# ilovin/lstm_ctc_ocr

Measured on AMD Instinct MI355X. Metric: captcha images/sec training (32x256, bs=64/GPU), higher is better.
Workload: dtype bf16; 1 GPU; VGG-7 + BiLSTM(256) + CTC train step, H=32 W=256, 10-char labels, C=64, bs=64/GPU (BASELINE.json configs[1]), Adam lr 1e-4 wd 1e-5 clip 10; global_batch=64, parallelism=dp1, hipgraph=True

## Files before the change

### include/ocr_hip.h

```cpp
#ifndef OCR_HIP_H
#define OCR_HIP_H
#include <stddef.h>
#ifdef __cplusplus
extern "C" {
#endif

enum { OCR_STATUS_OK = 0, OCR_STATUS_MEMOPS = 1, OCR_STATUS_INVALID = 2, OCR_STATUS_EXEC = 3 };

enum {
    OCR_EPI_BIAS = 1, OCR_EPI_RELU = 2, OCR_EPI_OUT_F32 = 4,
    OCR_EPI_MASK = 16, OCR_EPI_ROWSWAP = 32, OCR_EPI_ACCUM = 64
};

const char* ocr_status_string(int status);
int ocr_abi_version(void);
const char* ocr_build_id(void);

int ocr_ctc_workspace_size(int max_label_len, int max_time, int minibatch, size_t* bytes);
int ocr_ctc_loss(const float* activations, float* gradients, const int* flat_labels, const int* label_lengths,
                 const int* input_lengths, int alphabet_size, int minibatch, int max_time, int max_label_len,
                 int blank_label, float* costs, void* workspace, void* stream);
int ocr_ctc_debug(void* dbg);
int ocr_ctc_train_supported(int alphabet_size, int max_time, int max_label_len);
int ocr_ctc_loss_train(const float* activations, void* grad_ntc_bf16, float scale, const int* flat_labels,
                       const int* label_lengths, const int* input_lengths, int alphabet_size, int minibatch, int max_time,
                       int max_label_len, int blank_label, float* costs, void* stream);
int ocr_set_ctc_engine(int fast);
int ocr_ctc_long_placement(int alphabet_size, int max_time, int max_label_len);
int ocr_ctc_long_supported(int alphabet_size, int max_time, int max_label_len);
int ocr_ctc_long_workspace_size(int alphabet_size, int max_label_len, int max_time, int minibatch, size_t* bytes);
int ocr_ctc_loss_long(const float* activations, float* gradients ,
                      void* grad_ntc_bf16 , float scale,
                      const int* flat_labels, const int* label_lengths, const int* input_lengths,
                      int alphabet_size, int minibatch, int max_time, int max_label_len, int blank_label,
                      float* costs, void* workspace, size_t workspace_bytes, void* stream);
int ocr_ctc_greedy_decode(const float* activations, const int* input_lengths, int alphabet_size, int minibatch,
                          int max_time, int blank_label, int pad_value, int* decoded, int* decoded_lengths,
                          void* stream);

int ocr_ctc_beam_workspace_size(int alphabet_size, int minibatch, int max_time, int beam_width, size_t* bytes);
int ocr_ctc_beam_decode(const float* activations, const int* input_lengths, int alphabet_size, int minibatch,
                        int max_time, int beam_width, int merge_repeated, int pad_value, int* decoded,
                        int* decoded_lengths, float* neg_log_prob, void* workspace, size_t workspace_bytes, void* stream);
int ocr_ctc_beam_kernel_choice(int alphabet_size, int beam_width);
int ocr_set_beam_engine(int engine);

int ocr_gemm_nt_bf16(const void* P, long ldp, const void* Q, long ldq, void* out, long ldo, int M, int N, int K,
                     const float* bias, const void* mask, long ldmask, int flags, int splits, int row_group,
                     int row_skip, int swap_inner, int swap_outer, void* stream);
int ocr_set_gemm_engine(int use_large_tile);
int ocr_conv3x3_bf16(const void* x, const void* wpack, void* y, int Nb, int W, int H, int Cin, int Cout,
                     const float* bias, const void* mask, int flags, void* stream);
int ocr_conv3x3_stats_rows(int Nb, int W, int H, int Cin, int Cout, int flags);
int ocr_conv3x3_bf16_stats(const void* x, const void* wpack, void* y, int Nb, int W, int H, int Cin, int Cout, const float* bias, int flags,
                           float* partials, void* stream);
int ocr_conv3x3_kernel_choice(int Nb, int W, int H, int Cin, int Cout, int flags, int kw, int kh);
int ocr_conv3x3_accum_supported(int Nb, int W, int H, int Cin, int Cout);
int ocr_conv_halo_clock_debug(void* dbg);
int ocr_conv_ws_debug(void* dbg);
int ocr_conv3x3_pool_supported(int Nb, int W, int H, int Cin, int Cout, int kw, int kh);
int ocr_conv3x3_pool_codes_supported(int Nb, int W, int H, int Cin, int Cout, int kw, int kh);
int ocr_conv3x3_relu_pool_codes_bf16(const void* x, const void* wpack, void* y, void* pooled, void* codes, int Nb, int W, int H, int Cin,
                                     int Cout, const float* bias, int kw, int kh, void* stream);
int ocr_conv3x3_relu_pool_bf16(const void* x, const void* wpack, void* y, void* pooled, int Nb, int W, int H, int Cin, int Cout,
                               const float* bias, int kw, int kh, void* stream);
int ocr_conv3x3_unpool_supported(int Nb, int W, int H, int Cin, int Cout, int kw, int kh);
int ocr_conv3x3_dgrad_unpool_bf16(const void* dy, const void* wdgrad, void* out_full, const void* codes, int Nb, int W, int H, int Cin,
                                  int Cout, int kw, int kh, int relu_mask, void* stream);
int ocr_gemm_tn_bf16(const void* A, long lda, const void* B, long ldb, float* out, long ldo, int Mk, int I, int J,
                     int row_group, int row_skip, long a_row_off, float scale, int splits, float* colsum, void* stream);
long ocr_gemm_tn_split_workspace_floats(int Mk, int I, int J);
int ocr_gemm_tn_split_bf16(const void* A, long lda, const void* B, long ldb, float* out, long ldo, int Mk, int I, int J, float scale,
                           float* colsum, float* part, long part_floats, void* stream);
int ocr_gemm_tn_batched_bf16(const void* A, long lda, long strideA, const void* B, long ldb, long strideB, float* out, long ldo,
                             long strideOut, int Mk, int I, int J, int nbatch, float scale, int splits, float* colsum,
                             long strideColsum, void* stream);
typedef struct ocr_tn_job {
    const void* A; long lda; long strideA;
    const void* B; long ldb; long strideB;
    float* out; long ldo; long strideOut;
    float* colsum; long strideColsum;
    int Mk, I, J, nbatch;
    int row_group, row_skip;
    float scale; int reserved;
} ocr_tn_job;
int ocr_gemm_tn_jobs_supported(const ocr_tn_job* jobs, int njobs);
int ocr_gemm_tn_jobs_bf16(const ocr_tn_job* jobs, int njobs, void* stream);
int ocr_set_wgrad_engine(int engine);
int ocr_conv3x3_wgrad_bf16(const void* x, const void* dy, float* dw, float* dbias, int Nb, int W, int H, int Cin,
                           int Cout, int splits, void* stream);
int ocr_conv3x3_wgrad_kernel_choice(int Nb, int W, int H, int Cin, int Cout, int has_workspace, int splits);

int ocr_conv3x3_wgrad_workspace_size(int Nb, int W, int H, int Cin, int Cout, size_t* bytes);
int ocr_conv3x3_wgrad_ws_bf16(const void* x, const void* dy, float* dw, float* dbias, int Nb, int W, int H, int Cin,
                              int Cout, int splits, void* workspace, size_t workspace_bytes, void* stream);
int ocr_conv3x3_wgrad_defer_bf16(const void* x, const void* dy, float* dw, float* dbias, int Nb, int W, int H, int Cin, int Cout,
                                 void* workspace, size_t workspace_bytes, void* job, int* job_blocks, int* deferred, void* stream);
int ocr_wgrad9_reduce_jobs(const void* jobs, int njobs, int total_blocks, void* stream);

int ocr_conv1_fwd(const float* x, const float* w, const float* bias, void* y, int Nb, int W, int H, int Cout,
                  int relu, void* stream);
int ocr_conv1_wgrad(const float* x, const void* dz, float* dw, float* db, int Nb, int W, int H, int Cout,
                    void* stream);
int ocr_eltwise_bf16(int op, const void* a, const void* b, void* out, long n, void* stream);
int ocr_conv1_pool_fwd(const float* x, const float* w, const float* bias, void* p, int Nb, int W, int H, int Cout, void* stream);
int ocr_conv1_pool_fwd_train(const float* x, const float* w, const float* bias, void* p, int Nb, int W, int H, int Cout,
                             void* codes, float* zero, long zero_n, void* ones, long ones_n, void* stream);
int ocr_conv1_pool_bwd_codes(const float* x, const float* w, const float* bias, const void* dp, float* dw, float* db,
                             int Nb, int W, int H, int Cout, const void* codes, void* stream);
int ocr_conv1_pool_bwd_slab_rows(int Nb, int W, int H);
int ocr_conv1_pool_bwd_slab(const float* x, const float* w, const float* bias, const void* dp, int Nb, int W, int H, int Cout,
                            const void* codes, float* slab, void* stream);
int ocr_conv1_pool_bwd(const float* x, const float* w, const float* bias, const void* dp, float* dw, float* db, int Nb,
                       int W, int H, int Cout, void* stream);
int ocr_maxpool_fwd(const void* x, void* y, int Nb, int W, int H, int C, int kw, int kh, void* stream);
int ocr_maxpool_bwd(const void* x, const void* dy, void* dx, int Nb, int W, int H, int C, int kw, int kh,
                    int relu_mask, void* stream);
int ocr_maxpool_bwd_codes(const void* codes, const void* dy, void* dx, int Nb, int W, int H, int C, int kw, int kh,
                          int relu_mask, void* stream);
size_t ocr_bn_workspace_bytes(long M, int C);
int ocr_bn_train_fwd(const void* x, void* y, const float* gamma, const float* beta, float* save_mean,
                     float* save_rstd, long M, int C, float eps, int relu, void* workspace, const void* residual, void* stream);
int ocr_bn_train_bwd(const void* x, const void* y, const void* dy, void* dx, const float* gamma,
                     const float* save_mean, const float* save_rstd, float* dgamma, float* dbeta, long M, int C,
                     int relu, void* workspace, void* stream);
int ocr_bn_train_fwd2(const void* x, void* y, const float* gamma, const float* beta, float* save_mean, float* save_rstd, long M, int C,
                      float eps, int relu, void* workspace, const void* residual, int partial_rows, void* pooled, void* stream);
int ocr_bn_train_bwd2(const void* x, const void* y, const void* dy, void* dx, const float* gamma, const float* save_mean,
                      const float* save_rstd, float* dgamma, float* dbeta, long M, int C, int relu, void* workspace, int pooled_dy,
                      int partial_rows, void* stream);
int ocr_bn_train_fwd_codes(const void* x, const float* gamma, const float* beta, float* save_mean, float* save_rstd, long M, int C,
                           float eps, int relu, void* workspace, int partial_rows, void* pooled, void* codes, void* stream);
int ocr_bn_train_bwd_codes(const void* x, const void* codes, const void* dy, void* dx, const float* gamma, const float* save_mean,
                           const float* save_rstd, float* dgamma, float* dbeta, long M, int C, int relu, void* workspace, void* stream);
int ocr_bn_train_bwd_codes_col(const void* x, const void* codes, const void* col, int Nb, int W, int HC, void* dy_pooled_out, void* dx,
                               const float* gamma, const float* save_mean, const float* save_rstd, float* dgamma, float* dbeta, long M,
                               int C, int relu, void* workspace, void* stream);
int ocr_conv3x3_bnbwd_rows(int Nb, int W, int H, int Cin, int Cout);
int ocr_conv3x3_dgrad_bnbwd_bf16(const void* dy, const void* wdgrad, void* dx, int Nb, int W, int H, int Cin, int Cout, const void* mask_y,
                                 const void* z, const float* mean, const float* rstd, float* partials, void* stream);
int ocr_colsum_bf16(const void* a, float* out, long M, int C, long lda, void* stream);
int ocr_pack_transpose(const float* in, void* out, int R, int Cc, long ldin, int lstm_units, void* stream);
int ocr_pack_conv_dgrad(const float* w, void* out, int Cin, int Cout, void* stream);
int ocr_pack_jobs(const void* jobs, int njobs, int total_blocks, void* stream);
int ocr_cast_f32_bf16(const float* in, void* out, long n, void* stream);
int ocr_u8_to_unit_f32(const void* in, float* out, long n, void* stream);
int ocr_step_report(const float* costs, int n, const double* scalars, const void* word_addrs, int nwords, double* out, void* stream);
int ocr_bind_batch(const void* pixels, int pixels_are_u8, float* x, long n_pixels, const int* seq_len, int* seq_len_dst, int n_seq,
                   const int* labels, int* labels_dst, int n_labels, const int* labels_len, int* labels_len_dst, int n_labels_len,
                   void* stream);
int ocr_cast2d_f32_bf16(const float* in, long ldin, void* out, long ldout, int rows, int cols, void* stream);
int ocr_tnc_to_ntc_bf16(const float* in, void* out, int T, int N, int C, float scale, void* stream);
int ocr_conv5_col2im(const void* col, void* dx, int Nb, int W, int HC, void* stream);

int ocr_bn_infer_fwd(const void* x, void* y, const float* gamma, const float* beta, const float* mean, const float* var,
                     long M, int C, float eps, int relu, void* stream);
int ocr_bn_infer_bwd(const void* x, const void* y, const void* dy, void* dx, const float* gamma, const float* mean,
                     const float* var, float* dgamma, float* dbeta, long M, int C, float eps, int relu, void* stream);
int ocr_dropout_bf16(const void* in, void* out, long n, unsigned seed, const void* step_counter, float keep_prob, void* stream);
int ocr_avgpool_bf16(const void* src, void* dst, int Nb, int W, int H, int C, int kw, int kh, int backward, void* stream);
int ocr_subsample_bf16(const void* src, void* dst, int Nb, int W, int H, int C, int Wo, int Ho, int sw, int sh, int ow, int oh,
                       int backward, void* stream);
int ocr_softmax_f32(const float* in, float* out, long rows, int C, void* stream);

int ocr_lstm_fwd_step(const float* xproj, const void* whT_packed, const int* seq_len, void* hout, float* gates,
                      float* cell, int Nb, int T, int U, int step, float forget_bias, int ndir, void* stream);
int ocr_lstm_bwd_step(const void* wh, long ldw, long w_dir_stride, const int* seq_len, const void* dhout,
                      const float* gates, const float* cell, void* dz, float* dc_state, int Nb, int T, int U,
                      int step, int ndir, void* stream);
int ocr_lstm_seq_supported(int Nb, int U);
long ocr_lstm_seq_sync_words(int Nb, int U);
int ocr_lstm_seq_debug(void* dbg );
int ocr_lstm_seq_test_skew(int units, int at);
int ocr_lstm_fwd_seq(const float* xproj, const void* whT_packed, const int* seq_len, void* hout, float* gates,
                     float* cell, int Nb, int T, int U, float forget_bias, void* sync, void* stream);
int ocr_lstm_bwd_seq(const void* wh, long ldw, long w_dir_stride, const int* seq_len, const void* dhout,
                     const float* gates, const float* cell, void* dz, int Nb, int T, int U, void* sync, void* stream);
#define OCR_LSTM_PREPARED 1
int ocr_lstm_fwd_seq2(const float* xproj, const void* whT_packed, const int* seq_len, void* hout, float* gates,
                      float* cell, int Nb, int T, int U, float forget_bias, void* sync, int flags, void* stream);
int ocr_lstm_bwd_seq2(const void* wh, long ldw, long w_dir_stride, const int* seq_len, const void* dhout,
                      const float* gates, const float* cell, void* dz, int Nb, int T, int U, void* sync, int flags, void* stream);
int ocr_lstm_fwd_seq_x_supported(int Nb, int U, int D);
int ocr_lstm_fwd_seq_x(const void* x, const void* wxT_packed, const float* bias_packed, int D, const void* whT_packed,
                       const int* seq_len, void* hout, float* gates, float* cell, int Nb, int T, int U, float forget_bias,
                       void* sync, int flags, void* stream);
int ocr_set_lstm_proto(int proto);
int ocr_set_lstm_ksplit(int waves);
int ocr_lstm_hprev(const void* hout, const int* seq_len, void* hprev, int Nb, int T, int U, int ndir, void* stream);
int ocr_lstm_xh(const void* x, const void* hout, const int* seq_len, void* xh, int Nb, int T, int D, int U, int ndir, void* stream);
int ocr_lstm_pack_bias(const float* b_fw, const float* b_bw , float* out, int U, int ndir, void* stream);

int ocr_optim_scalar_count(void);
int ocr_optim_init(void* scalars , double lr, void* stream);
int ocr_optim_set_lr(void* scalars, double lr, int multiply, void* stream);
int ocr_optim_step(float* params, float* grads, float* state1, float* state2, long n, long reg_begin, long reg_end,
                   float weight_decay, float clip_norm, int solver, float beta1, float beta2, float eps,
                   void* scalars, void* stream);
int ocr_optim_step_guarded(float* params, float* grads, float* state1, float* state2, long n, long reg_begin, long reg_end,
                           float weight_decay, float clip_norm, int solver, float beta1, float beta2, float eps,
                           void* scalars, const void* guard_addrs, int nguard, void* stream);
int ocr_optim_step_guarded2(float* params, float* grads, float* state1, float* state2, long n, long reg_begin, long reg_end,
                            float weight_decay, float clip_norm, int solver, float beta1, float beta2, float eps,
                            void* scalars, const void* guard_addrs, int nguard, const float* drop_flag, void* stream);
int ocr_guard_flag(const void* guard_addrs, int nguard, float* flag_out, void* stream);

int ocr_captcha_synth(const int* params, int n_images, int words_per_image, int max_glyphs, const void* atlas, const int* stamp, int n_stamp,
                      void* out, int W, int out_h, int canvas_cap, int width_cap, void* stream);

int ocr_wgrad9_debug(void* dbg);

int ocr_probe_tr16(const int* addr , int* out , void* stream);
int ocr_probe_xcc(int* out , int nblocks, int threads, void* stream);
int ocr_occupy_cus(int nblocks, int threads, int lds_bytes, float us, void* stream);
int ocr_mfma_busy_probe(float* out, int nblocks, int threads , int iters, long long* clk, void* stream);

#ifdef __cplusplus
}
#endif
#endif
```

### lstm_ctc_ocr_amd/_native.py

```python
import ctypes
import os
import re

_HERE = os.path.dirname(os.path.abspath(__file__))
LIB_PATH = os.environ.get("OCR_NATIVE_LIB") or os.path.join(_HERE, "libocrhip.so")
HEADER_PATH = os.path.join(os.path.dirname(_HERE), "include", "ocr_hip.h")

EPI_BIAS, EPI_RELU, EPI_OUT_F32, EPI_MASK, EPI_ROWSWAP, EPI_ACCUM = 1, 2, 4, 16, 32, 64

_P, _I, _L, _F, _D = ctypes.c_void_p, ctypes.c_int, ctypes.c_long, ctypes.c_float, ctypes.c_double

_SIGS = {
    "ocr_abi_version": ([], _I),
    "ocr_build_id": ([], ctypes.c_char_p),
    "ocr_status_string": ([_I], ctypes.c_char_p),
    "ocr_ctc_workspace_size": ([_I, _I, _I, ctypes.POINTER(ctypes.c_size_t)], _I),
    "ocr_ctc_loss": ([_P, _P, _P, _P, _P, _I, _I, _I, _I, _I, _P, _P, _P], _I),
    "ocr_set_ctc_engine": ([_I], _I),
    "ocr_ctc_debug": ([_P], _I),
    "ocr_ctc_train_supported": ([_I, _I, _I], _I),
    "ocr_ctc_loss_train": ([_P, _P, _F, _P, _P, _P, _I, _I, _I, _I, _I, _P, _P], _I),
    "ocr_ctc_long_placement": ([_I, _I, _I], _I),
    "ocr_ctc_long_supported": ([_I, _I, _I], _I),
    "ocr_ctc_long_workspace_size": ([_I, _I, _I, _I, ctypes.POINTER(ctypes.c_size_t)], _I),
    "ocr_ctc_loss_long": ([_P, _P, _P, _F, _P, _P, _P, _I, _I, _I, _I, _I, _P, _P, ctypes.c_size_t, _P], _I),
    "ocr_ctc_greedy_decode": ([_P, _P, _I, _I, _I, _I, _I, _P, _P, _P], _I),
    "ocr_ctc_beam_workspace_size": ([_I, _I, _I, _I, ctypes.POINTER(ctypes.c_size_t)], _I),
    "ocr_ctc_beam_decode": ([_P, _P, _I, _I, _I, _I, _I, _I, _P, _P, _P, _P, ctypes.c_size_t, _P], _I),
    "ocr_ctc_beam_kernel_choice": ([_I, _I], _I),
    "ocr_set_beam_engine": ([_I], _I),
    "ocr_gemm_nt_bf16": ([_P, _L, _P, _L, _P, _L, _I, _I, _I, _P, _P, _L, _I, _I, _I, _I, _I, _I, _P], _I),
    "ocr_set_gemm_engine": ([_I], _I),
    "ocr_gemm_tn_batched_bf16": ([_P, _L, _L, _P, _L, _L, _P, _L, _L, _I, _I, _I, _I, _F, _I, _P, _L, _P], _I),
    "ocr_gemm_tn_jobs_supported": ([_P, _I], _I),
    "ocr_gemm_tn_jobs_bf16": ([_P, _I, _P], _I),
    "ocr_lstm_xh": ([_P, _P, _P, _P, _I, _I, _I, _I, _I, _P], _I),
    "ocr_set_wgrad_engine": ([_I], _I),
    "ocr_conv3x3_bf16": ([_P, _P, _P, _I, _I, _I, _I, _I, _P, _P, _I, _P], _I),
    "ocr_conv_halo_clock_debug": ([_P], _I),
    "ocr_occupy_cus": ([_I, _I, _I, _F, _P], _I),
    "ocr_conv_ws_debug": ([_P], _I),
    "ocr_conv3x3_accum_supported": ([_I, _I, _I, _I, _I], _I),
    "ocr_conv3x3_kernel_choice": ([_I, _I, _I, _I, _I, _I, _I, _I], _I),
    "ocr_conv3x3_pool_supported": ([_I, _I, _I, _I, _I, _I, _I], _I),
    "ocr_conv3x3_relu_pool_bf16": ([_P, _P, _P, _P, _I, _I, _I, _I, _I, _P, _I, _I, _P], _I),
    "ocr_conv3x3_pool_codes_supported": ([_I, _I, _I, _I, _I, _I, _I], _I),
    "ocr_conv3x3_relu_pool_codes_bf16": ([_P, _P, _P, _P, _P, _I, _I, _I, _I, _I, _P, _I, _I, _P], _I),
    "ocr_gemm_tn_bf16": ([_P, _L, _P, _L, _P, _L, _I, _I, _I, _I, _I, _L, _F, _I, _P, _P], _I),
    "ocr_gemm_tn_split_workspace_floats": ([_I, _I, _I], _L),
    "ocr_gemm_tn_split_bf16": ([_P, _L, _P, _L, _P, _L, _I, _I, _I, _F, _P, _P, _L, _P], _I),
    "ocr_conv3x3_wgrad_bf16": ([_P, _P, _P, _P, _I, _I, _I, _I, _I, _I, _P], _I),
    "ocr_conv3x3_wgrad_kernel_choice": ([_I, _I, _I, _I, _I, _I, _I], _I),
    "ocr_conv3x3_wgrad_workspace_size": ([_I, _I, _I, _I, _I, ctypes.POINTER(ctypes.c_size_t)], _I),
    "ocr_conv3x3_wgrad_ws_bf16": ([_P, _P, _P, _P, _I, _I, _I, _I, _I, _I, _P, ctypes.c_size_t, _P], _I),
    "ocr_conv3x3_wgrad_defer_bf16": ([_P, _P, _P, _P, _I, _I, _I, _I, _I, _P, ctypes.c_size_t, _P, ctypes.POINTER(_I),
                                      ctypes.POINTER(_I), _P], _I),
    "ocr_wgrad9_reduce_jobs": ([_P, _I, _I, _P], _I),
    "ocr_conv1_fwd": ([_P, _P, _P, _P, _I, _I, _I, _I, _I, _P], _I),
    "ocr_conv1_wgrad": ([_P, _P, _P, _P, _I, _I, _I, _I, _P], _I),
    "ocr_eltwise_bf16": ([_I, _P, _P, _P, _L, _P], _I),
    "ocr_conv1_pool_fwd": ([_P, _P, _P, _P, _I, _I, _I, _I, _P], _I),
    "ocr_conv1_pool_fwd_train": ([_P, _P, _P, _P, _I, _I, _I, _I, _P, _P, _L, _P, _L, _P], _I),
    "ocr_conv1_pool_bwd_codes": ([_P, _P, _P, _P, _P, _P, _I, _I, _I, _I, _P, _P], _I),
    "ocr_conv1_pool_bwd_slab_rows": ([_I, _I, _I], _I),
    "ocr_conv1_pool_bwd_slab": ([_P, _P, _P, _P, _I, _I, _I, _I, _P, _P, _P], _I),
    "ocr_conv1_pool_bwd": ([_P, _P, _P, _P, _P, _P, _I, _I, _I, _I, _P], _I),
    "ocr_maxpool_fwd": ([_P, _P, _I, _I, _I, _I, _I, _I, _P], _I),
    "ocr_maxpool_bwd": ([_P, _P, _P, _I, _I, _I, _I, _I, _I, _I, _P], _I),
    "ocr_bn_workspace_bytes": ([_L, _I], ctypes.c_size_t),
    "ocr_bn_train_fwd": ([_P, _P, _P, _P, _P, _P, _L, _I, _F, _I, _P, _P, _P], _I),
    "ocr_bn_train_bwd": ([_P, _P, _P, _P, _P, _P, _P, _P, _P, _L, _I, _I, _P, _P], _I),
    "ocr_bn_train_fwd2": ([_P, _P, _P, _P, _P, _P, _L, _I, _F, _I, _P, _P, _I, _P, _P], _I),
    "ocr_bn_train_bwd2": ([_P, _P, _P, _P, _P, _P, _P, _P, _P, _L, _I, _I, _P, _I, _I, _P], _I),
    "ocr_maxpool_bwd_codes": ([_P, _P, _P, _I, _I, _I, _I, _I, _I, _I, _P], _I),
    "ocr_bn_train_fwd_codes": ([_P, _P, _P, _P, _P, _L, _I, _F, _I, _P, _I, _P, _P, _P], _I),
    "ocr_bn_train_bwd_codes": ([_P, _P, _P, _P, _P, _P, _P, _P, _P, _L, _I, _I, _P, _P], _I),
    "ocr_bn_train_bwd_codes_col": ([_P, _P, _P, _I, _I, _I, _P, _P, _P, _P, _P, _P, _P, _L, _I, _I, _P, _P], _I),
    "ocr_conv3x3_unpool_supported": ([_I, _I, _I, _I, _I, _I, _I], _I),
    "ocr_conv3x3_dgrad_unpool_bf16": ([_P, _P, _P, _P, _I, _I, _I, _I, _I, _I, _I, _I, _P], _I),
    "ocr_conv3x3_bnbwd_rows": ([_I, _I, _I, _I, _I], _I),
    "ocr_conv3x3_dgrad_bnbwd_bf16": ([_P, _P, _P, _I, _I, _I, _I, _I, _P, _P, _P, _P, _P, _P], _I),
    "ocr_conv3x3_stats_rows": ([_I, _I, _I, _I, _I, _I], _I),
    "ocr_conv3x3_bf16_stats": ([_P, _P, _P, _I, _I, _I, _I, _I, _P, _I, _P, _P], _I),
    "ocr_bn_infer_fwd": ([_P, _P, _P, _P, _P, _P, _L, _I, _F, _I, _P], _I),
    "ocr_bn_infer_bwd": ([_P, _P, _P, _P, _P, _P, _P, _P, _P, _L, _I, _F, _I, _P], _I),
    "ocr_dropout_bf16": ([_P, _P, _L, ctypes.c_uint, _P, _F, _P], _I),
    "ocr_avgpool_bf16": ([_P, _P, _I, _I, _I, _I, _I, _I, _I, _P], _I),
    "ocr_subsample_bf16": ([_P, _P, _I, _I, _I, _I, _I, _I, _I, _I, _I, _I, _I, _P], _I),
    "ocr_softmax_f32": ([_P, _P, _L, _I, _P], _I),
    "ocr_colsum_bf16": ([_P, _P, _L, _I, _L, _P], _I),
    "ocr_pack_transpose": ([_P, _P, _I, _I, _L, _I, _P], _I),
    "ocr_pack_conv_dgrad": ([_P, _P, _I, _I, _P], _I),
    "ocr_pack_jobs": ([_P, _I, _I, _P], _I),
    "ocr_cast_f32_bf16": ([_P, _P, _L, _P], _I),
    "ocr_u8_to_unit_f32": ([_P, _P, _L, _P], _I),
    "ocr_step_report": ([_P, _I, _P, _P, _I, _P, _P], _I),
    "ocr_bind_batch": ([_P, _I, _P, _L, _P, _P, _I, _P, _P, _I, _P, _P, _I, _P], _I),
    "ocr_captcha_synth": ([_P, _I, _I, _I, _P, _P, _I, _P, _I, _I, _I, _I, _P], _I),
    "ocr_cast2d_f32_bf16": ([_P, _L, _P, _L, _I, _I, _P], _I),
    "ocr_tnc_to_ntc_bf16": ([_P, _P, _I, _I, _I, _F, _P], _I),
    "ocr_conv5_col2im": ([_P, _P, _I, _I, _I, _P], _I),
    "ocr_lstm_fwd_step": ([_P, _P, _P, _P, _P, _P, _I, _I, _I, _I, _F, _I, _P], _I),
    "ocr_lstm_bwd_step": ([_P, _L, _L, _P, _P, _P, _P, _P, _P, _I, _I, _I, _I, _I, _P], _I),
    "ocr_lstm_seq_supported": ([_I, _I], _I),
    "ocr_lstm_seq_debug": ([_P], _I),
    "ocr_lstm_seq_test_skew": ([_I, _I], _I),
    "ocr_lstm_seq_sync_words": ([_I, _I], _L),
    "ocr_lstm_fwd_seq": ([_P, _P, _P, _P, _P, _P, _I, _I, _I, _F, _P, _P], _I),
    "ocr_lstm_bwd_seq": ([_P, _L, _L, _P, _P, _P, _P, _P, _I, _I, _I, _P, _P], _I),
    "ocr_lstm_fwd_seq2": ([_P, _P, _P, _P, _P, _P, _I, _I, _I, _F, _P, _I, _P], _I),
    "ocr_lstm_fwd_seq_x_supported": ([_I, _I, _I], _I),
    "ocr_lstm_fwd_seq_x": ([_P, _P, _P, _I, _P, _P, _P, _P, _P, _I, _I, _I, _F, _P, _I, _P], _I),
    "ocr_lstm_bwd_seq2": ([_P, _L, _L, _P, _P, _P, _P, _P, _I, _I, _I, _P, _I, _P], _I),
    "ocr_lstm_hprev": ([_P, _P, _P, _I, _I, _I, _I, _P], _I),
    "ocr_lstm_pack_bias": ([_P, _P, _P, _I, _I, _P], _I),
    "ocr_optim_scalar_count": ([], _I),
    "ocr_optim_init": ([_P, _D, _P], _I),
    "ocr_optim_set_lr": ([_P, _D, _I, _P], _I),
    "ocr_optim_step": ([_P, _P, _P, _P, _L, _L, _L, _F, _F, _I, _F, _F, _F, _P, _P], _I),
    "ocr_optim_step_guarded": ([_P, _P, _P, _P, _L, _L, _L, _F, _F, _I, _F, _F, _F, _P, _P, _I, _P], _I),
    "ocr_optim_step_guarded2": ([_P, _P, _P, _P, _L, _L, _L, _F, _F, _I, _F, _F, _F, _P, _P, _I, _P, _P], _I),
    "ocr_guard_flag": ([_P, _I, _P, _P], _I),
    "ocr_wgrad9_debug": ([_P], _I),
    "ocr_probe_tr16": ([_P, _P, _P], _I),
    "ocr_set_lstm_proto": ([_I], _I),
    "ocr_set_lstm_ksplit": ([_I], _I),
    "ocr_probe_xcc": ([_P, _I, _I, _P], _I),
    "ocr_mfma_busy_probe": ([_P, _I, _I, _I, _P, _P], _I),
}


class NativeError(RuntimeError):
    pass


def declared_symbols(header=HEADER_PATH):
    text = open(header).read()
    text = re.sub(r"/\*.*?\*/", "", text, flags=re.S)
    return sorted(set(re.findall(r"\b(ocr_[a-z0-9_]+)\s*\(", text)))


def source_build_id(csrc=os.path.join(_HERE, "csrc"), experiments=False):
    import glob
    import hashlib
    rel = [os.path.basename(f) for f in glob.glob(os.path.join(csrc, "*.hip"))]
    h = hashlib.sha256()
    for f in sorted(rel) + ["common.h", "conv_plan.h", "Makefile"]:
        h.update(open(os.path.join(csrc, f), "rb").read())
    return h.hexdigest()[:16] + ("-exp" if experiments else "")


def build_id():
    return lib().ocr_build_id().decode()


_lib = None


def lib():
    global _lib
    if _lib is None:
        if not os.path.exists(LIB_PATH):
            raise NativeError(
                "libocrhip.so not found at %s — build it with `python -c 'import __graft_entry__ as g; g.build()'` "
                "(there is no CPU/eager fallback for the hot path)" % LIB_PATH)
        _lib = ctypes.CDLL(LIB_PATH)
        for name, (argtypes, restype) in _SIGS.items():
            fn = getattr(_lib, name)
            fn.argtypes = argtypes
            fn.restype = restype
        for env, setter in (("OCR_GEMM_ENGINE", "ocr_set_gemm_engine"), ("OCR_WGRAD_ENGINE", "ocr_set_wgrad_engine")):
            if os.environ.get(env):
                getattr(_lib, setter)(int(os.environ[env]))
    return _lib


def status_string(code):
    return lib().ocr_status_string(code).decode()


def call(name, *args):
    rc = getattr(lib(), name)(*args)
    if rc != 0:
        raise NativeError("%s failed: status %d (%s)" % (name, rc, status_string(rc)))


def ptr(t):
    return None if t is None else t.data_ptr()


def stream():
    import torch
    return torch.cuda.current_stream().cuda_stream
```

### lstm_ctc_ocr_amd/csrc/common.h

```cpp
#pragma once
#include <stdlib.h>
#include <hip/hip_runtime.h>
#include <stdint.h>
#include <atomic>

#define OCR_WAVE 64

enum {
    OCR_OK = 0,
    OCR_ERR_MEMOPS = 1,
    OCR_ERR_INVALID = 2,
    OCR_ERR_EXEC = 3,
};

#define OCR_CHECK_LAUNCH()                                        \
    do {                                                          \
        hipError_t e__ = hipGetLastError();                       \
        if (e__ != hipSuccess) return OCR_ERR_EXEC;               \
    } while (0)

typedef uint16_t bf16_t;
typedef __attribute__((ext_vector_type(8))) __bf16 bf16x8;
typedef __attribute__((ext_vector_type(4))) float f32x4;
typedef __attribute__((ext_vector_type(4))) unsigned int u32x4;
typedef __attribute__((ext_vector_type(2))) unsigned int u32x2;

__device__ __forceinline__ bf16_t f2bf(float f) {
    uint32_t u = __float_as_uint(f);
    if ((u & 0x7fffffffu) > 0x7f800000u) return (bf16_t)((u >> 16) | 0x40);
    u += 0x7fffu + ((u >> 16) & 1u);
    return (bf16_t)(u >> 16);
}
__device__ __forceinline__ float bf2f(bf16_t h) { return __uint_as_float(((uint32_t)h) << 16); }
typedef __attribute__((ext_vector_type(2))) __bf16 bf16x2_t;
__device__ __forceinline__ uint32_t pack_bf2(float lo, float hi) {
    bf16x2_t v = {(__bf16)lo, (__bf16)hi};
    return __builtin_bit_cast(uint32_t, v);
}
__device__ __forceinline__ float bf_lo(uint32_t p) { return __uint_as_float(p << 16); }
__device__ __forceinline__ float bf_hi(uint32_t p) { return __uint_as_float(p & 0xffff0000u); }

template <int CNT>
__device__ __forceinline__ uint32_t pool_code_word(const u32x4 (&rows)[CNT]) {
    uint32_t word = 0;
#pragma unroll
    for (int c = 0; c < 8; ++c) {
        float v[CNT];
#pragma unroll
        for (int e = 0; e < CNT; ++e) {
            const uint32_t pr = c < 2 ? rows[e].x : c < 4 ? rows[e].y : c < 6 ? rows[e].z : rows[e].w;
            v[e] = (c & 1) ? bf_hi(pr) : bf_lo(pr);
        }
        int best = 0; float bv = v[0];
#pragma unroll
        for (int e = 1; e < CNT; ++e) if (v[e] > bv) { bv = v[e]; best = e; }
        word |= (uint32_t)(best | ((bv > 0.f) ? 4 : 0)) << (4 * c);
    }
    return word;
}

typedef unsigned short u16x2_t __attribute__((ext_vector_type(2)));
template <int CNT>
__device__ __forceinline__ uint32_t pool_code2_u16(const uint32_t (&p)[CNT], uint32_t& mx) {
    const u16x2_t one = {1, 1};
    u16x2_t v[CNT];
#pragma unroll
    for (int e = 0; e < CNT; ++e) v[e] = __builtin_bit_cast(u16x2_t, p[e]);
    u16x2_t m = v[0];
#pragma unroll
    for (int e = 1; e < CNT; ++e) m = __builtin_elementwise_max(m, v[e]);
    u16x2_t t = __builtin_elementwise_min((u16x2_t)(m - v[CNT - 2]), one);
#pragma unroll
    for (int e = CNT - 3; e >= 0; --e) t = __builtin_elementwise_min((u16x2_t)(m - v[e]), one) * (u16x2_t)(t + one);
    const u16x2_t code = t + (u16x2_t)(__builtin_elementwise_min(m, one) << (u16x2_t){2, 2});
    mx = __builtin_bit_cast(uint32_t, m);
    return __builtin_bit_cast(uint32_t, code);
}
__device__ __forceinline__ uint32_t pool_code2_merge(uint32_t c0, uint32_t c1, uint32_t c2, uint32_t c3) {
    return ((c0 | (c0 >> 12)) & 0xffu) | (((c1 | (c1 >> 12)) & 0xffu) << 8) | (((c2 | (c2 >> 12)) & 0xffu) << 16) | ((c3 | (c3 >> 12)) << 24);
}

__device__ __forceinline__ void unpack8(u32x4 p, float* f) {
    f[0] = bf_lo(p.x); f[1] = bf_hi(p.x); f[2] = bf_lo(p.y); f[3] = bf_hi(p.y);
    f[4] = bf_lo(p.z); f[5] = bf_hi(p.z); f[6] = bf_lo(p.w); f[7] = bf_hi(p.w);
}
__device__ __forceinline__ uint32_t max2(uint32_t a, uint32_t b) {
    uint32_t lo = (bf_lo(b) > bf_lo(a)) ? (b & 0xffffu) : (a & 0xffffu);
    uint32_t hi = (bf_hi(b) > bf_hi(a)) ? (b & 0xffff0000u) : (a & 0xffff0000u);
    return lo | hi;
}
__device__ __forceinline__ u32x4 max8(u32x4 a, u32x4 b) {
    u32x4 r = {max2(a.x, b.x), max2(a.y, b.y), max2(a.z, b.z), max2(a.w, b.w)};
    return r;
}
__device__ __forceinline__ u32x4 col2im_unit8(const bf16_t* __restrict__ col, unsigned idx, int W, int HC) {
    const unsigned hc8 = (unsigned)HC >> 3;
    const unsigned e = (idx % hc8) * 8u, q = idx / hc8;
    const unsigned w = q % (unsigned)W, n = q / (unsigned)W;
    float a[8], b[8];
#pragma unroll
    for (int c = 0; c < 8; ++c) { a[c] = 0.f; b[c] = 0.f; }
    const long r0 = ((long)n * (W - 1) + w) * 2L;
    if ((int)w < W - 1) unpack8(*(const u32x4*)(col + r0 * HC + e), a);
    if (w > 0) unpack8(*(const u32x4*)(col + (r0 - 1) * HC + e), b);
    bf16_t o[8];
#pragma unroll
    for (int c = 0; c < 8; ++c) o[c] = f2bf((0.f + a[c]) + b[c]);
    u32x4 pk = {(uint32_t)o[0] | ((uint32_t)o[1] << 16), (uint32_t)o[2] | ((uint32_t)o[3] << 16),
                (uint32_t)o[4] | ((uint32_t)o[5] << 16), (uint32_t)o[6] | ((uint32_t)o[7] << 16)};
    return pk;
}

__device__ __forceinline__ float wave_sum(float v) {
#pragma unroll
    for (int o = 32; o > 0; o >>= 1) v += __shfl_xor(v, o, 64);
    return v;
}
__device__ __forceinline__ float wave_max(float v) {
#pragma unroll
    for (int o = 32; o > 0; o >>= 1) v = fmaxf(v, __shfl_xor(v, o, 64));
    return v;
}
template <typename AccT, bool STORE = false>
__device__ __forceinline__ void block_channel_reduce(const float (&v)[8], float* red, AccT* dst, int C, int groups,
                                                     int rl, int gq, int rlanes) {
    __syncthreads();
    if (rl < rlanes) {
#pragma unroll
        for (int c = 0; c < 8; ++c) red[rl * C + gq * 8 + c] = v[c];
    }
    __syncthreads();
    for (int ch = threadIdx.x; ch < C; ch += 256) {
        float t = 0.f;
        for (int r = 0; r < rlanes; ++r) t += red[r * C + ch];
        if (STORE) dst[ch] = (AccT)t;
        else atomicAdd(&dst[ch], (AccT)t);
    }
}

__device__ __forceinline__ float sigmoidf_(float x) { return __frcp_rn(1.0f + __expf(-x)); }
__device__ __forceinline__ float tanhf_(float x) {
    float e = __expf(-2.0f * fabsf(x));
    float t = (1.0f - e) * __frcp_rn(1.0f + e);
    return copysignf(t, x);
}

static inline const char* ocr_tune_env(const char* name) {
#ifdef OCR_EXPERIMENTS
    return getenv(name);
#else
    (void)name; return nullptr;
#endif
}
__device__ __forceinline__ long long ocr_wall_clock() { return (long long)__builtin_amdgcn_s_memrealtime(); }
__device__ __forceinline__ void ocr_clk_enter(long long* clk) {
    clk[0] = (long long)__builtin_amdgcn_s_memtime(); clk[1] = ocr_wall_clock();
}
__device__ __forceinline__ void ocr_clk_exit(long long* clk) {
    const long long c = (long long)__builtin_amdgcn_s_memtime(), t = ocr_wall_clock();
    clk[2] = c; clk[3] = t;
    clk[4] += c - clk[0]; clk[5] += t - clk[1]; clk[6] += 1;
}
__host__ __device__ static inline int ceil_div(long a, long b) { return (int)((a + b - 1) / b); }
static inline int grid_for(long total, int cap = 4096) {
    long b = (total + 255) / 256;
    if (b > cap) b = cap;
    if (b < 1) b = 1;
    return (int)b;
}

#define OCR_MAX_DEVICES 64
template <auto KERNEL>
static inline hipError_t ocr_allow_lds(int bytes) {
    static std::atomic<int> allowed[OCR_MAX_DEVICES];
    int dev = 0;
    if (hipGetDevice(&dev) != hipSuccess || dev < 0 || dev >= OCR_MAX_DEVICES) return hipErrorInvalidDevice;
    int have = allowed[dev].load(std::memory_order_acquire);
    if (bytes <= have) return hipSuccess;
    const hipError_t e = hipFuncSetAttribute((const void*)KERNEL, hipFuncAttributeMaxDynamicSharedMemorySize, bytes);
    if (e != hipSuccess) return e;
    while (have < bytes && !allowed[dev].compare_exchange_weak(have, bytes, std::memory_order_acq_rel)) {}
    return hipSuccess;
}
```

### lstm_ctc_ocr_amd/csrc/gemm.hip

```cpp
#include "conv_plan.h"
#include <string.h>

enum {
    EPI_BIAS = 1,
    EPI_RELU = 2,
    EPI_OUT_F32 = 4,
    EPI_ATOMIC = 8,
    EPI_MASK = 16,
    EPI_ROWSWAP = 32,
    EPI_ACCUM = 64,
};

struct GemmArgs {
    const bf16_t* P;
    const bf16_t* Q;
    long ldp, ldq;
    int M, N, K;
    int k_per_split;
    int grp, skip;
    int cW, cH, cC;
    void* out;
    long ldo;
    const float* bias;
    const bf16_t* mask;
// ... 118 lines not shown
#pragma unroll
            for (int b = 0; b < FM; ++b)
                bfr[b] = *(const bf16x8*)(&Ps[(wm * 16 * FM + b * 16 + frow) * LDS_ROW + fk]);
#pragma unroll
            for (int a = 0; a < FN; ++a)
#pragma unroll
                for (int b = 0; b < FM; ++b)
                    acc[a][b] = __builtin_amdgcn_mfma_f32_16x16x32_bf16(af[a], bfr[b], acc[a][b], 0, 0, 0);
        }
    }

    const int flags = g.flags;
    const bool add_bias = (flags & EPI_BIAS) && (!(flags & EPI_ATOMIC) || blockIdx.z == 0);
#pragma unroll
    for (int a = 0; a < FN; ++a) {
        int n = n0 + wn * 16 * FN + a * 16 + (lane >> 4) * 4;
        if (n >= g.N) continue;
        f32x4 bv = {0.f, 0.f, 0.f, 0.f};
        if (add_bias) bv = *(const f32x4*)(g.bias + n);
#pragma unroll
        for (int b = 0; b < FM; ++b) {
            int m = m0 + wm * 16 * FM + b * 16 + (lane & 15);
            if (m >= g.M) continue;
            f32x4 v = acc[a][b] + bv;
            if (flags & EPI_RELU) {
                v.x = fmaxf(v.x, 0.f); v.y = fmaxf(v.y, 0.f); v.z = fmaxf(v.z, 0.f); v.w = fmaxf(v.w, 0.f);
            }
            if (flags & EPI_MASK) {
                u32x2 mk = *(const u32x2*)(g.mask + (long)m * g.ldmask + n);
                if (!(bf_lo(mk.x) > 0.f)) v.x = 0.f;
                if (!(bf_hi(mk.x) > 0.f)) v.y = 0.f;
                if (!(bf_lo(mk.y) > 0.f)) v.z = 0.f;
                if (!(bf_hi(mk.y) > 0.f)) v.w = 0.f;
            }
            long orow = m;
            if (flags & EPI_ROWSWAP) orow = (long)(m % g.swap_inner) * g.swap_outer + m / g.swap_inner;
            if (flags & EPI_OUT_F32) {
                float* o = (float*)g.out + orow * g.ldo + n;
                if (flags & EPI_ATOMIC) {
                    atomicAdd(o + 0, v.x); atomicAdd(o + 1, v.y); atomicAdd(o + 2, v.z); atomicAdd(o + 3, v.w);
                } else if (flags & EPI_ACCUM) {
                    f32x4 old = *(f32x4*)o;
                    *(f32x4*)o = old + v;
                } else {
                    *(f32x4*)o = v;
                }
            } else {
                u32x2 pk;
                pk.x = pack_bf2(v.x, v.y);
                pk.y = pack_bf2(v.z, v.w);
                *(u32x2*)((bf16_t*)g.out + orow * g.ldo + n) = pk;
            }
        }
    }
}

template <int MODE, int FM, int FN>
static int launch_gemm(const GemmArgs& g, hipStream_t stream) {
    constexpr int BM = 32 * FM, BN = 32 * FN;
    int splits = ceil_div(g.K, g.k_per_split);
    dim3 grid(ceil_div(g.M, BM), ceil_div(g.N, BN), splits);
    gemm_nt_kernel<MODE, FM, FN><<<grid, 256, 0, stream>>>(g);
    OCR_CHECK_LAUNCH();
    return OCR_OK;
}

static int dispatch_gemm(GemmArgs& g, int mode, int splits, hipStream_t stream) {
    if (g.M <= 0 || g.N <= 0 || g.K <= 0 || (g.K & 7) || (g.N & 3)) return OCR_ERR_INVALID;
    if (!g.P || !g.Q || !g.out) return OCR_ERR_INVALID;
    if (splits < 1) splits = 1;
    int kps = ceil_div(ceil_div(g.K, splits), 32) * 32;
    g.k_per_split = kps;
    if (splits > 1) {
        if (!(g.flags & EPI_OUT_F32) || (g.flags & (EPI_RELU | EPI_MASK | EPI_ACCUM))) return OCR_ERR_INVALID;
        g.flags |= EPI_ATOMIC;
    }
    long big_blocks = (long)ceil_div(g.M, 128) * ceil_div(g.N, 128) * ceil_div(g.K, kps);
    bool big = big_blocks >= 192 && g.N >= 128;
    if (mode == 1) {
        if (g.cC % 32 || g.K != 9 * g.cC) return OCR_ERR_INVALID;
        return big ? launch_gemm<1, 4, 4>(g, stream) : launch_gemm<1, 2, 2>(g, stream);
    }
    return big ? launch_gemm<0, 4, 4>(g, stream) : launch_gemm<0, 2, 2>(g, stream);
}

int ig_try_dispatch(const void* P, long ldp, const void* Q, long ldq, void* out, long ldo, int M, int N, int K,
                    const float* bias, const void* mask, long ldmask, int flags, int mode, int grp, int skip, int cW,
                    int cH, int cC, int swap_inner, int swap_outer, hipStream_t stream);
static int g_use_igemm = 1, g_use_halo = 1;
extern int g_ig_stages;
extern "C" int ocr_set_gemm_engine(int mode) {
    if (mode < 0 || mode > 3) return OCR_ERR_INVALID;
    g_use_igemm = mode != 0; g_use_halo = mode == 1; g_ig_stages = (mode == 2) ? 2 : 3;
    return OCR_OK;
}

extern "C" int ocr_gemm_nt_bf16(const void* P, long ldp, const void* Q, long ldq, void* out, long ldo,
                                int M, int N, int K, const float* bias, const void* mask, long ldmask,
                                int flags, int splits, int row_group, int row_skip, int swap_inner,
                                int swap_outer, void* stream) {
    GemmArgs g = {};
    g.P = (const bf16_t*)P; g.Q = (const bf16_t*)Q; g.ldp = ldp; g.ldq = ldq;
    g.M = M; g.N = N; g.K = K; g.grp = row_group; g.skip = row_skip;
    g.out = out; g.ldo = ldo; g.bias = bias; g.mask = (const bf16_t*)mask; g.ldmask = ldmask;
    g.flags = flags & ~EPI_ATOMIC; g.swap_inner = swap_inner; g.swap_outer = swap_outer;
    if ((flags & EPI_BIAS) && !bias) return OCR_ERR_INVALID;
    if ((flags & EPI_MASK) && !mask) return OCR_ERR_INVALID;
    if ((flags & EPI_ROWSWAP) && (swap_inner <= 0 || swap_outer <= 0)) return OCR_ERR_INVALID;
    if (g_use_igemm && splits <= 1 && P && Q && out && M > 0 && N > 0 && K > 0) {
        int rc = ig_try_dispatch(P, ldp, Q, ldq, out, ldo, M, N, K, bias, mask, ldmask, g.flags, 0, row_group, row_skip, 0, 0, 0,
                                 swap_inner, swap_outer, (hipStream_t)stream);
        if (rc >= 0) return rc;
    }
    return dispatch_gemm(g, 0, splits, (hipStream_t)stream);
}


struct ConvKnobs {
    int ws, k2, k3, k2_cfg;
    int k2_minsteps, k2_mintiles, k2_allow_a, k2_abl, k2_nst;
    int k3_minsteps, k3_genw, k3_prio;
    int halo_nw, halo_stagger, halo_stagger_bit, halo_prio;
};
static int env_int(const char* e, int dflt) { return e ? atoi(e) : dflt; }
static ConvKnobs read_conv_knobs() {
    ConvKnobs k;
    k.ws = env_int(getenv("OCR_CONV_WS"), 1);
    k.k2 = env_int(getenv("OCR_CONV_K2"), 1);
    k.k3 = env_int(getenv("OCR_CONV_K3"), 1);
    const char* cfg = getenv("OCR_K2_CFG");
    k.k2_cfg = (cfg && (cfg[0] == 'A' || cfg[0] == 'D')) ? cfg[0] : 0;
    k.k2_minsteps = env_int(ocr_tune_env("OCR_K2_MINSTEPS"), 18);
    k.k2_mintiles = env_int(ocr_tune_env("OCR_K2_MINTILES"), 128);
    const char* tiles = ocr_tune_env("OCR_K2_TILES");
    k.k2_allow_a = !(tiles && tiles[0] == 'D');
    k.k2_abl = env_int(ocr_tune_env("OCR_K2_ABL"), 0);
    k.k2_nst = env_int(ocr_tune_env("OCR_K2_NST"), 0);
    k.k3_minsteps = env_int(ocr_tune_env("OCR_K3_MINSTEPS"), 18);
    k.k3_genw = env_int(ocr_tune_env("OCR_K3_GENW"), 1);
    k.k3_prio = env_int(ocr_tune_env("OCR_K3_PRIO"), 2);
    k.halo_nw = env_int(ocr_tune_env("OCR_HALO_NW"), 0);
    const char* st = ocr_tune_env("OCR_HALO_STAGGER");
    const char* comma = st ? strchr(st, ',') : nullptr;
    k.halo_stagger = st && atoi(st) > 0 ? atoi(st) : 0;
    k.halo_stagger_bit = comma ? atoi(comma + 1) : 32;
    k.halo_prio = env_int(ocr_tune_env("OCR_HALO_PRIO"), 1);
    return k;
}
static const ConvKnobs& conv_knobs() {
    static const ConvKnobs k = read_conv_knobs();
    return k;
}

static bool plan_ws(ConvPlan& p, const ConvKnobs& k) {
    if (!k.ws || (p.flags & ~(EPI_BIAS | EPI_RELU | EPI_MASK))) return false;
    if (p.epi_kind && (!(p.flags & EPI_RELU) || (p.flags & EPI_MASK))) return false;
    if ((p.Cout & 63) || (long)p.M * p.Cin * 2 > 0x7fffffffL || (long)p.M * p.Cout * 2 > 0x7fffffffL) return false;
    int nc, bm;
    if (p.H == 16 && p.Cin == 64) { nc = 16; bm = 256; }
    else if (p.H == 16 && p.Cin == 128) { nc = 8; bm = 128; }
    else if (p.H == 8 && p.Cin == 128) { nc = 16; bm = 128; }
    else return false;
    if (p.W % nc || p.M % bm || (p.epi_kind == CONV_EPI_POOL22 && (p.W & 1))) return false;
    static int cus = 0;
    if (!cus) {
        int dev = 0; hipDeviceProp_t prop;
        if (hipGetDevice(&dev) == hipSuccess && hipGetDeviceProperties(&prop, dev) == hipSuccess && prop.multiProcessorCount > 0) cus = prop.multiProcessorCount;
    }
    const int ncu = cus > 0 ? cus : 256;
    const int mtiles = p.M / bm, ntiles = p.Cout / 64;
    if (k.ws == 1 && (p.Cin != 64 || (long)mtiles * ntiles < 2L * ncu)) return false;
    int slots = ncu / ntiles;
    if (slots < 1) slots = 1;
    if (slots > mtiles) slots = mtiles;
    p.per_slot = (mtiles + slots - 1) / slots;
    p.slots = (mtiles + p.per_slot - 1) / p.per_slot;
    p.grid = p.slots * ntiles;
    p.xcd_map = (p.grid % 8 == 0 && (p.grid / 8) % ntiles == 0) ? 1 : 0;
    p.family = CONV_WS; p.ws_nc = nc; p.ws_ksplit = p.Cin == 64 ? 1 : 2;
    return true;
}

static char k2_tile(const ConvPlan& p, const ConvKnobs& k, int minsteps) {
    const long M = p.M;
    if ((p.Cin & 63) || (p.Cout & 63) || M < 4096 || p.H > 16 || p.H < 1) return 0;
    if (M * p.Cin * 2 >= 0x7fffffffL || (long)p.Cout * 9 * p.Cin * 2 >= 0x7fffffffL) return 0;
    for (int pass = 0; pass < 2; ++pass)
        for (const char c : {'A', 'D'}) {
            if (k.k2_cfg && c != k.k2_cfg) continue;
            if (!k.k2_cfg && c == 'A' && !k.k2_allow_a) continue;
            const int bn = c == 'A' ? 128 : 64;
            if (p.Cout % bn) continue;
            if (k.k2_cfg) return c;
            if (9 * (p.Cin / 64) < minsteps) return 0;
            if ((M + 255) / 256 * (p.Cout / bn) >= (pass == 0 ? 224 : k.k2_mintiles)) return c;
        }
    return 0;
}

static bool plan_k3(ConvPlan& p, const ConvKnobs& k, char tile) {
    const int H = p.H, epi = p.epi_kind;
    if (H != 2 && H != 4 && H != 8 && H != 16) return false;
    if (p.M % 256 || (p.Cin & 63) || (p.Cout & 63) || (tile == 'A' && p.Cout % 128)) return false;
    const int NC = 256 / H, PS = (NC + 2 + 7) / 8 * 8;
    const bool genw = p.W % NC != 0;
    if (genw && (H == 16 || NC + 2 + (NC + p.W - 1) / p.W > PS)) return false;
    if (genw && !k.k3_genw) return false;
    if (H == 2 && (!genw || epi == CONV_EPI_POOL12 || epi == CONV_EPI_POOL22)) return false;
    if (epi >= CONV_EPI_STATS && (p.flags & EPI_ACCUM)) return false;
    if (epi == CONV_EPI_BNBWD && (!(p.flags & EPI_MASK) || p.Cin == 64 || (H != 4 && H != 8))) return false;
    p.family = CONV_K3; p.tile = tile; p.genw = genw; p.single = H == 16 && p.Cin == 64; p.prio = k.k3_prio;
    return true;
}

static bool plan_k3_k2(ConvPlan& p, const ConvKnobs& k) {
    if (k.k3) {
        const char t = k2_tile(p, k, k.k3_minsteps >= 0 ? k.k3_minsteps : k.k2_minsteps);
        if (t && plan_k3(p, k, t)) return true;
    }
    if (p.epi_kind >= CONV_EPI_STATS) return false;
    const char t = k2_tile(p, k, k.k2_minsteps);
    if (!t) return false;
    int nst = t == 'A' ? 5 : 4;
    if ((t == 'A' && k.k2_nst == 4) || (t == 'D' && (k.k2_nst == 5 || k.k2_nst == 6))) nst = k.k2_nst;
    const int FM = t == 'A' ? 8 : 4, BN = t == 'A' ? 128 : 64;
    const int NRpad = (256 + 2 * p.H + 4 + 7) / 8 * 8;
    const int lds = 2 * NRpad * 128 + nst * BN * 128;
    if (lds > 163840 || lds < 8 * FM * 2048) return false;
#ifdef OCR_EXPERIMENTS
    if (lds + 10240 > 163840 && (k.k2_abl & 8)) return false;
#endif
    p.family = CONV_K2; p.tile = t; p.nst = nst; p.abl = k.k2_abl;
    return true;
}

static bool plan_halo(ConvPlan& p, const ConvKnobs& k) {
    const int H = p.H, Cout = p.Cout, nw = k.halo_nw;
    p.prio = k.halo_prio; p.stagger = k.halo_stagger; p.stagger_bit = k.halo_stagger_bit;
    if (nw != 8) {
        const int NR = 128 + 2 * H + 2, NRp = (NR + 32) / 32 * 32;
        const long mt4 = (p.M + 127) / 128;
        if (NRp / 32 == 5 || NRp / 32 == 6) {
            p.family = CONV_HALO; p.nw = 4; p.bn = (Cout >= 128 && mt4 * ((Cout + 127) / 128) >= 448) ? 128 : 64;
            return true;
        }
        if (nw == 4) return false;
    }
    const int NRpad = (256 + 2 * H + 2 + 64) / 64 * 64;
    if (NRpad / 64 != 5 && NRpad / 64 != 6) return false;
    const long mt = (p.M + 255) / 256;
    p.family = CONV_HALO; p.nw = 8;
    p.bn = (Cout >= 128 && (mt * ((Cout + 127) / 128) >= 200 || mt * ((Cout + 63) / 64) < 256)) ? 128 : 64;
    return true;
}

static void plan_unpool(ConvPlan& p, const ConvKnobs& k) {
    const int H = p.H;
    if (!k.k2 || !k.k3 || p.flags || (H != 4 && H != 8) || p.M <= 0 || p.M % 256 || p.W % (256 / H) || (p.Cin & 63) || (p.Cout & 63)) return;
    if ((long)p.M * p.Cin * 2 >= 0x7fffffffL || (long)p.Cout * 9 * p.Cin * 2 >= 0x7fffffffL) return;
    const ConvPlan plain = conv3x3_plan(p.M, p.W, H, p.Cin, p.Cout, 0, CONV_EPI_PLAIN);
    p.tile = (plain.family == CONV_K3 && !plain.genw) ? plain.tile : ((p.Cout % 128) ? 'D' : 'A');
    p.family = CONV_K3; p.genw = false; p.single = false; p.prio = k.k3_prio;
}

ConvPlan conv3x3_plan(int M, int W, int H, int Cin, int Cout, int flags, int epi_kind) {
    const ConvKnobs& k = conv_knobs();
    ConvPlan p = {};
    p.family = CONV_GEMM; p.M = M; p.W = W; p.H = H; p.Cin = Cin; p.Cout = Cout; p.flags = flags; p.epi_kind = epi_kind;
    if (epi_kind == CONV_EPI_UNPOOL12 || epi_kind == CONV_EPI_UNPOOL22) {
        if (g_use_halo) plan_unpool(p, k);
        return p;
    }
    if (!g_use_halo || (Cin & 63) || (Cout & 3) || M < 1024 || H > 30) return p;
    if (flags & ~(EPI_BIAS | EPI_RELU | EPI_MASK | EPI_ACCUM)) return p;
    if (epi_kind < CONV_EPI_STATS && plan_ws(p, k)) return p;
    if (epi_kind >= CONV_EPI_STATS) {
        if (epi_kind > CONV_EPI_BNBWD || (flags & EPI_ACCUM) || (M & 255)) return p;
        if (epi_kind == CONV_EPI_STATS ? (flags & EPI_MASK) != 0 : !(flags & EPI_MASK)) return p;
        if (k.k2) plan_k3_k2(p, k);
        return p;
    }
    if (epi_kind) {
        if ((flags & (EPI_MASK | EPI_ACCUM)) || !(flags & EPI_RELU) || (H & 1) || (Cout % 64)) return p;
        if (epi_kind == CONV_EPI_POOL22 && ((H != 4 && H != 8 && H != 16) || (W & 1))) return p;
        if (epi_kind != CONV_EPI_POOL12 && epi_kind != CONV_EPI_POOL22) return p;
        if (M % (epi_kind == CONV_EPI_POOL22 ? 2 * H : 2)) return p;
    }
    if (k.k2 && plan_k3_k2(p, k)) return p;
    plan_halo(p, k);
    return p;
}

static int conv3x3_launch(const ConvPlan& p, const ConvOperands& o, hipStream_t stream) {
    switch (p.family) {
    case CONV_WS: return launch_ws(p, o, stream);
    case CONV_K3: return launch_k3(p, o, stream);
    case CONV_K2: return launch_k2(p, o, stream);
    case CONV_HALO: return launch_halo(p, o, stream);
    }
    return OCR_ERR_INVALID;
}
static int conv3x3_pixels(int Nb, int W, int H, int Cin, int Cout) {
    const long M = (long)Nb * W * H;
    return (Nb <= 0 || W <= 0 || H <= 0 || Cin <= 0 || Cout <= 0 || M > 0x7fffffffL) ? 0 : (int)M;
}

extern "C" int ocr_conv3x3_accum_supported(int Nb, int W, int H, int Cin, int Cout) {
    return conv3x3_plan(conv3x3_pixels(Nb, W, H, Cin, Cout), W, H, Cin, Cout, EPI_ACCUM, CONV_EPI_PLAIN).family != CONV_GEMM;
}
extern "C" int ocr_conv3x3_kernel_choice(int Nb, int W, int H, int Cin, int Cout, int flags, int kw, int kh) {
    if (Nb <= 0 || W <= 0 || H <= 0 || Cin <= 0 || Cout <= 0) return -OCR_ERR_INVALID;
    const int pool_kind = (kw == 1 && kh == 2) ? 1 : ((kw == 2 && kh == 2) ? 2 : 0);
    if ((kw || kh) && !pool_kind) return 0;
    return conv3x3_plan(Nb * W * H, W, H, Cin, Cout, flags & ~(EPI_ATOMIC | EPI_ROWSWAP), pool_kind).choice();
}

extern "C" int ocr_conv3x3_bf16(const void* x, const void* wpack, void* y, int Nb, int W, int H,
                                int Cin, int Cout, const float* bias, const void* mask, int flags,
                                void* stream) {
    GemmArgs g = {};
    g.P = (const bf16_t*)x; g.Q = (const bf16_t*)wpack; g.ldp = Cin; g.ldq = 9L * Cin;
    g.M = Nb * W * H; g.N = Cout; g.K = 9 * Cin; g.cW = W; g.cH = H; g.cC = Cin;
// ... 71 lines not shown
```

### lstm_ctc_ocr_amd/csrc/gemm_tn.hip

```cpp
#include "common.h"

struct TnArgs {
    const bf16_t* A;
    const bf16_t* B;
    long lda, ldb;
    int Mk;
    int I, J;
    int k_per_split;
    int grp, skip;
    long a_row_off;
    int cW, cH, cC;
    float* out;
    long ldo;
    float scale;
    float* colsum;
    float* part;
};

typedef __attribute__((ext_vector_type(8))) unsigned short u16x8;

typedef __attribute__((ext_vector_type(4))) short s16x4;
typedef __attribute__((ext_vector_type(8))) short s16x8;

template <bool USE_TR>
// ... 24 lines not shown
    constexpr int NCA = 32 * CPA / 256, NCB = 32 * CPB / 256;
    static_assert(NCA >= 1 && NCB >= 1, "tile too small for 256 threads");
    __shared__ __attribute__((aligned(16))) bf16_t As[32 * LDA];
    __shared__ __attribute__((aligned(16))) bf16_t Bs[32 * LDB];

    const int tid = threadIdx.x, lane = tid & 63, wave = tid >> 6;
    const int wi = wave >> 1, wj = wave & 1;
    const int itiles = ceil_div(g.I, BI);
    const int tap = (MODE == 1) ? (int)(blockIdx.x / itiles) : 0;
    const int i0 = (int)(blockIdx.x % itiles) * BI;
    const int j0 = blockIdx.y * BJ;
    const int kbeg = blockIdx.z * g.k_per_split;
    const int kend = min(g.Mk, kbeg + g.k_per_split);
    const int dw = tap / 3 - 1, dh = tap % 3 - 1;
    const bool do_cs = g.colsum != nullptr && i0 == 0 && (MODE == 0 || tap == 4);
    float cs[8] = {0.f, 0.f, 0.f, 0.f, 0.f, 0.f, 0.f, 0.f};

    u32x4 ast[NCA], bst[NCB];
    auto load_tiles = [&](int k0) {
#pragma unroll
        for (int t = 0; t < NCA; ++t) {
            int c = tid + t * 256;
            int r = c / CPA, col = (c % CPA) * 8;
            int m = k0 + r;
            u32x4 v = {0, 0, 0, 0};
            bool ok = m < kend && (i0 + col) < g.I;
            if (ok) {
                if (MODE == 0) {
                    long phys = (long)m + (g.grp > 0 ? (long)(m / g.grp) * g.skip : 0);
                    v = *(const u32x4*)(g.A + phys * g.lda + g.a_row_off + i0 + col);
                } else {
                    int h = m % g.cH, q = m / g.cH, w = q % g.cW;
                    int ww = w + dw, hh = h + dh;
                    if ((unsigned)ww < (unsigned)g.cW && (unsigned)hh < (unsigned)g.cH)
                        v = *(const u32x4*)(g.A + ((long)m + (long)dw * g.cH + dh) * g.cC + i0 + col);
                }
            }
            ast[t] = v;
        }
#pragma unroll
        for (int t = 0; t < NCB; ++t) {
            int c = tid + t * 256;
            int r = c / CPB, col = (c % CPB) * 8;
            int m = k0 + r;
            u32x4 v = {0, 0, 0, 0};
            if (m < kend && (j0 + col) < g.J) v = *(const u32x4*)(g.B + (long)m * g.ldb + j0 + col);
            bst[t] = v;
        }
    };
    auto store_tiles = [&]() {
#pragma unroll
        for (int t = 0; t < NCA; ++t) {
            int c = tid + t * 256;
            *(u32x4*)(&As[(c / CPA) * LDA + (c % CPA) * 8]) = ast[t];
        }
#pragma unroll
        for (int t = 0; t < NCB; ++t) {
            int c = tid + t * 256;
            *(u32x4*)(&Bs[(c / CPB) * LDB + (c % CPB) * 8]) = bst[t];
        }
    };

    f32x4 acc[FI][FJ];
#pragma unroll
    for (int a = 0; a < FI; ++a)
#pragma unroll
        for (int b = 0; b < FJ; ++b) acc[a][b] = (f32x4){0.f, 0.f, 0.f, 0.f};

    if (kbeg < kend) {
        load_tiles(kbeg);
        for (int k0 = kbeg; k0 < kend; k0 += 32) {
            __syncthreads();
            store_tiles();
            if (do_cs) {
#pragma unroll
                for (int t = 0; t < NCB; ++t) {
                    cs[0] += bf_lo(bst[t].x); cs[1] += bf_hi(bst[t].x); cs[2] += bf_lo(bst[t].y); cs[3] += bf_hi(bst[t].y);
                    cs[4] += bf_lo(bst[t].z); cs[5] += bf_hi(bst[t].z); cs[6] += bf_lo(bst[t].w); cs[7] += bf_hi(bst[t].w);
                }
            }
            __syncthreads();
            if (k0 + 32 < kend) load_tiles(k0 + 32);
            bf16x8 af[FI], bfr[FJ];
#pragma unroll
            for (int a = 0; a < FI; ++a) af[a] = load_frag<USE_TR>(As, LDA, wi * 16 * FI + a * 16, lane);
#pragma unroll
            for (int b = 0; b < FJ; ++b) bfr[b] = load_frag<USE_TR>(Bs, LDB, wj * 16 * FJ + b * 16, lane);
#pragma unroll
            for (int a = 0; a < FI; ++a)
#pragma unroll
                for (int b = 0; b < FJ; ++b)
                    acc[a][b] = __builtin_amdgcn_mfma_f32_16x16x32_bf16(af[a], bfr[b], acc[a][b], 0, 0, 0);
        }
    }

    if (do_cs) {
        __shared__ float red[256 * 8];
#pragma unroll
        for (int e = 0; e < 8; ++e) red[tid * 8 + e] = cs[e];
        __syncthreads();
        if (tid < BJ && j0 + tid < g.J) {
            float t = 0.f;
            for (int u = tid >> 3; u < 256; u += CPB) t += red[u * 8 + (tid & 7)];
            if (g.part) g.part[(long)blockIdx.z * ((long)g.I * g.J + g.J) + (long)g.I * g.J + j0 + tid] = t * g.scale;
            else atomicAdd(g.colsum + j0 + tid, t * g.scale);
        }
    }
    float* pz = g.part ? g.part + (long)blockIdx.z * ((long)g.I * g.J + g.J) : nullptr;
    float* out = g.out;
    long ldo = g.ldo;
    if (MODE == 1) { out += (long)tap * g.cC * g.J; ldo = g.J; }
#pragma unroll
    for (int a = 0; a < FI; ++a) {
#pragma unroll
        for (int b = 0; b < FJ; ++b) {
            int j = j0 + wj * 16 * FJ + b * 16 + (lane & 15);
            if (j >= g.J) continue;
#pragma unroll
            for (int r = 0; r < 4; ++r) {
                int i = i0 + wi * 16 * FI + a * 16 + (lane >> 4) * 4 + r;
                if (i < g.I) {
                    if (pz) pz[(long)i * g.J + j] = acc[a][b][r] * g.scale;
                    else atomicAdd(out + (long)i * ldo + j, acc[a][b][r] * g.scale);
                }
            }
        }
    }
}

template <int MODE, int FI, int FJ>
static int launch_tn(const TnArgs& g, int taps, hipStream_t stream) {
    constexpr int BI = 32 * FI, BJ = 32 * FJ;
    dim3 grid(ceil_div(g.I, BI) * taps, ceil_div(g.J, BJ), ceil_div(g.Mk, g.k_per_split));
    gemm_tn_kernel<MODE, FI, FJ><<<grid, 256, 0, stream>>>(g);
    OCR_CHECK_LAUNCH();
    return OCR_OK;
}

static int pick_splits(long tiles, int Mk) {
    int s = (int)((1024 + tiles - 1) / tiles);
    int maxs = Mk / 128; if (maxs < 1) maxs = 1;
    if (s > maxs) s = maxs;
    if (s < 1) s = 1;
    return s;
}

int tn2_try_dispatch(const void* A, long lda, const void* B, long ldb, float* out, long ldo, int Mk, int I, int J, int mode,
                     int grp, int skip, long a_row_off, int cW, int cH, int cC, float scale, int splits, float* colsum,
                     hipStream_t stream, int nbatch = 1, long sA = 0, long sB = 0, long sO = 0, long sC = 0);
int wgrad9_try_dispatch(const void* x, const void* dy, float* dw, float* dbias, int Nb, int W, int H, int Cin, int Cout,
                        void* workspace, size_t ws_bytes, hipStream_t stream, void* defer_job = nullptr, int* defer_blocks = nullptr);
int tn2_choice(int Mk, int I, int J, int mode, int splits, int nbatch, int* S);
int wgrad9_choice(int Nb, int W, int H, int Cin, int Cout, int* S);
static int g_use_tn2 = 1, g_use_w9 = 1;
extern "C" int ocr_set_wgrad_engine(int engine) { g_use_tn2 = engine != 0; g_use_w9 = engine >= 2; return OCR_OK; }

extern "C" int ocr_gemm_tn_bf16(const void* A, long lda, const void* B, long ldb, float* out, long ldo,
                                int Mk, int I, int J, int row_group, int row_skip, long a_row_off,
                                float scale, int splits, float* colsum, void* stream) {
    if (!A || !B || !out || Mk <= 0 || I <= 0 || J <= 0 || (I & 7) || (J & 7)) return OCR_ERR_INVALID;
    TnArgs g = {};
    g.A = (const bf16_t*)A; g.B = (const bf16_t*)B; g.lda = lda; g.ldb = ldb; g.Mk = Mk; g.I = I; g.J = J;
    if (g_use_tn2) {
        int rc = tn2_try_dispatch(A, lda, B, ldb, out, ldo, Mk, I, J, 0, row_group, row_skip, a_row_off, 0, 0, 0, scale, splits,
                                  colsum, (hipStream_t)stream);
        if (rc >= 0) return rc;
    }
    g.grp = row_group; g.skip = row_skip; g.a_row_off = a_row_off; g.out = out; g.ldo = ldo; g.scale = scale; g.colsum = colsum;
    bool big = (I >= 128 && J >= 128);
    long tiles = big ? (long)ceil_div(I, 128) * ceil_div(J, 128) : (long)ceil_div(I, 64) * ceil_div(J, 64);
    if (splits <= 0) splits = pick_splits(tiles, Mk);
    g.k_per_split = ceil_div(ceil_div(Mk, splits), 32) * 32;
    return big ? launch_tn<0, 4, 4>(g, 1, (hipStream_t)stream) : launch_tn<0, 2, 2>(g, 1, (hipStream_t)stream);
}

__global__ __launch_bounds__(256) void tn_split_reduce_kernel(const float* __restrict__ part, int S, int I, int J, float* __restrict__ out,
                                                              long ldo, float* __restrict__ colsum) {
    const long IJ = (long)I * J, stride = IJ + J;
    const long e = (long)blockIdx.x * 256 + threadIdx.x;
    if (e >= stride || (e >= IJ && colsum == nullptr)) return;
    float t = 0.f;
    int s = 0;
    for (; s + 8 <= S; s += 8) {
        float v[8];
#pragma unroll
        for (int u = 0; u < 8; ++u) v[u] = part[(long)(s + u) * stride + e];
#pragma unroll
        for (int u = 0; u < 8; ++u) t += v[u];
    }
    for (; s < S; ++s) t += part[(long)s * stride + e];
    if (e < IJ) out[(e / J) * ldo + e % J] += t;
    else colsum[e - IJ] += t;
}

static void tn_split_plan(int Mk, int I, int J, bool* big, int* k_per_split, int* S) {
    *big = (I >= 128 && J >= 128);
    long tiles = *big ? (long)ceil_div(I, 128) * ceil_div(J, 128) : (long)ceil_div(I, 64) * ceil_div(J, 64);
    *k_per_split = ceil_div(ceil_div(Mk, pick_splits(tiles, Mk)), 32) * 32;
    *S = ceil_div(Mk, *k_per_split);
}

extern "C" long ocr_gemm_tn_split_workspace_floats(int Mk, int I, int J) {
    if (Mk <= 0 || I <= 0 || J <= 0) return -1;
    bool big; int kps, S;
    tn_split_plan(Mk, I, J, &big, &kps, &S);
    return (long)S * ((long)I * J + J);
}

extern "C" int ocr_gemm_tn_split_bf16(const void* A, long lda, const void* B, long ldb, float* out, long ldo, int Mk, int I, int J,
                                      float scale, float* colsum, float* part, long part_floats, void* stream) {
    if (!A || !B || !out || !part || Mk <= 0 || I <= 0 || J <= 0 || (I & 7) || (J & 7) || ldo < J) return OCR_ERR_INVALID;
    if (part_floats < ocr_gemm_tn_split_workspace_floats(Mk, I, J)) return OCR_ERR_INVALID;
    TnArgs g = {};
    g.A = (const bf16_t*)A; g.B = (const bf16_t*)B; g.lda = lda; g.ldb = ldb; g.Mk = Mk; g.I = I; g.J = J;
    g.out = out; g.ldo = ldo; g.scale = scale; g.colsum = colsum; g.part = part;
    bool big; int S;
    tn_split_plan(Mk, I, J, &big, &g.k_per_split, &S);
    int rc = big ? launch_tn<0, 4, 4>(g, 1, (hipStream_t)stream) : launch_tn<0, 2, 2>(g, 1, (hipStream_t)stream);
    if (rc != OCR_OK) return rc;
    const long n = (long)I * J + J;
    tn_split_reduce_kernel<<<(unsigned)ceil_div(n, 256), 256, 0, (hipStream_t)stream>>>(part, S, I, J, out, ldo, colsum);
    OCR_CHECK_LAUNCH();
    return OCR_OK;
}

extern "C" int ocr_gemm_tn_batched_bf16(const void* A, long lda, long strideA, const void* B, long ldb, long strideB, float* out,
                                        long ldo, long strideOut, int Mk, int I, int J, int nbatch, float scale, int splits,
                                        float* colsum, long strideColsum, void* stream) {
    if (!A || !B || !out || Mk <= 0 || I <= 0 || J <= 0 || (I & 7) || (J & 7) || nbatch <= 0) return OCR_ERR_INVALID;
    if (g_use_tn2 && nbatch > 1) {
        int rc = tn2_try_dispatch(A, lda, B, ldb, out, ldo, Mk, I, J, 0, 0, 0, 0, 0, 0, 0, scale, splits, colsum, (hipStream_t)stream,
                                  nbatch, strideA, strideB, strideOut, strideColsum);
        if (rc >= 0) return rc;
    }
    for (int b = 0; b < nbatch; ++b) {
        int rc = ocr_gemm_tn_bf16((const bf16_t*)A + b * strideA, lda, (const bf16_t*)B + b * strideB, ldb, out + b * strideOut, ldo, Mk,
                                  I, J, 0, 0, 0, scale, splits, colsum ? colsum + b * strideColsum : nullptr, stream);
        if (rc != OCR_OK) return rc;
    }
    return OCR_OK;
}

extern "C" int ocr_conv3x3_wgrad_bf16(const void* x, const void* dy, float* dw, float* dbias, int Nb, int W, int H,
                                      int Cin, int Cout, int splits, void* stream);
extern "C" int ocr_conv3x3_wgrad_ws_bf16(const void* x, const void* dy, float* dw, float* dbias, int Nb, int W, int H, int Cin,
                                         int Cout, int splits, void* workspace, size_t workspace_bytes, void* stream) {
    if (!x || !dy || !dw || Nb <= 0 || W <= 0 || H <= 0 || (Cin & 7) || (Cout & 7)) return OCR_ERR_INVALID;
    if (g_use_w9 && workspace && splits <= 0) {
        int rc = wgrad9_try_dispatch(x, dy, dw, dbias, Nb, W, H, Cin, Cout, workspace, workspace_bytes, (hipStream_t)stream);
        if (rc >= 0) return rc;
    }
    return ocr_conv3x3_wgrad_bf16(x, dy, dw, dbias, Nb, W, H, Cin, Cout, splits, stream);
}

extern "C" int ocr_conv3x3_wgrad_defer_bf16(const void* x, const void* dy, float* dw, float* dbias, int Nb, int W, int H, int Cin,
                                            int Cout, void* workspace, size_t workspace_bytes, void* job, int* job_blocks,
                                            int* deferred, void* stream) {
    if (!x || !dy || !dw || !job || !job_blocks || !deferred || Nb <= 0 || W <= 0 || H <= 0 || (Cin & 7) || (Cout & 7)) return OCR_ERR_INVALID;
    *deferred = 0;
    if (g_use_w9 && workspace) {
        int rc = wgrad9_try_dispatch(x, dy, dw, dbias, Nb, W, H, Cin, Cout, workspace, workspace_bytes, (hipStream_t)stream, job, job_blocks);
        if (rc >= 0) { if (rc == OCR_OK) *deferred = 1; return rc; }
    }
    return ocr_conv3x3_wgrad_bf16(x, dy, dw, dbias, Nb, W, H, Cin, Cout, 0, stream);
}

static void tn_wgrad_plan(int Mk, int Cin, int Cout, int splits, bool* big, int* k_per_split) {
    *big = (Cin >= 128 && Cout >= 128);
    long tiles = 9L * (*big ? (long)ceil_div(Cin, 128) * ceil_div(Cout, 128) : (long)ceil_div(Cin, 64) * ceil_div(Cout, 64));
    if (splits <= 0) splits = pick_splits(tiles, Mk);
    *k_per_split = ceil_div(ceil_div(Mk, splits), 32) * 32;
}

extern "C" int ocr_conv3x3_wgrad_bf16(const void* x, const void* dy, float* dw, float* dbias, int Nb, int W, int H,
                                      int Cin, int Cout, int splits, void* stream) {
    if (!x || !dy || !dw || Nb <= 0 || W <= 0 || H <= 0 || (Cin & 7) || (Cout & 7)) return OCR_ERR_INVALID;
    if (g_use_tn2) {
        int rc = tn2_try_dispatch(x, Cin, dy, Cout, dw, Cout, Nb * W * H, Cin, Cout, 1, 0, 0, 0, W, H, Cin, 1.0f, splits, dbias,
                                  (hipStream_t)stream);
        if (rc >= 0) return rc;
    }
    TnArgs g = {};
    g.A = (const bf16_t*)x; g.B = (const bf16_t*)dy; g.lda = Cin; g.ldb = Cout;
    g.Mk = Nb * W * H; g.I = Cin; g.J = Cout; g.cW = W; g.cH = H; g.cC = Cin;
    g.out = dw; g.ldo = Cout; g.scale = 1.0f; g.colsum = dbias;
    bool big;
    tn_wgrad_plan(g.Mk, Cin, Cout, splits, &big, &g.k_per_split);
    return big ? launch_tn<1, 4, 4>(g, 9, (hipStream_t)stream) : launch_tn<1, 2, 2>(g, 9, (hipStream_t)stream);
}

extern "C" int ocr_conv3x3_wgrad_kernel_choice(int Nb, int W, int H, int Cin, int Cout, int has_workspace, int splits) {
    if (Nb <= 0 || W <= 0 || H <= 0 || Cin <= 0 || Cout <= 0 || (Cin & 7) || (Cout & 7)) return -OCR_ERR_INVALID;
    int S = 0, k;
    if (g_use_w9 && has_workspace && splits <= 0 && (k = wgrad9_choice(Nb, W, H, Cin, Cout, &S)) >= 0) return k | (S << 8);
    const int Mk = Nb * W * H;
    if (g_use_tn2 && (k = tn2_choice(Mk, Cin, Cout, 1, splits, 1, &S)) >= 0) return (k == 2 ? 6 : 5) | (S << 8);
    bool big; int kps;
    tn_wgrad_plan(Mk, Cin, Cout, splits, &big, &kps);
    return (big ? 7 : 8) | (ceil_div(Mk, kps) << 8);
}
```

### lstm_ctc_ocr_amd/csrc/wgrad9.hip

```cpp
#include "common.h"
#include <stdlib.h>
#include <utility>
#include <type_traits>

struct W9Args {
    const bf16_t* X; const bf16_t* dY;
    int M, Cin, Cout, cW, cH;
    int k_per_split;
    int S, T_ci, T_co, map;
    float* part;
    float* cs_part;
};

__device__ u32x4 w9_zero_page[4];
typedef const __attribute__((address_space(1))) void* gptr_t;
typedef __attribute__((address_space(3))) void* lptr_t;
typedef __attribute__((ext_vector_type(4))) short s16x4;

constexpr int W9_NDMA = 5;
constexpr int W9_STAGE = 8 * W9_NDMA * 1024;
constexpr int W9_NST = 3;
constexpr int W9_LA = 2;
constexpr int W9_NSLOT = W9_LA + 1;
constexpr int W9_DMA_AT = 3;
constexpr unsigned W9_ZOFF = W9_NST * W9_STAGE;
constexpr int W9_LDS = 4 * 9 * 4 * 4 * 64 * 4;

__device__ __forceinline__ void w9_tr(s16x4& dst, unsigned addr, int imm) { asm volatile("ds_read_b64_tr_b16 %0, %1 offset:%2" : "=v"(dst) : "v"(addr), "n"(imm)); }
#define W9_WAIT(n) asm volatile("s_waitcnt lgkmcnt(%0)" ::"n"(n) : "memory")

constexpr int w9_gsize(int p) { return (p == 0 || p == 10) ? 8 : 2; }
constexpr int w9_gpos(int n) { return n < 9 ? 1 + n : 2 + n; }
constexpr int w9_younger(int n, int upto) { int o = 0; for (int q = w9_gpos(n) + 1; q <= upto; ++q) o += w9_gsize(q); return o; }
constexpr int w9_upto(int n, int LA) {
    int p = w9_gpos(n) + LA;
    if (p > 19) p = 19;
    const int own = n == 0 ? 10 : 2;
    while (own + w9_younger(n, p) > 15) --p;
    return p;
}
struct W9Tab { int upto[18]; int wait[18]; };
constexpr W9Tab w9_make_tab(int LA) {
    W9Tab t = {};
    for (int n = 0; n < 18; ++n) { t.upto[n] = w9_upto(n, LA); t.wait[n] = w9_younger(n, t.upto[n]); }
    return t;
}
constexpr W9Tab W9_TAB = w9_make_tab(W9_LA);

template <int FROM, int... I, class F>
__device__ __forceinline__ void w9_for_seq(std::integer_sequence<int, I...>, F&& f) { (f(std::integral_constant<int, FROM + I>{}), ...); }
template <int FROM, int TO, class F>
__device__ __forceinline__ void w9_for(F&& f) { w9_for_seq<FROM>(std::make_integer_sequence<int, (TO >= FROM ? TO - FROM + 1 : 0)>{}, f); }

__device__ __forceinline__ void w9_wait(int reads) {
    switch (reads) {
        case 0: W9_WAIT(0); break;   case 2: W9_WAIT(2); break;   case 4: W9_WAIT(4); break;   case 6: W9_WAIT(6); break;
        case 8: W9_WAIT(8); break;   case 10: W9_WAIT(10); break; case 12: W9_WAIT(12); break; default: W9_WAIT(14); break;
    }
}

__device__ __forceinline__ void w9_mfma_tap(f32x4 (&acc)[4], const s16x4& alo, const s16x4& ahi, const s16x4 (&blo)[4], const s16x4 (&bhi)[4]) {
    const u32x2 lo = __builtin_bit_cast(u32x2, alo), hi = __builtin_bit_cast(u32x2, ahi);
    const u32x4 av = {lo.x, lo.y, hi.x, hi.y};
    const bf16x8 fa = __builtin_bit_cast(bf16x8, av);
#pragma unroll
    for (int c = 0; c < 4; ++c) {
        const u32x2 bl = __builtin_bit_cast(u32x2, blo[c]), bh = __builtin_bit_cast(u32x2, bhi[c]);
        const u32x4 bv = {bl.x, bl.y, bh.x, bh.y};
        acc[c] = __builtin_amdgcn_mfma_f32_16x16x32_bf16(fa, __builtin_bit_cast(bf16x8, bv), acc[c], 0, 0, 0);
    }
}

__device__ __forceinline__ void w9_block_decode(const W9Args& g, int& split, int& tile) {
    const int b = blockIdx.x, T = g.T_ci * g.T_co;
    if (g.map == 1) { const int x = b & 7, q = b >> 3; split = (q / T) * 8 + x; tile = q % T; }
    else if (g.map == 2) { const int x = b & 7, q = b >> 3, G = 8 / g.S; split = x / G; tile = (x % G) * (T / G) + q; }
    else { split = b / T; tile = b % T; }
}

__device__ __forceinline__ unsigned w9_cs_offset(int tid) {
    const int csq = tid & 7, csr = tid >> 3;
    return csr * 128 + (((((csq >> 1) ^ ((csr >> 1) & 3)) << 1) | (csq & 1)) << 4);
}
__device__ __forceinline__ void w9_cs_step(float (&cs)[8], unsigned addr) {
    u32x4 v0, v1;
    asm volatile("ds_read_b128 %0, %1" : "=v"(v0) : "v"(addr));
    asm volatile("ds_read_b128 %0, %1 offset:8192" : "=v"(v1) : "v"(addr));
    W9_WAIT(0);
    __builtin_amdgcn_sched_barrier(0);
    cs[0] += bf_lo(v0.x) + bf_lo(v1.x); cs[1] += bf_hi(v0.x) + bf_hi(v1.x); cs[2] += bf_lo(v0.y) + bf_lo(v1.y); cs[3] += bf_hi(v0.y) + bf_hi(v1.y);
    cs[4] += bf_lo(v0.z) + bf_lo(v1.z); cs[5] += bf_hi(v0.z) + bf_hi(v1.z); cs[6] += bf_lo(v0.w) + bf_lo(v1.w); cs[7] += bf_hi(v0.w) + bf_hi(v1.w);
}
__device__ __forceinline__ void w9_cs_store(const W9Args& g, unsigned char* smem, const float (&cs)[8], int split, int co0, int tid) {
    float* red = (float*)smem;
#pragma unroll
    for (int e = 0; e < 8; ++e) red[tid * 8 + e] = cs[e];
    __syncthreads();
    if (tid < 64) {
        float s = 0.f;
        for (int u = 0; u < 64; ++u) s += red[(u * 8 + (tid >> 3)) * 8 + (tid & 7)];
        g.cs_part[(long)split * g.Cout + co0 + tid] = s;
    }
    __syncthreads();
}

__device__ __forceinline__ void w9_store_tile(const W9Args& g, unsigned char* smem, const f32x4 (&acc)[9][4], int split, int ci0, int co0,
                                              int cb, int kh, int lane) {
    const int g4 = lane >> 4, L = lane & 15;
    float* xch = (float*)smem + cb * (9 * 4 * 4 * 64) + lane;
    if (kh == 1) {
#pragma unroll
        for (int t = 0; t < 9; ++t)
#pragma unroll
            for (int c = 0; c < 4; ++c)
#pragma unroll
                for (int r = 0; r < 4; ++r) xch[((t * 4 + c) * 4 + r) * 64] = acc[t][c][r];
    }
    __syncthreads();
    if (kh == 0) {
        float* slab = g.part + (long)split * 9 * g.Cin * g.Cout;
#pragma unroll
        for (int t = 0; t < 9; ++t)
#pragma unroll
            for (int c = 0; c < 4; ++c)
#pragma unroll
                for (int r = 0; r < 4; ++r) {
                    const int ci = ci0 + cb * 16 + g4 * 4 + r, co = co0 + c * 16 + L;
                    slab[((long)t * g.Cin + ci) * g.Cout + co] = acc[t][c][r] + xch[((t * 4 + c) * 4 + r) * 64];
                }
    }
}

__global__ __launch_bounds__(512) void wgrad9_kernel(W9Args g) {
    extern __shared__ __attribute__((aligned(16))) unsigned char smem[];
    const int tid = threadIdx.x, lane = tid & 63;
    const unsigned lds0 = (unsigned)(size_t)(lptr_t)smem;
    const int wave = __builtin_amdgcn_readfirstlane(tid >> 6);
    const int cb = wave & 3, kh = wave >> 2;
    const int H = g.cH, W = g.cW;
    int split, tile;
    w9_block_decode(g, split, tile);
    const int ti = tile / g.T_co, tj = tile % g.T_co;
    const int ci0 = ti * 64, co0 = tj * 64;
    const int kbeg = split * g.k_per_split;
    const int kend = min(g.M, kbeg + g.k_per_split);
    const int nsteps = kend > kbeg ? (kend - kbeg + 127) >> 7 : 0;
    const int NR = 128 + 2 * H + 2;
    const int nhalo = (NR + 7) >> 3;
    const int NRp = nhalo << 3;
    const bool do_cs = g.cs_part != nullptr && ti == 0;
    const bf16_t* zero = (const bf16_t*)w9_zero_page;

    const int rr = lane >> 3, pp = lane & 7;
    const int qsrc = ((((pp >> 1) ^ ((rr >> 1) & 3)) << 1) | (pp & 1)) * 8;
    const bf16_t* src[W9_NDMA];
    int pix[W9_NDMA];
#pragma unroll
    for (int i = 0; i < W9_NDMA; ++i) {
        const int u = wave + 8 * i;
        src[i] = zero; pix[i] = 0x40000000;
        if (u < nhalo) {
            const int r = 8 * u + rr;
            pix[i] = (r < NR) ? kbeg - (H + 1) + r : 0x40000000;
            src[i] = g.X + (long)(kbeg - (H + 1) + r) * g.Cin + ci0 + qsrc;
        } else if (u < nhalo + 16) {
            const int r = 8 * (u - nhalo) + rr;
            pix[i] = kbeg + r;
            src[i] = g.dY + (long)(kbeg + r) * g.Cout + co0 + qsrc;
        }
    }
    auto stage_load = [&](int step, int buf) {
        unsigned char* st = smem + buf * W9_STAGE;
#pragma unroll
        for (int i = 0; i < W9_NDMA; ++i) {
            const int u = wave + 8 * i;
            const int px = pix[i] + step * 128;
            const bf16_t* s = zero;
            if (u < nhalo) { if (px >= 0 && px < g.M) s = src[i] + (long)step * 128 * g.Cin; }
            else if (u < nhalo + 16) { if (px < kend) s = src[i] + (long)step * 128 * g.Cout; }
            __builtin_amdgcn_global_load_lds((gptr_t)s, (lptr_t)(st + u * 1024), 16, 0, 0);
        }
    };

    const int g4 = lane >> 4, L = lane & 15;
    const int rowl = kh * 64 + 4 * g4 + (L >> 2);
    unsigned offA[9], offB[4];
#pragma unroll
    for (int t = 0; t < 9; ++t) {
        const int a0 = rowl + (H + 1) + (t / 3 - 1) * H + (t % 3 - 1);
        offA[t] = a0 * 128 + ((cb ^ ((a0 >> 1) & 3)) << 5) + (L & 3) * 8;
    }
#pragma unroll
    for (int c = 0; c < 4; ++c) offB[c] = NRp * 128 + rowl * 128 + ((c ^ ((rowl >> 1) & 3)) << 5) + (L & 3) * 8;
    const int hsup = (4 * g4 + (L >> 2)) % H;
    const bool red_m = hsup == 0;
    const bool red_p = hsup == H - 1;
    const unsigned zabs = lds0 + W9_ZOFF + (L & 3) * 8;
#pragma unroll
    for (int t = 0; t < 9; ++t) {
        const int dh = t % 3 - 1;
        if ((dh < 0 && red_m) || (dh > 0 && red_p)) offA[t] = lds0 + W9_ZOFF + (offA[t] & 255);
    }
    *(u32x4*)(smem + W9_ZOFF + tid * 16) = (u32x4){0, 0, 0, 0};
    const int hs = H == 2 ? 1 : (H == 4 ? 2 : (H == 8 ? 3 : 4));
    const int ncol = 32 >> hs;
    int wc = (kbeg >> hs) % W;
    const int lc0 = (4 * g4 + (L >> 2)) >> hs, lc1 = (4 * g4 + (L >> 2) + 16) >> hs;

    f32x4 acc[9][4];
#pragma unroll
    for (int t = 0; t < 9; ++t)
#pragma unroll
        for (int c = 0; c < 4; ++c) acc[t][c] = (f32x4){0.f, 0.f, 0.f, 0.f};
    float cs[8] = {0.f, 0.f, 0.f, 0.f, 0.f, 0.f, 0.f, 0.f};
    const unsigned offC = NRp * 128 + w9_cs_offset(tid);

#pragma unroll
    for (int p = 0; p < W9_NST - 1; ++p)
        if (p < nsteps) stage_load(p, p);
    int cur = 0;
    for (int step = 0; step < nsteps; ++step) {
        if (step + 1 < nsteps) asm volatile("s_waitcnt vmcnt(%0)" ::"n"(W9_NDMA) : "memory");
        else asm volatile("s_waitcnt vmcnt(0)" ::: "memory");
        __builtin_amdgcn_s_barrier();
        asm volatile("" ::: "memory");
        const unsigned sb = lds0 + cur * W9_STAGE;
        const unsigned sbm = red_m ? 0u : sb, sbp = red_p ? 0u : sb;

        s16x4 alo[W9_NSLOT], ahi[W9_NSLOT], blo[2][4], bhi[2][4];
        bool zl_m[2], zh_m[2], zl_p[2], zh_p[2];
#pragma unroll
        for (int kb = 0; kb < 2; ++kb) {
            int cbase = wc + ((kh * 64 + kb * 32) >> hs);
            while (cbase >= W) cbase -= W;
            const bool bd = cbase == 0 || cbase + ncol >= W;
            int c0 = cbase + lc0, c1 = cbase + lc1;
            if (c0 >= W) c0 -= W;
            if (c1 >= W) c1 -= W;
            zl_m[kb] = bd && c0 == 0; zh_m[kb] = bd && c1 == 0; zl_p[kb] = bd && c0 == W - 1; zh_p[kb] = bd && c1 == W - 1;
        }
        auto issue = [&](int P) __attribute__((always_inline)) {
            if (P == 0 || P == 10) {
                const int kb = P == 0 ? 0 : 1;
#pragma unroll
                for (int c = 0; c < 4; ++c) { w9_tr(blo[kb][c], sb + offB[c], kb * 32 * 128); w9_tr(bhi[kb][c], sb + offB[c], kb * 32 * 128 + 16 * 128); }
            } else {
                const int m = P < 10 ? P - 1 : P - 2, kb = m / 9, tt = m % 9;
                const unsigned sa = (tt % 3 == 0 ? sbm : (tt % 3 == 2 ? sbp : sb)) + offA[tt];
                unsigned sl = sa, sh = sa;
                if (tt / 3 == 0) { sl = zl_m[kb] ? zabs : sa; sh = zh_m[kb] ? zabs : sa; }
                if (tt / 3 == 2) { sl = zl_p[kb] ? zabs : sa; sh = zh_p[kb] ? zabs : sa; }
                w9_tr(alo[m % W9_NSLOT], sl, kb * 32 * 128); w9_tr(ahi[m % W9_NSLOT], sh, kb * 32 * 128 + 16 * 128);
            }
        };
#pragma unroll
        for (int P = 0; P < 20; ++P)
            if (P <= W9_TAB.upto[0]) issue(P);
#pragma unroll
        for (int n = 0; n < 18; ++n) {
            if (n == W9_DMA_AT) {
                if (step + 2 < nsteps) { int nb = cur + 2; if (nb >= W9_NST) nb -= W9_NST; stage_load(step + 2, nb); }
            }
            if (n > 0) {
#pragma unroll
                for (int P = 0; P < 20; ++P)
                    if (P > W9_TAB.upto[n - 1] && P <= W9_TAB.upto[n]) issue(P);
            }
            w9_wait(W9_TAB.wait[n]);
            __builtin_amdgcn_sched_barrier(0);
            w9_mfma_tap(acc[n % 9], alo[n % W9_NSLOT], ahi[n % W9_NSLOT], blo[n / 9], bhi[n / 9]);
            __builtin_amdgcn_sched_barrier(0);
        }
        if (do_cs) w9_cs_step(cs, sb + offC);
        wc += 128 >> hs;
        while (wc >= W) wc -= W;
        cur = (cur + 1 == W9_NST) ? 0 : cur + 1;
    }
    __syncthreads();

    if (do_cs) w9_cs_store(g, smem, cs, split, co0, tid);
    w9_store_tile(g, smem, acc, split, ci0, co0, cb, kh, lane);
}

__device__ long long* w9_dbg;
#ifdef OCR_EXPERIMENTS
#define W9P_PHASE(slot) do { if (w9_dbg && threadIdx.x == 0) w9_dbg[blockIdx.x * 8 + (slot)] = wall_clock64(); } while (0)
#else
#define W9P_PHASE(slot) do { } while (0)
#endif
constexpr int w9p_plane(int H, int kh, int kk, int dh, int half) {
    const int pl = H == 4 ? kh * 2 + kk + dh : kh * 4 + kk * 2 + half + dh;
    return pl >= 0 && pl < H ? pl : -1;
}
template <int H, bool GENW>
__global__ __launch_bounds__(512) void wgrad9p_kernel(W9Args g) {
    constexpr int NC = 128 / H;
    constexpr int PS = (NC + 2 + 7) / 8 * 8;
    constexpr int XROWS = H * PS, XPIECES = XROWS / 8;
    static_assert(XPIECES + 16 <= 8 * W9_NDMA, "a stage holds the planes and the dY tile");
    constexpr unsigned OOB = 0x80000000u;
    extern __shared__ __attribute__((aligned(16))) unsigned char smem[];
    const int tid = threadIdx.x, lane = tid & 63;
    W9P_PHASE(0);
    const unsigned lds0 = (unsigned)(size_t)(lptr_t)smem;
    const int wave = __builtin_amdgcn_readfirstlane(tid >> 6);
    const int cb = wave & 3, kh = wave >> 2;
    const int W = g.cW;
    int split, tile;
    w9_block_decode(g, split, tile);
    const int ti = tile / g.T_co, tj = tile % g.T_co;
    const int ci0 = ti * 64, co0 = tj * 64;
    const int kbeg = split * g.k_per_split;
    const int kend = min(g.M, kbeg + g.k_per_split);
    const int nsteps = kend > kbeg ? (kend - kbeg) >> 7 : 0;
    const bool do_cs = g.cs_part != nullptr && ti == 0;

    const int rr = lane >> 3, pp = lane & 7;
    const int qsrc = ((((pp >> 1) ^ ((rr >> 1) & 3)) << 1) | (pp & 1)) * 8;
    const __amdgpu_buffer_rsrc_t xsrd = __builtin_amdgcn_make_buffer_rsrc((void*)(g.X + ((long)kbeg - H) * g.Cin), 0,
                                                                          (int)(((long)g.M - kbeg + H) * g.Cin * 2), 0x00020000);
    const __amdgpu_buffer_rsrc_t ysrd = __builtin_amdgcn_make_buffer_rsrc((void*)(g.dY + (long)kbeg * g.Cout), 0,
                                                                          (int)(((long)g.M - kbeg) * g.Cout * 2), 0x00020000);
    constexpr int ZLO = NC + 4, ZHI = H == 4 ? NC + 4 - 16 : NC + 4;
    static_assert(NC + 2 <= ZLO && ZLO < PS, "a zero row exists behind the columns of every plane");
    unsigned voff[W9_NDMA], eL[W9_NDMA], eR[W9_NDMA];
#pragma unroll
    for (int i = 0; i < W9_NDMA; ++i) {
        const int u = wave + 8 * i;
        voff[i] = OOB; eL[i] = 0; eR[i] = 0;
        if (u < XPIECES) {
            const int r = 8 * u + rr, h = r / PS, cp = r % PS;
            if (cp < NC + 2) voff[i] = (unsigned)(((cp * H + h) * g.Cin + ci0 + qsrc) * 2);
            eL[i] = cp == 0 ? OOB : 0; eR[i] = cp == NC + 1 ? OOB : 0;
        } else if (u < XPIECES + 16) {
            const int r = 8 * (u - XPIECES) + rr, h = r / NC, col = r % NC;
            voff[i] = (unsigned)(((col * H + h) * g.Cout + co0 + qsrc) * 2);
        }
    }
    const int xstep = 128 * g.Cin * 2, ystep = 128 * g.Cout * 2;
    const int wc0 = (kbeg / H) % W;
    auto stage_load = [&](int step, int buf, int wcs ) {
        const unsigned selL = wcs == 0 ? OOB : 0u, selR = wcs + NC == W ? OOB : 0u;
#pragma unroll
        for (int i = 0; i < W9_NDMA; ++i) {
            const int u = wave + 8 * i;
            lptr_t dst = (lptr_t)(smem + buf * W9_STAGE + u * 1024);
            if (u < XPIECES) {
                const unsigned vo = voff[i] | (eL[i] & selL) | (eR[i] & selR);
                __builtin_amdgcn_raw_ptr_buffer_load_lds(xsrd, dst, 16, (int)vo, step * xstep, 0, 0);
            } else {
                __builtin_amdgcn_raw_ptr_buffer_load_lds(ysrd, dst, 16, (int)voff[i], step * ystep, 0, 0);
            }
        }
    };

    const int g4 = lane >> 4, L = lane & 15;
    unsigned baseA[3], zabs[3], offB[4];
#pragma unroll
    for (int d = 0; d < 3; ++d) {
        const int cp = 1 + 4 * g4 + (L >> 2) + (d - 1);
        baseA[d] = cp * 128 + ((cb ^ ((cp >> 1) & 3)) << 5) + (L & 3) * 8;
        zabs[d] = lds0 + W9_ZOFF + baseA[d];
    }
    const int clo = 4 * g4 + (L >> 2);
    const unsigned zlo0 = ZLO * 128 + (baseA[0] & 127), zlo2 = ZLO * 128 + (baseA[2] & 127);
    const unsigned zhi0 = ZHI * 128 + (baseA[0] & 127), zhi2 = ZHI * 128 + (baseA[2] & 127);
    const int rowl = kh * 64 + 4 * g4 + (L >> 2);
#pragma unroll
    for (int c = 0; c < 4; ++c) offB[c] = XROWS * 128 + rowl * 128 + ((c ^ ((rowl >> 1) & 3)) << 5) + (L & 3) * 8;
    *(u32x4*)(smem + W9_ZOFF + tid * 16) = (u32x4){0, 0, 0, 0};

    f32x4 acc[9][4];
#pragma unroll
    for (int t = 0; t < 9; ++t)
#pragma unroll
        for (int c = 0; c < 4; ++c) acc[t][c] = (f32x4){0.f, 0.f, 0.f, 0.f};
    float cs[8] = {0.f, 0.f, 0.f, 0.f, 0.f, 0.f, 0.f, 0.f};
    const unsigned offC = XROWS * 128 + w9_cs_offset(tid);

    int wcl = wc0;
    int wcc = wc0;
#pragma unroll
    for (int p = 0; p < W9_NST - 1; ++p)
        if (p < nsteps) { stage_load(p, p, wcl); wcl += NC; if (wcl >= W) wcl -= W; }

    auto run = [&](auto khc) {
        constexpr int KH = decltype(khc)::value;
        int cur = 0;
        for (int step = 0; step < nsteps; ++step) {
            if (step + 1 < nsteps) asm volatile("s_waitcnt vmcnt(%0)" ::"n"(W9_NDMA) : "memory");
            else asm volatile("s_waitcnt vmcnt(0)" ::: "memory");
            __builtin_amdgcn_s_barrier();
            asm volatile("" ::: "memory");
            const unsigned sb = lds0 + cur * W9_STAGE;
            unsigned sbA[3], sbAh[3], sbB[4];
#pragma unroll
            for (int d = 0; d < 3; ++d) { sbA[d] = sb + baseA[d]; sbAh[d] = sbA[d]; }
            if (GENW && W - wcc < NC) {
                const int bq = W - wcc, chi = clo + (H == 4 ? 16 : 0);
                if (clo == bq) sbA[0] = sb + zlo0;
                if (clo == bq - 1) sbA[2] = sb + zlo2;
                if (chi == bq) sbAh[0] = sb + zhi0;
                if (chi == bq - 1) sbAh[2] = sb + zhi2;
            }
#pragma unroll
            for (int c = 0; c < 4; ++c) sbB[c] = sb + offB[c];
            s16x4 alo[W9_NSLOT], ahi[W9_NSLOT], blo[2][4], bhi[2][4];
            auto issue = [&](auto pc) {
                constexpr int P = decltype(pc)::value;
                if constexpr (P == 0 || P == 10) {
                    constexpr int kb = P == 0 ? 0 : 1;
#pragma unroll
                    for (int c = 0; c < 4; ++c) { w9_tr(blo[kb][c], sbB[c], kb * 32 * 128); w9_tr(bhi[kb][c], sbB[c], kb * 32 * 128 + 16 * 128); }
                } else {
                    constexpr int m = P < 10 ? P - 1 : P - 2, kb = m / 9, tt = m % 9, dw = tt / 3, dh = tt % 3 - 1;
                    constexpr int pl = w9p_plane(H, KH, kb, dh, 0), ph = w9p_plane(H, KH, kb, dh, 1);
                    constexpr int il = pl >= 0 ? pl * PS * 128 : 0, ih = (ph >= 0 ? ph * PS * 128 : 0) + (H == 4 ? 16 * 128 : 0);
                    w9_tr(alo[m % W9_NSLOT], pl >= 0 ? sbA[dw] : zabs[dw], il);
                    w9_tr(ahi[m % W9_NSLOT], ph >= 0 ? sbAh[dw] : zabs[dw], ih);
                }
            };
            w9_for<0, 17>([&](auto nc) {
                constexpr int n = decltype(nc)::value, kk = n / 9, t = n % 9, dh = t % 3 - 1;
                if constexpr (n == W9_DMA_AT) {
                    if (step + 2 < nsteps) { int nb = cur + 2; if (nb >= W9_NST) nb -= W9_NST; stage_load(step + 2, nb, wcl); wcl += NC; if (wcl >= W) wcl -= W; }
                }
                if constexpr (n == 0) w9_for<0, W9_TAB.upto[0]>(issue);
                else w9_for<W9_TAB.upto[n > 0 ? n - 1 : 0] + 1, W9_TAB.upto[n]>(issue);
                w9_wait(W9_TAB.wait[n]);
                __builtin_amdgcn_sched_barrier(0);
                if constexpr (w9p_plane(H, KH, kk, dh, 0) >= 0 || w9p_plane(H, KH, kk, dh, 1) >= 0)
                    w9_mfma_tap(acc[t], alo[n % W9_NSLOT], ahi[n % W9_NSLOT], blo[kk], bhi[kk]);
                __builtin_amdgcn_sched_barrier(0);
            });
            if (do_cs) w9_cs_step(cs, sb + offC);
            cur = (cur + 1 == W9_NST) ? 0 : cur + 1;
            if (GENW) { wcc += NC; if (wcc >= W) wcc -= W; }
        }
    };
    if (kh == 0) run(std::integral_constant<int, 0>{}); else run(std::integral_constant<int, 1>{});
    __syncthreads();
    W9P_PHASE(1);

    if (do_cs) w9_cs_store(g, smem, cs, split, co0, tid);
    W9P_PHASE(2);
    w9_store_tile(g, smem, acc, split, ci0, co0, cb, kh, lane);
#ifdef OCR_EXPERIMENTS
    W9P_PHASE(3);
    asm volatile("s_waitcnt vmcnt(0)" ::: "memory");
    W9P_PHASE(4);
#endif
}

__device__ __forceinline__ void w9_reduce_body(float* __restrict__ dw, const float* __restrict__ part, long n4, long slab4, int S, int rows,
                                               float* __restrict__ dbias, const float* __restrict__ cs_part, int Cout, int blk) {
    __shared__ f32x4 red[256];
    const int cols = 256 / rows;
    const int col = threadIdx.x % cols, row = threadIdx.x / cols;
    const long i = (long)blk * cols + col;
    f32x4 a = {0.f, 0.f, 0.f, 0.f}, t = a;
    if (i < n4) {
        f32x4 b = {0.f, 0.f, 0.f, 0.f}, c = b, d = b;
        const f32x4* p = (const f32x4*)part + i;
        if (row == 0) t = ((const f32x4*)dw)[i];
        int s = row;
        for (; s + 3 * rows < S; s += 4 * rows) {
            a += __builtin_nontemporal_load(p + (long)s * slab4);              b += __builtin_nontemporal_load(p + (long)(s + rows) * slab4);
            c += __builtin_nontemporal_load(p + (long)(s + 2 * rows) * slab4); d += __builtin_nontemporal_load(p + (long)(s + 3 * rows) * slab4);
        }
        for (; s < S; s += rows) a += __builtin_nontemporal_load(p + (long)s * slab4);
        a = (a + b) + (c + d);
    }
    red[row * cols + col] = a;
    __syncthreads();
    if (row == 0 && i < n4) {
        for (int r = 0; r < rows; ++r) t += red[r * cols + col];
        ((f32x4*)dw)[i] = t;
    }
    if (dbias != nullptr && blk == 0)
        for (int c = threadIdx.x; c < Cout; c += blockDim.x) {
            float t = dbias[c];
            for (int s = 0; s < S; ++s) t += cs_part[(long)s * Cout + c];
            dbias[c] = t;
        }
}
__global__ __launch_bounds__(256) void wgrad9_reduce_kernel(float* __restrict__ dw, const float* __restrict__ part, long n4, long slab4,
                                                            int S, int rows, float* __restrict__ dbias, const float* __restrict__ cs_part, int Cout) {
    w9_reduce_body(dw, part, n4, slab4, S, rows, dbias, cs_part, Cout, blockIdx.x);
}
struct W9ReduceJob {
    float* dw; const float* part; float* dbias; const float* cs_part;
    long n4, slab4;
    int S, rows, Cout, block_start;
};
__global__ __launch_bounds__(256) void wgrad9_reduce_jobs_kernel(const W9ReduceJob* __restrict__ jobs, int njobs) {
    __shared__ int jsel[4];
    int j = 0;
    for (int k = threadIdx.x; k < njobs; k += 256)
        if (jobs[k].block_start <= (int)blockIdx.x) j = k;
#pragma unroll
    for (int off = 32; off > 0; off >>= 1) j = max(j, __shfl_xor(j, off));
    if ((threadIdx.x & 63) == 0) jsel[threadIdx.x >> 6] = j;
    __syncthreads();
    j = max(max(jsel[0], jsel[1]), max(jsel[2], jsel[3]));
    const W9ReduceJob jb = jobs[j];
    w9_reduce_body(jb.dw, jb.part, jb.n4, jb.slab4, jb.S, jb.rows, jb.dbias, jb.cs_part, jb.Cout, (int)blockIdx.x - jb.block_start);
}

struct W9Plan { int S, k_per_split, map, T_ci, T_co; size_t bytes; };

static bool w9_plan(int M, int W, int H, int Cin, int Cout, W9Plan* p) {
    if ((Cin & 63) || (Cout & 63) || (H != 2 && H != 4 && H != 8 && H != 16) || M < 512 || (M % H) || W * H < 32) return false;
    const int T_ci = Cin / 64, T_co = Cout / 64, T = T_ci * T_co;
    static int smax = -1;
    if (smax < 0) { const char* e = ocr_tune_env("OCR_W9_SMAX"); smax = e ? atoi(e) : 64; if (smax < 1) smax = 1; }
    int S = 1;
    while ((long)S * 2 * T <= 256 && S * 2 <= smax && M / (S * 2) >= 512) S *= 2;
    p->S = S; p->T_ci = T_ci; p->T_co = T_co;
    p->k_per_split = ceil_div(ceil_div(M, S), 128) * 128;
    p->map = S >= 8 ? 1 : ((T % (8 / S)) == 0 ? 2 : 0);
    p->bytes = (size_t)S * ((size_t)9 * Cin * Cout + Cout) * sizeof(float);
    return true;
}

extern "C" int ocr_wgrad9_debug(void* dbg ) {
    long long* q = (long long*)dbg;
    return hipMemcpyToSymbol(HIP_SYMBOL(w9_dbg), &q, sizeof(q)) == hipSuccess ? OCR_OK : OCR_ERR_MEMOPS;
}

extern "C" int ocr_conv3x3_wgrad_workspace_size(int Nb, int W, int H, int Cin, int Cout, size_t* bytes) {
    if (!bytes || Nb <= 0 || W <= 0 || H <= 0 || Cin <= 0 || Cout <= 0) return OCR_ERR_INVALID;
    W9Plan p;
    *bytes = w9_plan(Nb * W * H, W, H, Cin, Cout, &p) ? p.bytes : 0;
    return OCR_OK;
}

enum { W9K_WGRAD9 = 0, W9K_P4 = 1, W9K_P8 = 2, W9K_P4_ZERO_ROW = 3, W9K_P8_ZERO_ROW = 4 };
static int w9_choose(int M, int W, int H, int Cin, int Cout, W9Plan* p) {
    if (!w9_plan(M, W, H, Cin, Cout, p)) return -1;
    static int planes = -1;
    if (planes < 0) { const char* e = getenv("OCR_W9_PLANES"); planes = e ? atoi(e) : 1; }
    static int genw = -1;
    if (genw < 0) { const char* e = getenv("OCR_W9P_GENW"); genw = e ? atoi(e) : 1; }
    const bool whole = (H == 4 || H == 8) && W % (128 / H) == 0;
    const bool use_p = planes && (H == 4 || H == 8) && (whole || (genw && W >= 128 / H)) && M % 128 == 0 &&
                       (long)M * (Cin > Cout ? Cin : Cout) * 2 < 0x7fffffffL;
    if (!use_p) return W9K_WGRAD9;
    if (!whole || (genw == 2 && W >= 128 / H)) return H == 4 ? W9K_P4_ZERO_ROW : W9K_P8_ZERO_ROW;
    return H == 4 ? W9K_P4 : W9K_P8;
}
int wgrad9_choice(int Nb, int W, int H, int Cin, int Cout, int* S) {
    W9Plan p;
    const int k = w9_choose(Nb * W * H, W, H, Cin, Cout, &p);
    if (k >= 0) *S = p.S;
    return k;
}

template <auto KERNEL>
static int w9_launch(const W9Args& g, int grid, hipStream_t stream) {
    if (ocr_allow_lds<KERNEL>(W9_LDS) != hipSuccess) return OCR_ERR_EXEC;
    KERNEL<<<grid, 512, W9_LDS, stream>>>(g);
    return OCR_OK;
}

int wgrad9_try_dispatch(const void* x, const void* dy, float* dw, float* dbias, int Nb, int W, int H, int Cin, int Cout,
                        void* workspace, size_t ws_bytes, hipStream_t stream, void* defer_job, int* defer_blocks) {
    W9Plan p;
    const int M = Nb * W * H;
    if (!workspace) return -1;
    const int kern = w9_choose(M, W, H, Cin, Cout, &p);
    if (kern < 0 || ws_bytes < p.bytes) return -1;
    W9Args g = {};
    g.X = (const bf16_t*)x; g.dY = (const bf16_t*)dy; g.M = M; g.Cin = Cin; g.Cout = Cout; g.cW = W; g.cH = H;
    g.k_per_split = p.k_per_split; g.S = p.S; g.T_ci = p.T_ci; g.T_co = p.T_co; g.map = p.map;
    g.part = (float*)workspace;
    g.cs_part = dbias ? g.part + (size_t)p.S * 9 * Cin * Cout : nullptr;
    const int grid = p.S * p.T_ci * p.T_co;
    int rc;
    switch (kern) {
        case W9K_P4: rc = w9_launch<wgrad9p_kernel<4, false>>(g, grid, stream); break;
        case W9K_P8: rc = w9_launch<wgrad9p_kernel<8, false>>(g, grid, stream); break;
        case W9K_P4_ZERO_ROW: rc = w9_launch<wgrad9p_kernel<4, true>>(g, grid, stream); break;
        case W9K_P8_ZERO_ROW: rc = w9_launch<wgrad9p_kernel<8, true>>(g, grid, stream); break;
        default: rc = w9_launch<wgrad9_kernel>(g, grid, stream); break;
    }
    if (rc != OCR_OK) return rc;
    OCR_CHECK_LAUNCH();
    const long n4 = (long)9 * Cin * Cout / 4;
    int rows = p.S / 8;
    rows = rows < 1 ? 1 : (rows > 8 ? 8 : rows);
    while (rows & (rows - 1)) rows &= rows - 1;
    const int cols = 256 / rows;
    const int blocks = (int)((n4 + cols - 1) / cols);
    if (defer_job != nullptr) {
        W9ReduceJob jb = {dw, g.part, dbias, g.cs_part, n4, n4, p.S, rows, Cout, 0};
        *(W9ReduceJob*)defer_job = jb;
        *defer_blocks = blocks;
        return OCR_OK;
    }
    wgrad9_reduce_kernel<<<blocks, 256, 0, stream>>>(dw, g.part, n4, n4, p.S, rows, dbias, g.cs_part, Cout);
    OCR_CHECK_LAUNCH();
    return OCR_OK;
}

extern "C" int ocr_wgrad9_reduce_jobs(const void* jobs, int njobs, int total_blocks, void* stream) {
    static_assert(sizeof(W9ReduceJob) == 64, "W9ReduceJob is mirrored by engine.py");
    if (!jobs || njobs <= 0 || total_blocks <= 0) return OCR_ERR_INVALID;
    wgrad9_reduce_jobs_kernel<<<total_blocks, 256, 0, (hipStream_t)stream>>>((const W9ReduceJob*)jobs, njobs);
    OCR_CHECK_LAUNCH();
    return OCR_OK;
}
```

### lstm_ctc_ocr_amd/engine.py

```python
import time

import numpy as np
import torch

from . import dist as ocr_dist
from . import ops
from ._native import NativeError, call as nat_call
from .engine_ops import (BF16, F32, I32, _env, _number, _switch, _AddOp, _AvgPoolOp, _BatchNormOp, _BiLstmOp, _ConcatOp, _ConvOp,
                         _Conv3x3Op, _DropoutOp, _FcOp, _InputOp, _PoolOp, _ReluOp, _SoftmaxOp, _SubsampleOp, _ViewOp, _conv_op)
from .layout import FlatLayout, execution_order, init_host_parameters

ALIGN = 64





class ShapePlan(object):

    def _init_fields(self, N, W):
        self.N, self.W = N, W
        self.buf, self.shape = {}, {}
        self.scratch = {}
        self.dy_done = set()
        self.w9_pending, self.w9_tables = [], {}
        self.w9_pending_bytes = 0
        self.tn_pending = []
        self.tn_side_open = False
        self.fused_pools = set()
        self.bn_stat_rows = {}
        self.bn_bwd_rows = {}
        self.unpool_pools = set()
        self.col_bn = {}
        self.lstm_sync_keys = ()
        self.lstm_arena, self.lstm_sync = None, ()
        self.rings_ready, self.rings_armed = set(), False
        self.graph_fb = self.graph_fwd = self.graph_fb1 = self.graph_fb2 = self.graph_dp = self.graph_step = None
        self._guard_addrs = None
        self._report = None

    def __init__(self, eng, N, W):
        self._init_fields(N, W)
        dev = eng.device
        self.x = torch.zeros((N, W, eng.num_features), dtype=F32, device=dev)
        self.labels = torch.zeros(N * eng.max_label_len, dtype=I32, device=dev)
        self.labels_len = torch.zeros(N, dtype=I32, device=dev)
        self.seq_len = torch.ones(N, dtype=I32, device=dev)
        self.oshape = {'data': (N, W, eng.num_features)}
        for op in eng.ops:
            s = self.oshape[op.prev.key]
            op.alloc(self, s)
            self.oshape[op.key] = op.out_shape(s)
        keys = self.lstm_sync_keys
        if keys:
            self.lstm_arena = torch.zeros(sum(self.buf[k].numel() for k in keys), dtype=I32, device=dev)
            off = 0
            for k in keys:
                n = self.buf[k].numel()
                self.buf[k] = self.lstm_arena[off:off + n]
                off += n
        self.lstm_sync = tuple(self.buf[k] for k in keys)
        own = [k for k in self.buf if k.endswith('/w9ws')]
        if own and sum(self.buf[k].numel() for k in own) > eng.w9_defer_max_bytes and not eng.w9_flush_bytes:
            need = max(self.buf[k].numel() for k in own)
            for k in own:
                del self.buf[k]
            self.buf['wgrad_ws'] = torch.empty(need, dtype=torch.uint8, device=dev)
        self.T, _, self.C = self.oshape[eng.ops[-1].key]
        self.costs = torch.zeros(N, dtype=F32, device=dev)
        self.ctc_grad = torch.empty((self.T, N, self.C), dtype=F32, device=dev)
        ws_bytes = ops.ctc_workspace_bytes(eng.max_label_len, self.T, N) if eng.max_label_len <= 127 else 1
        if eng.ctc_path_of(self.C, self.T) == 'long':
            ws_bytes = max(ws_bytes, ops.ctc_long_workspace_bytes(self.C, eng.max_label_len, self.T, N))
        self.ctc_ws = torch.empty(ws_bytes, dtype=torch.uint8, device=dev)
        self.decoded = torch.zeros((N, self.T), dtype=I32, device=dev)
        self.decoded_len = torch.zeros(N, dtype=I32, device=dev)


class Engine(object):

    def __init__(self, net, device='cuda:0', seed=None, max_label_len=31, use_graphs=True, group=None,
                 persistent_lstm=True, fuse_conv1_pool=True, ctc_long=True):
        from .config import cfg
        if max_label_len > self.CTC_MAX_LABEL_LEN:
            raise ValueError('max_label_len = %d: the CTC loss covers labels of at most %d characters' % (max_label_len, self.CTC_MAX_LABEL_LEN))
        if not torch.cuda.is_available():
            raise NativeError('Engine needs a ROCm GPU: the hot path has no CPU implementation')
        self.cfg = cfg
        self.net = net
        self.device = torch.device(device)
        torch.cuda.set_device(self.device)
        self.num_features = cfg.NUM_FEATURES
        self.max_label_len = max_label_len
        self.ctc_long = ctc_long
        self.use_graphs = use_graphs
        self.persistent_lstm = persistent_lstm
        self.fuse_conv1_pool = fuse_conv1_pool
        self.fuse_bn_stats = _switch('OCR_FUSE_BN_STATS')
        self.w9_flush_bytes = int(_number('OCR_W9_FLUSH_MB', 80, float) * (1 << 20))
        self.tn_defer = _switch('OCR_TN_JOBS')
        self.tn_side = _switch('OCR_TN_SIDE', False)
        self.side_stream = torch.cuda.Stream(device=self.device) if (self.tn_side and torch.device(self.device).type == 'cuda') else None
        self.group = group
        self.world = 1
        self._check_xcd_placement()
        self.force_allreduce = bool(_env('OCR_FORCE_ALLREDUCE'))
        if group is not None or (torch.distributed.is_available() and torch.distributed.is_initialized()):
            self.world = torch.distributed.get_world_size(group)
        if _env('OCR_FAKE_WORLD'):
            self.world = _number('OCR_FAKE_WORLD', None)
            self.force_allreduce = True
        self.overlap_allreduce = _switch('OCR_OVERLAP_ALLREDUCE')
        self.dp_graph = _env('OCR_DP_GRAPH', '0') == '1'
        self.defer_w9 = _switch('OCR_W9_DEFER')
        self.w9_defer_max_bytes = _number('OCR_W9_DEFER_MAX_MB', self.W9_DEFER_MAX_BYTES >> 20) << 20
        self.w9_ws_pool = {}
        self.comm_stream = torch.cuda.Stream(device=self.device)
        self.dp_host_s = [0.0, 0.0, 0.0, 0.0, 0.0, 0]
        self._pack_table = None
        self._fault_hook = None
        self._watch_pending = None
        self.dropped_reports = 0
        self._lower(net)
        self._layout(net)
        self._init_params(cfg.RNG_SEED if seed is None else seed)
        self.split_op = 0
        if self.split_layer is not None:
            for i, op in enumerate(self.ops):
                if op.name == self.split_layer:
                    self.split_op = i
                    break
            for i, op in enumerate(self.ops):
                for name, owner in self._owner.items():
                    if owner == op.name:
                        assert (self.offsets[name] >= self.late_begin) == (i >= self.split_op), (op.name, name)
        self.plans = {}
        if self.dp_graph and (self.world > 1 or self.force_allreduce):
            self.dp_graph = self._check_graph_collectives()
        self.training = False
        self.train_keep_prob = 0.5
        self.scalars = torch.zeros(ops.optim_scalar_count(), dtype=torch.float64, device=self.device)
        self.opt_ready = False
        self.graph_opt = None
        self.iteration = 0
        self.refresh_weights()
        staged = getattr(net, '_staged_arrays', None)
        if staged:
            self.load_arrays(staged)

    _xcd_checked = False

    def _check_xcd_placement(self):
        if Engine._xcd_checked:
            return
        Engine._xcd_checked = True
        n = 256
        out = torch.zeros(2 * n, dtype=torch.int32, device=self.device)
        nat_call('ocr_probe_xcc', out.data_ptr(), n, 64, torch.cuda.current_stream(self.device).cuda_stream)
        xcc = out[:n].cpu().numpy()
        colocated = all(len(set(xcc[r::8].tolist())) == 1 for r in range(8))
        if not colocated:
            nat_call('ocr_set_lstm_proto', 0)

    def _layout(self, net):
        lay = FlatLayout(net.param_specs.values(), ALIGN, order=[op.name for op in self.ops])
        self._owner = lay.owner
        self.specs, self.offsets, self.n_total = lay.specs, lay.offsets, lay.n_total
        self.split_layer, self.reg_range, self.late_begin = lay.split_layer, lay.reg_range, lay.late_begin
        dev = self.device
        self.params = torch.zeros(self.n_total, dtype=F32, device=dev)
        self._grads_store = torch.zeros(self.n_total + self.GUARD_PAD, dtype=F32, device=dev)
        self.grads = self._grads_store[:self.n_total]
        self.drop_flag = self._grads_store[self.n_total:self.n_total + 1]
        self.params_bf16 = torch.zeros(self.n_total, dtype=BF16, device=dev)

    GUARD_PAD = 64

    def offset(self, name):
        return self.offsets[name]

    def _view(self, flat, name):
        s = self.specs[name]
        n = int(np.prod(s.shape))
        o = self.offsets[name]
        return flat[o:o + n].view(s.shape)

    def param(self, name):
        return self._view(self.params, name)

    def grad(self, name):
        return self._view(self.grads, name)

    def shadow(self, name):
        return self._view(self.params_bf16, name)

    def _init_params(self, seed):
        self.params.copy_(init_host_parameters(self.specs, self.offsets, self.n_total, seed))

    def load_arrays(self, arrays):
        for name, arr in arrays.items():
            t = torch.as_tensor(np.asarray(arr, np.float32))
            if tuple(t.shape) != tuple(self.specs[name].shape):
                raise ValueError('%s: shape %s does not match %s' % (name, tuple(t.shape), self.specs[name].shape))
            self.param(name).copy_(t)
        self.refresh_weights()

    def state_arrays(self):
        return {name: self.param(name).detach().cpu().numpy().copy() for name in self.specs}

    PACK_DTYPE = np.dtype([('type', '<i4'), ('R', '<i4'), ('Cc', '<i4'), ('lstm_units', '<i4'), ('ldin', '<i8'),
                           ('ldout', '<i8'), ('src', '<u8'), ('dst', '<u8'), ('n', '<i8'), ('block_start', '<i4'),
                           ('nblocks', '<i4')])

    def _build_pack_table(self):
        jobs = []
        for op in self.ops:
            for name in op.shadow_params():
                n = int(np.prod(self.specs[name].shape))
                assert n % 4 == 0, name
                jobs.append(dict(type=3, src=self._view(self.params, name).reshape(-1), dst=self._view(self.params_bf16, name).reshape(-1), n=n))
        for op in self.ops:
            jobs.extend(op.pack_jobs())
        tab = np.zeros(len(jobs), self.PACK_DTYPE)
        start = 0
        for i, j in enumerate(jobs):
            t = j['type']
            if t == 0:
                nb = ((j['Cc'] + 63) // 64) * ((j['R'] + 63) // 64)
            elif t == 1:
                nb = min((j['n'] + 255) // 256, 512)
            elif t == 2:
                nb = min((j['R'] * j['Cc'] // 4 + 255) // 256, 512)
            elif t == 4:
                nb = min((j['n'] + 255) // 256, 512)
            else:
                nb = min((j['n'] // 4 + 255) // 256, 2048)
            tab[i] = (t, j.get('R', 0), j.get('Cc', 0), j.get('lstm_units', 0), j.get('ldin', 0), j.get('ldout', 0),
                      j['src'].data_ptr(), j['dst'].data_ptr(), j.get('n', 0), start, nb)
            start += nb
        assert tab.itemsize == 64
        self._pack_table = torch.from_numpy(tab.view(np.uint8).copy()).to(self.device)
        self._pack_njobs, self._pack_blocks = len(jobs), start

    def refresh_weights(self):
        if self._pack_table is None:
            self._build_pack_table()
        ops.pack_jobs(self._pack_table, self._pack_njobs, self._pack_blocks)
        for op in self.ops:
            op.refresh()

    def _lower(self, net):
        table = {'conv': _conv_op, 'fc': _FcOp, 'max_pool': _PoolOp, 'reshape_squeeze': _ViewOp, 'dropout': _DropoutOp, 'bi_lstm': _BiLstmOp, 'lstm': _BiLstmOp,
                 'add': _AddOp, 'relu': _ReluOp, 'batch_norm': _BatchNormOp, 'avg_pool': _AvgPoolOp, 'concat': _ConcatOp,
                 'softmax': _SoftmaxOp}
        data_op = _InputOp(self)
        built = {}
        self.ops = []
        for nd in execution_order(net.get_output('logits')):
            if nd.op not in table:
                raise NotImplementedError('layer %r (%s) has no gfx950 lowering yet' % (nd.op, nd.name))
            ins = [data_op if i.op == 'input' else built[id(i)] for i in (nd.inputs if nd.op in ('add', 'concat') else nd.inputs[:1])]
            op = table[nd.op](self, nd, ins[0])
            op.inputs = ins
            op.key = '%02d:%s' % (len(self.ops), nd.name)
            for i in ins:
                i.grad_owner().consumers += 1
            self.ops.append(op)
            if nd.op == 'conv' and (nd.attrs['s_h'], nd.attrs['s_w']) != (1, 1):
                if nd.attrs['bn']:
                    raise NotImplementedError('%s: a strided convolution with batch norm is not lowered' % nd.name)
                sub = _SubsampleOp(self, nd, op)
                sub.name = nd.name + '/stride'
                sub.inputs, sub.key = [op], '%02d:%s/stride' % (len(self.ops), nd.name)
                op.consumers += 1
                self.ops.append(sub)
                op = sub
            built[id(nd)] = op
        if _switch('OCR_FUSE_ADD_RELU'):
            for r in self.ops:
                a = r.prev
                if isinstance(r, _ReluOp) and isinstance(a, _AddOp) and a.consumers == 1:
                    a.relu, r.fused_into = True, a
                    a.consumers = r.consumers
                    for p in a.inputs:
                        if (isinstance(p, _ConvOp) and p.bn and not p.relu and p.consumers == 1 and p.kind != 'c1'
                                and a.inputs.count(p) == 1):
                            p.mask_from = a
                    cands = [p for p in a.inputs if getattr(p, 'mask_from', None) is a]
                    if cands and len(a.inputs) == 2:
                        p = max(cands, key=lambda q: self.ops.index(q))
                        other = a.inputs[1] if a.inputs[0] is p else a.inputs[0]
                        if isinstance(other, _InputOp) or self.ops.index(other) < self.ops.index(p):
                            p.tail_into, a.fwd_by = (a, other), p
        if _switch('OCR_FUSE_CONV_POOL'):
            for b in self.ops:
                a = b.prev
                if (isinstance(b, _PoolOp) and isinstance(a, _Conv3x3Op) and a.relu and not a.bn and a.biased
                        and a.consumers == 1 and (b.kw_t, b.kh_f) in ((1, 2), (2, 2))):
                    a.pool_after = b
        if _switch('OCR_FUSE_BN_POOL'):
            for b in self.ops:
                a = b.prev
                if (isinstance(b, _PoolOp) and isinstance(a, _ConvOp) and a.bn and a.kind != 'c1' and a.consumers == 1
                        and a.tail_into is None and a.mask_from is None and (b.kw_t, b.kh_f) == (1, 2)):
                    a.bn_pool, b.bn_fused_into = b, a
        if self.fuse_conv1_pool:
            for a, b in zip(self.ops[:-1], self.ops[1:]):
                if (isinstance(a, _ConvOp) and a.kind == 'c1' and a.relu and isinstance(b, _PoolOp) and b.prev is a
                        and a.consumers == 1 and (b.kw_t, b.kh_f) == (2, 2)):
                    a.fused_pool, b.fused_into = b, a

    def _scratch(self, sp, like):
        key = (tuple(like.shape), like.dtype)
        if key not in sp.scratch:
            sp.scratch[key] = torch.empty_like(like)
        return sp.scratch[key]

    def grad_dst(self, sp, producer):
        d = producer.dy(sp)
        if d is None:
            return None, (lambda: None)
        owner = producer.grad_owner()
        if owner.consumers <= 1 or owner.key not in sp.dy_done:
            sp.dy_done.add(owner.key)
            return d, (lambda: None)
        tmp = self._scratch(sp, d)
        return tmp, (lambda: ops.eltwise(0, d, tmp, d))

    def grad_dst_acc(self, sp, producer, can_accumulate):
        d = producer.dy(sp)
        if d is None:
            return None, (lambda: None), False
        owner = producer.grad_owner()
        first = owner.consumers <= 1 or owner.key not in sp.dy_done
        if first or not can_accumulate:
            dst, finish = self.grad_dst(sp, producer)
            return dst, finish, False
        return d, (lambda: None), True

    def deliver(self, sp, producer, grad, mask=None):
        d = producer.dy(sp)
        if d is None:
            return
        g = grad.view(d.shape)
        if mask is None and producer.mask_in_consumer:
            mask = producer.y(sp)
        owner = producer.grad_owner()
        first = owner.consumers <= 1 or owner.key not in sp.dy_done
        sp.dy_done.add(owner.key)
        if first:
            if mask is None:
                d.copy_(g)
            else:
                ops.eltwise(2, g, mask.view(d.shape), d)
        elif mask is None:
            ops.eltwise(0, d, g, d)
        else:
            ops.eltwise(4, g, mask.view(d.shape), d)

    def plan(self, N, W):
        key = (N, W)
        if key not in self.plans:
            self.plans[key] = ShapePlan(self, N, W)
        return self.plans[key]

    def _bind(self, sp, data, seq_len, labels=None, labels_len=None):
        def as_i32(v):
            return v if torch.is_tensor(v) else torch.as_tensor(np.asarray(v, np.int32))
        sl = as_i32(seq_len)
        lab = ll = None
        if labels is not None:
            lab, ll = as_i32(labels), as_i32(labels_len)
            if lab.numel() > sp.labels.numel():
                raise ValueError('flat label vector longer than batch * max_label_len (%d)' % sp.labels.numel())
        ints = [t for t in (sl, lab, ll) if t is not None]
        if (torch.is_tensor(data) and data.is_cuda and data.dtype in (torch.uint8, F32) and data.is_contiguous()
                and data.numel() == sp.x.numel() and all(t.is_cuda and t.dtype == I32 and t.is_contiguous() for t in ints)
                and sl.numel() == sp.seq_len.numel() and (ll is None or ll.numel() == sp.labels_len.numel())):
            ops.bind_batch(data, sp.x, sl, sp.seq_len, lab, sp.labels, ll, sp.labels_len)
            return
        if torch.is_tensor(data) and data.dtype == torch.uint8:
            ops.u8_to_unit_f32(data if data.is_cuda else data.to(self.device, non_blocking=True), sp.x)
            dsts, srcs = [sp.seq_len], [sl]
        else:
            x = torch.as_tensor(np.asarray(data, np.float32)) if not torch.is_tensor(data) else data
            dsts, srcs = [sp.x, sp.seq_len], [x, sl]
        if lab is not None:
            dsts += [sp.labels[:lab.numel()], sp.labels_len]
            srcs += [lab, ll]
        for d, t in zip(dsts, srcs):
            d.copy_(t, non_blocking=True)

    def step_counter(self):
        return self.scalars[6:7]

    def _forward(self, sp, training=False):
        self.training = training
        self._zero_pending = bool(training) and self.grads.numel() % 4 == 0 and _switch('OCR_FUSE_ZERO')
        if training and not self._zero_pending:
            self.grads.zero_()
        sp.rings_ready, sp.rings_armed = set(), False
        self._ones_pending = sp.lstm_arena if (training and sp.lstm_arena is not None and _switch('OCR_FUSE_RINGFILL')) else None
        for op in self.ops:
            op.fwd(sp)
        self._ones_pending = None
        if self._zero_pending:
            self.grads.zero_()
            self._zero_pending = False

    def _loss_and_backward(self, sp, flush=True):
        sp.dy_done = set()
        sp.w9_pending = []
        sp.tn_pending = []
        logits = self.ops[-1].y(sp)
        scale = ocr_dist.loss_scale(sp.N, self.world)
        path = self.ctc_path_of(sp.C, sp.T)
        if path == 'fast':
            ops.ctc_loss_train(logits, self.ops[-1].dy(sp), scale, sp.labels, sp.labels_len, sp.seq_len, self.max_label_len,
                               sp.costs, blank=0)
        elif path == 'long':
            ops.ctc_loss_long(logits, sp.labels, sp.labels_len, sp.seq_len, self.max_label_len, blank=0, want_grad=False,
                              grad_ntc_bf16=self.ops[-1].dy(sp), scale=scale, workspace=sp.ctc_ws, costs=sp.costs)
        else:
            ops.ctc_loss(logits, sp.labels, sp.labels_len, sp.seq_len, self.max_label_len, blank=0, want_grad=True,
                         workspace=sp.ctc_ws, costs=sp.costs, grads=sp.ctc_grad)
            ops.tnc_to_ntc_bf16(sp.ctc_grad, self.ops[-1].dy(sp), scale)
        for op in reversed(self.ops[self.split_op:]):
            op.bwd(sp)
        self._flush_tn(sp)
        self._join_tn(sp)
        if flush:
            self._flush_w9(sp)

    CTC_MAX_LABEL_LEN = 255

    def ctc_path_of(self, C, T):
        if ops.ctc_train_supported(C, T, self.max_label_len):
            return 'fast'
        if self.ctc_long and ops.ctc_long_supported(C, T, self.max_label_len):
            return 'long'
        return 'general'

    def ctc_path(self, N, W):
        sp = self.plan(N, W)
        return self.ctc_path_of(sp.C, sp.T)

    def _backward_early(self, sp):
        for op in reversed(self.ops[:self.split_op]):
            op.bwd(sp)
        self._flush_tn(sp)
        self._join_tn(sp)
        self._flush_w9(sp)

    def tn_push(self, sp, job, keep, fallback):
        if not self.tn_defer or not ops.gemm_tn_jobs_supported([job]):
            fallback()
            return
        sp.tn_pending.append((job, keep, fallback))
        if len(sp.tn_pending) == 2:
            self._flush_tn(sp)

    def _flush_tn(self, sp):
        pend, sp.tn_pending = sp.tn_pending, []
        if len(pend) == 2:
            if self.tn_side:
                main = torch.cuda.current_stream(self.device)
                self.side_stream.wait_stream(main)
                with torch.cuda.stream(self.side_stream):
                    ops.gemm_tn_jobs([pend[0][0], pend[1][0]])
                sp.tn_side_open = True
            else:
                ops.gemm_tn_jobs([pend[0][0], pend[1][0]])
        else:
            for _, _, fallback in pend:
                fallback()

    def _join_tn(self, sp):
        if sp.tn_side_open:
            torch.cuda.current_stream(self.device).wait_stream(self.side_stream)
            sp.tn_side_open = False

    W9_DEFER_MAX_BYTES = 192 << 20
    W9_JOB_DTYPE = np.dtype([('dw', '<u8'), ('part', '<u8'), ('dbias', '<u8'), ('cs_part', '<u8'), ('n4', '<i8'), ('slab4', '<i8'),
                             ('S', '<i4'), ('rows', '<i4'), ('Cout', '<i4'), ('block_start', '<i4')])

    def _flush_w9(self, sp):
        pend, sp.w9_pending = sp.w9_pending, []
        sp.w9_pending_bytes = 0
        if not pend:
            return
        raw = b''.join(job for job, _ in pend)
        ent = sp.w9_tables.get(raw)
        if ent is None:
            tab = np.frombuffer(raw, dtype=self.W9_JOB_DTYPE).copy()
            assert tab.itemsize == 64 and len(tab) == len(pend)
            start = 0
            for i, (_, nblk) in enumerate(pend):
                tab['block_start'][i] = start
                start += nblk
            dev = torch.from_numpy(tab.view(np.uint8).copy()).to(self.device)
            ent = sp.w9_tables[raw] = (dev, len(pend), start)
        ops.wgrad9_reduce_jobs(*ent)

    def _capture(self, fn):
        import gc
        gc.collect()
        torch.cuda.synchronize()
        g = torch.cuda.CUDAGraph()
        was = gc.isenabled()
        gc.disable()
        try:
            with torch.cuda.graph(g, capture_error_mode='thread_local'):
                fn()
        finally:
            if was:
                gc.enable()
        return g

    def _run_split(self, sp):
        def body1():
            self._forward(sp, training=True)
            self._loss_and_backward(sp)
            self._publish_guard(sp)

        def body2():
            self._backward_early(sp)

        if not self.use_graphs:
            body1()
            return body2
        if sp.graph_fb1 is None:
            body1(); body2()
            sp.graph_fb1, sp.graph_fb2 = self._capture(body1), self._capture(body2)
        sp.graph_fb1.replay()
        return sp.graph_fb2.replay

    def _check_graph_collectives(self):
        import torch.distributed as dist
        fake = bool(_env('OCR_FAKE_WORLD'))
        if not fake:
            if not (dist.is_available() and dist.is_initialized()) or dist.get_backend(self.group) != 'nccl':
                return False
        ok = True
        try:
            t = torch.ones(256, dtype=F32, device=self.device)
            main = torch.cuda.current_stream(self.device)
            self.comm_stream.wait_stream(main)
            with torch.cuda.stream(self.comm_stream):
                ocr_dist.allreduce_sum_(t, self.group, force=self.force_allreduce)
            main.wait_stream(self.comm_stream)
            torch.cuda.synchronize()

            def body():
                cur = torch.cuda.current_stream(self.device)
                self.comm_stream.wait_stream(cur)
                with torch.cuda.stream(self.comm_stream):
                    ocr_dist.allreduce_sum_(t, self.group, force=self.force_allreduce)
                cur.wait_stream(self.comm_stream)
            g = self._capture(body)
            t.fill_(1.0)
            g.replay(); g.replay()
            torch.cuda.synchronize()
            w = float(self.world if (fake or self.world > 1) else 1)
            ok = bool(float(t[0]) == w * w and float(t[-1]) == w * w)
        except Exception as e:
            import sys
            sys.stderr.write('[engine] OCR_DP_GRAPH=1: a captured collective failed on this group (%s: %s) — three-graph schedule instead\n' % (type(e).__name__, e))
            ok = False
        if not fake and dist.get_world_size(self.group) > 1:
            v = torch.tensor([1.0 if ok else 0.0], device=self.device)
            dist.all_reduce(v, op=dist.ReduceOp.MIN, group=self.group)
            ok = bool(float(v[0]) == 1.0)
        return ok

    def _run_dp_graph(self, sp):
        if not self.opt_ready:
            self.setup_optimizer()

        def exchange(lo, hi):
            cur = torch.cuda.current_stream(self.device)
            self.comm_stream.wait_stream(cur)
            with torch.cuda.stream(self.comm_stream):
                self.allreduce_grads(lo, hi)

        def body():
            self._forward(sp, training=True)
            self._loss_and_backward(sp)
            self._publish_guard(sp)
            exchange(self.late_begin, self.n_total)
            self._backward_early(sp)
            exchange(0, self.late_begin)
            torch.cuda.current_stream(self.device).wait_stream(self.comm_stream)
            self._optim_body(None)

        if sp.graph_dp is None:
            self._guard_addrs(sp)
            self._forward(sp, training=True)
            self._loss_and_backward(sp)
            self._backward_early(sp)
            sp.graph_dp = self._capture(body)
        sp.graph_dp.replay()

    def _run_step(self, sp):
        if not self.opt_ready:
            self.setup_optimizer()

        def fb():
            self._forward(sp, training=True)
            self._loss_and_backward(sp, flush=False)
            self._backward_early(sp)

        if sp.graph_step is None:
            self._guard(sp)
            fb()

            def body():
                fb()
                self._optim_body(sp)
            sp.graph_step = self._capture(body)
        sp.graph_step.replay()

    def _run(self, sp, which):
        attr = 'graph_fb' if which == 'fb' else 'graph_fwd'

        def body():
            self._forward(sp, training=(which == 'fb'))
            if which == 'fb':
                self._loss_and_backward(sp, flush=False)
                self._backward_early(sp)
                self._publish_guard(sp)

        if not self.use_graphs:
            body()
            return
        g = getattr(sp, attr)
        if g is None:
            body()
            g = self._capture(body)
            setattr(sp, attr, g)
# ... 205 lines not shown
```

### lstm_ctc_ocr_amd/engine_ops.py

```python
import os

import numpy as np
import torch

from . import ops

BF16, F32, I32 = torch.bfloat16, torch.float32, torch.int32
BN_EPS = 1e-3


def _env(name, default=None):
    return os.environ.get(name, default)


def _switch(name, default=True):
    return _env(name, '1' if default else '0') != '0'


def _number(name, default, kind=int):
    return kind(_env(name, default))


def _take_ring(sp, key):
    if key not in sp.rings_ready:
# ... 141 lines not shown
            add, other = self.tail_into
            y, res, relu = add.y(sp), other.y(sp).view(M, self.co), True
        pooled = self.bn_pool.y(sp).view(M // 2, self.co) if self.bn_pool is not None else None
        ops.bn_train_fwd(sp.buf[self.key + '/z'].view(M, self.co), e.param('%s/%s/gamma' % (self.name, self.name)),
                         e.param('%s/%s/beta' % (self.name, self.name)), BN_EPS, relu,
                         sp.buf[self.key + '/bnws'], out=None if y is None else y.view(M, self.co),
                         save_mean=sp.buf[self.key + '/mean'], save_rstd=sp.buf[self.key + '/rstd'], residual=res,
                         partial_rows=sp.bn_stat_rows[self.key], pooled=pooled, codes=codes)

    def _bn_bwd(self, sp):
        e, o = self.eng, sp.shape[self.key][1]
        M = o[0] * o[1] * o[2]
        dy, dz = self.dy(sp), sp.buf[self.key + '/dz']
        codes = sp.buf.get(self.key + '/pool_codes')
        ymask, relu = (self.y(sp) if codes is None else None), self.relu
        if self.mask_from is not None:
            dy, ymask, relu = self.mask_from.dy(sp), self.mask_from.y(sp), True
        dy2 = dy.view(M, self.co)
        if self.bn_pool is not None:
            dy2 = self.bn_pool.dy(sp).view(M // 2, self.co)
        colsrc = sp.col_bn.get(self.key)
        if colsrc is not None:
            col, Nb, W, HC = colsrc
            ops.bn_train_bwd_codes_col(sp.buf[self.key + '/z'].view(M, self.co), codes, col, Nb, W, HC, dy2,
                                       e.param('%s/%s/gamma' % (self.name, self.name)), sp.buf[self.key + '/mean'],
                                       sp.buf[self.key + '/rstd'], e.grad('%s/%s/gamma' % (self.name, self.name)),
                                       e.grad('%s/%s/beta' % (self.name, self.name)), relu, sp.buf[self.key + '/bnws'], out=dz.view(M, self.co))
            return dz
        ops.bn_train_bwd(sp.buf[self.key + '/z'].view(M, self.co), None if ymask is None else ymask.view(M, self.co), dy2,
                         e.param('%s/%s/gamma' % (self.name, self.name)), sp.buf[self.key + '/mean'],
                         sp.buf[self.key + '/rstd'], e.grad('%s/%s/gamma' % (self.name, self.name)),
                         e.grad('%s/%s/beta' % (self.name, self.name)), relu, sp.buf[self.key + '/bnws'],
                         out=dz.view(M, self.co), pooled_dy=self.bn_pool is not None,
                         partial_rows=sp.bn_bwd_rows.get(self.key, 0), codes=codes)
        return dz


class _Conv1Op(_ConvOp):
    kind = 'c1'

    def __init__(self, eng, node, prev):
        super(_Conv1Op, self).__init__(eng, node, prev)
        if (self.kh, self.kw, self.padding) != (3, 3, 'SAME') or self.co != 64 or self.bn or not self.biased:
            raise NotImplementedError('%s: the single-channel input conv is lowered for 3x3 SAME, 64 filters' % self.name)

    def pack_jobs(self):
        return []

    def alloc(self, sp, s):
        if self.fused_pool is None:
            return super(_Conv1Op, self).alloc(sp, s)
        dev = self.eng.device
        sp.shape[self.key] = (s, self.out_shape(s))
        if self.eng.defer_w9 and _switch('OCR_CONV1_SLAB'):
            sp.buf[self.key + '/slab'] = torch.empty((ops.conv1_pool_bwd_slab_rows(s[0], s[1], s[2]), 640), dtype=F32, device=dev)
        if _switch('OCR_CONV1_CODES'):
            sp.buf[self.key + '/codes'] = torch.empty((s[0] * (s[1] // 2) * (s[2] // 2), 8), dtype=torch.int32, device=dev)

    def _conv_fwd(self, sp, x, out, bias, codes):
        ops.conv1_fwd(x, self.eng.param(self.name + '/weights'), bias, relu=self.relu, out=out)

    def _conv_bwd(self, sp, x, dz, dw, db):
        ops.conv1_wgrad(x, dz, dw, db)

    def fwd(self, sp):
        if self.fused_pool is None:
            return super(_Conv1Op, self).fwd(sp)
        e = self.eng
        zero, e._zero_pending = (e.grads if e._zero_pending else None), False
        codes = sp.buf.get(self.key + '/codes') if e.training else None
        ones, e._ones_pending = e._ones_pending, None
        ops.conv1_pool_fwd(self.prev.y(sp), e.param(self.name + '/weights'), e.param(self.name + '/biases'), out=self.fused_pool.y(sp),
                           zero=zero, codes=codes, ones=ones)
        sp.rings_ready = set(sp.lstm_sync_keys) if ones is not None else set()
        sp.rings_armed = ones is not None

    def bwd(self, sp):
        if self.fused_pool is None:
            return super(_Conv1Op, self).bwd(sp)
        e = self.eng
        x, w, b, dp = self.prev.y(sp), e.param(self.name + '/weights'), e.param(self.name + '/biases'), self.fused_pool.dy(sp)
        codes = sp.buf.get(self.key + '/codes')
        slab = sp.buf.get(self.key + '/slab')
        if slab is None:
            ops.conv1_pool_bwd(x, w, b, dp, e.grad(self.name + '/weights'), e.grad(self.name + '/biases'), codes=codes)
            return
        ops.conv1_pool_bwd_slab(x, w, b, dp, slab, codes=codes)
        for dst, off, n4 in ((e.grad(self.name + '/weights'), 0, 144), (e.grad(self.name + '/biases'), 576, 16)):
            job = np.zeros(1, dtype=e.W9_JOB_DTYPE)
            job['dw'], job['part'], job['n4'], job['slab4'] = dst.data_ptr(), slab.data_ptr() + 4 * off, n4, 160
            job['S'], job['rows'], job['Cout'] = slab.shape[0], 8, 64
            sp.w9_pending.append((job.tobytes(), (n4 + 31) // 32))


class _Conv3x3Op(_ConvOp):
    kind = '3x3'

    def __init__(self, eng, node, prev):
        super(_Conv3x3Op, self).__init__(eng, node, prev)
        if self.ci % 32 or self.co % 8:
            raise NotImplementedError('%s: 3x3 conv needs C_in %% 32 == 0 and C_out %% 8 == 0' % self.name)
        self.wpack = torch.empty((self.co, 9 * self.ci), dtype=BF16, device=eng.device)
        if prev.dy_needed():
            self.wdgrad = torch.empty((self.ci, 9 * self.co), dtype=BF16, device=eng.device)

    def pack_jobs(self):
        jobs = super(_Conv3x3Op, self).pack_jobs()
        if hasattr(self, 'wdgrad'):
            w = self.eng.param(self.name + '/weights')
            jobs.append(dict(type=1, R=self.ci, Cc=self.co, src=w, dst=self.wdgrad, n=w.numel()))
        return jobs

    def _code_windows(self, sp, s, o):
        p = self.pool_after
        if (p is not None and p.key in sp.fused_pools
                and ops.conv3x3_pool_codes_supported(s[0], s[1], s[2], self.ci, self.co, p.kw_t, p.kh_f)):
            return o[0] * (o[1] // p.kw_t) * (o[2] // p.kh_f)
        return super(_Conv3x3Op, self)._code_windows(sp, s, o)

    def _stats_rows(self, sp, s):
        if not self.eng.fuse_bn_stats:
            return 0
        rows = ops.conv3x3_stats_rows(s[0], s[1], s[2], self.ci, self.co, bias=self.biased)
        return rows if rows * 2 * self.co * 4 <= sp.buf[self.key + '/bnws'].numel() - 2 * self.co * 8 else 0

    def alloc(self, sp, s):
        e, dev, p = self.eng, self.eng.device, self.pool_after
        if p is not None and ops.conv3x3_pool_supported(s[0], s[1], s[2], self.ci, self.co, p.kw_t, p.kh_f):
            sp.fused_pools.add(p.key)
        super(_Conv3x3Op, self).alloc(sp, s)
        p = self.prev
        if hasattr(self, 'wdgrad') and e.fuse_bn_stats and _switch('OCR_FUSE_BN_BWD') and _bnbwd_rows_allowed(p):
            rows = ops.conv3x3_bnbwd_rows(s[0], s[1], s[2], self.co, self.ci)
            sp.bn_bwd_rows[p.key] = rows if rows * 2 * self.ci * 4 <= sp.buf[p.key + '/bnws'].numel() - 2 * self.ci * 8 else 0
        if (hasattr(self, 'wdgrad') and _switch('OCR_FUSE_UNPOOL') and isinstance(p, _PoolOp) and p.consumers == 1
                and getattr(p.prev, 'pool_after', None) is p and p.key in sp.fused_pools and p.prev.key + '/pool_codes' in sp.buf
                and ops.conv3x3_unpool_supported(s[0], s[1], s[2], self.co, self.ci, p.kw_t, p.kh_f)
                and ops.conv3x3_kernel_choice(s[0], s[1], s[2], self.co, self.ci, bias=False, relu=False) in ('conv_k3/A', 'conv_k3/D')):
            sp.unpool_pools.add(p.key)
            del sp.buf[p.key + '/dy']
        need = ops.conv3x3_wgrad_workspace_bytes(s[0], s[1], s[2], self.ci, self.co)
        have = sp.buf.get('wgrad_ws')
        if need and e.defer_w9:
            pool = e.w9_ws_pool
            have_ws = pool.get(self.key)
            if have_ws is None or have_ws.numel() < need:
                wmax = max(_number('OCR_MAX_WIDTH', 320), sp.W)
                scale = max(1, wmax // sp.W + (1 if wmax % sp.W else 0))
                big = need
                if scale > 1:
                    big = max(need, ops.conv3x3_wgrad_workspace_bytes(s[0], s[1] * scale, s[2], self.ci, self.co))
                have_ws = pool[self.key] = torch.empty(big, dtype=torch.uint8, device=dev)
            sp.buf[self.key + '/w9ws'] = have_ws[:need]
        elif need and (have is None or have.numel() < need):
            sp.buf['wgrad_ws'] = torch.empty(need, dtype=torch.uint8, device=dev)

    def _conv_fwd(self, sp, x, out, bias, codes):
        w, p = self.wpack.view(self.co, 3, 3, self.ci), self.pool_after
        if p is not None and p.key in sp.fused_pools:
            if codes is not None:
                ops.conv3x3_relu_pool_codes(x, w, None, p.y(sp), codes, bias, p.kw_t, p.kh_f)
            else:
                ops.conv3x3_relu_pool(x, w, out, p.y(sp), bias, p.kw_t, p.kh_f)
        elif self.bn and sp.bn_stat_rows[self.key]:
            ops.conv3x3_stats(x, w, out, sp.buf[self.key + '/bnws'], bias=bias)
        else:
            ops.conv3x3(x, w, out=out, bias=bias, relu=self.mask_in_consumer)

    def _conv_bwd(self, sp, x, dz, dw, db):
        e, o, p = self.eng, sp.shape[self.key][1], self.prev
        own_ws = sp.buf.get(self.key + '/w9ws')
        if own_ws is not None:
            job, nblk = ops.conv3x3_wgrad_deferred(x, dz, dw, db, own_ws)
            if job is not None:
                sp.w9_pending.append((job, nblk))
                sp.w9_pending_bytes += own_ws.numel()
                if e.w9_flush_bytes and sp.w9_pending_bytes >= e.w9_flush_bytes:
                    e._flush_w9(sp)
        else:
            ops.conv3x3_wgrad(x, dz, dw, dbias=db, workspace=sp.buf.get('wgrad_ws'))
        if p.key in sp.unpool_pools:
            pdy, finish = e.grad_dst(sp, p.prev)
            if pdy is not None:
                ops.conv3x3_dgrad_unpool(dz, self.wdgrad.view(self.ci, 3, 3, self.co), sp.buf[p.prev.key + '/pool_codes'], p.kw_t, p.kh_f,
                                         p.prev.mask_in_consumer, out=pdy)
                finish()
            return
        pdy, finish, acc = e.grad_dst_acc(sp, p, ops.conv3x3_accum_supported(o[0], o[1], o[2], self.co, self.ci))
        if pdy is not None:
            wd = self.wdgrad.view(self.ci, 3, 3, self.co)
            if sp.bn_bwd_rows.get(p.key, 0) and not acc:
                ops.conv3x3_dgrad_bnbwd(dz, wd, pdy, p.y(sp), sp.buf[p.key + '/z'], sp.buf[p.key + '/mean'], sp.buf[p.key + '/rstd'],
                                        sp.buf[p.key + '/bnws'])
            else:
                ops.conv3x3(dz, wd, out=pdy, mask=x if p.mask_in_consumer else None, accumulate=acc)
            finish()


class _Conv1x1Op(_ConvOp):
    kind = '1x1'

    def __init__(self, eng, node, prev):
        super(_Conv1x1Op, self).__init__(eng, node, prev)
        if self.ci % 8 or self.co % 8:
            raise NotImplementedError('%s: 1x1 conv needs C_in %% 8 == 0 and C_out %% 8 == 0' % self.name)
        self.wpack = torch.empty((self.co, self.ci), dtype=BF16, device=eng.device)

    def shadow_params(self):
        return [self.name + '/weights']

    def _conv_fwd(self, sp, x, out, bias, codes):
        s = sp.shape[self.key][0]
        M = s[0] * s[1] * s[2]
        ops.gemm_nt(x.view(M, self.ci), self.wpack, out=out.view(M, self.co), bias=bias, relu=self.mask_in_consumer)

    def _conv_bwd(self, sp, x, dz, dw, db):
        e, o = self.eng, sp.shape[self.key][1]
        M = o[0] * o[1] * o[2]
        pdy, finish = e.grad_dst(sp, self.prev)
        ops.gemm_tn(x.view(M, self.ci), dz.view(M, self.co), dw.view(self.ci, self.co), colsum=db)
        if pdy is not None:
            wsh = e.shadow(self.name + '/weights').view(self.ci, self.co)
            ops.gemm_nt(dz.view(M, self.co), wsh, out=pdy.view(M, self.ci),
                        mask=x.view(M, self.ci) if self.prev.mask_in_consumer else None)
            finish()


class _ConvFullOp(_ConvOp):
    kind = 'full'

    def __init__(self, eng, node, prev):
        super(_ConvFullOp, self).__init__(eng, node, prev)
        self.wpack = torch.empty((self.co, self.kh * self.kw * self.ci), dtype=BF16, device=eng.device)

    def shadow_params(self):
        return [self.name + '/weights']

    def out_shape(self, s):
        N, W, H = s[0], s[1], s[2]
        if self.kw != H:
            raise NotImplementedError('%s: VALID conv is lowered only when k_w equals the feature-axis size '
                                      '(got k_w=%d, H=%d)' % (self.name, self.kw, H))
        return (N, W - self.kh + 1, 1, self.co)

    def alloc(self, sp, s):
        super(_ConvFullOp, self).alloc(sp, s)
        N, W, H, C = s
        sp.buf[self.key + '/col'] = torch.empty((N * (W - self.kh + 1), self.kh * H * C), dtype=BF16, device=self.eng.device)
        p = self.prev
        bn = getattr(p, 'bn_fused_into', None)
        if (_switch('OCR_FUSE_COL2IM_BN', False) and isinstance(p, _PoolOp) and bn is not None and p.consumers == 1 and self.kh == 2
                and not p.mask_in_consumer and bn.key + '/pool_codes' in sp.buf and (H * C) % 8 == 0):
            sp.col_bn[bn.key] = (sp.buf[self.key + '/col'], N, W, H * C)

    def _conv_fwd(self, sp, x, out, bias, codes):
        (N, W, H, C), o = sp.shape[self.key]
        Wo = o[1]
        ops.gemm_nt(x, self.wpack, out=out.view(N * Wo, self.co), M=N * Wo, N=self.co, K=self.kh * H * C,
                    ldp=H * C, ldq=self.kh * H * C, bias=bias, relu=self.mask_in_consumer, row_group=Wo, row_skip=self.kh - 1)

    def _conv_bwd(self, sp, x, dz, dw, db):
        e, ((N, W, H, C), o) = self.eng, sp.shape[self.key]
        Wo, M, K = o[1], o[0] * o[1] * o[2], self.kh * H * C
        pdy, finish = e.grad_dst(sp, self.prev)
        dz2, dw2 = dz.view(M, self.co), dw.view(K, self.co)
        e.tn_push(sp, ops.tn_job(x, H * C, dz2, self.co, dw2, self.co, M, K, self.co, row_group=Wo, row_skip=self.kh - 1, colsum=db),
                  (x, dz2, dw2, db),
                  lambda: ops.gemm_tn(x, dz2, dw2, Mk=M, I=K, J=self.co, lda=H * C, ldb=self.co,
                                      ldo=self.co, row_group=Wo, row_skip=self.kh - 1, colsum=db))
        if pdy is not None:
            if self.prev.mask_in_consumer or self.kh != 2:
                raise NotImplementedError('%s: data gradient of a full-height VALID conv is lowered for k_h = 2 '
                                          'behind a non-ReLU producer' % self.name)
            col = sp.buf[self.key + '/col']
            wsh = e.shadow(self.name + '/weights').view(K, self.co)
            ops.gemm_nt(dz2, wsh, out=col, M=M, N=K, K=self.co)
            bn = getattr(self.prev, 'bn_fused_into', None)
            if bn is None or bn.key not in sp.col_bn:
                ops.conv5_col2im(col, pdy, N, W, H * C)
            finish()


def _conv_op(eng, node, prev):
    a = node.attrs
    if a['c_i'] == 1:
        cls = _Conv1Op
    elif (a['k_h'], a['k_w'], a['padding']) == (3, 3, 'SAME'):
        cls = _Conv3x3Op
    elif (a['k_h'], a['k_w']) == (1, 1):
        cls = _Conv1x1Op
    elif a['padding'] == 'VALID':
        cls = _ConvFullOp
    else:
        raise NotImplementedError('%s: %dx%d %s convolution is not lowered' % (node.name, a['k_h'], a['k_w'], a['padding']))
    return cls(eng, node, prev)


class _FcOp(_Conv1x1Op):

    def out_shape(self, s):
        return tuple(s[:-1]) + (self.co,)

    def alloc(self, sp, s):
        o = self.out_shape(s)
        rows = int(np.prod(s[:-1]))
        sp.shape[self.key] = ((rows, 1, 1, s[-1]), (rows, 1, 1, self.co))
        sp.buf[self.key + '/y'] = torch.empty(o, dtype=BF16, device=self.eng.device)
        sp.buf[self.key + '/dy'] = torch.empty(o, dtype=BF16, device=self.eng.device)


class _PoolOp(_Op):
    def __init__(self, eng, node, prev):
        super(_PoolOp, self).__init__(eng, node, prev)
        a = node.attrs
        self.kw_t, self.kh_f = a['k_h'], a['k_w']
        if (a['s_h'], a['s_w']) != (a['k_h'], a['k_w']) or self.kw_t not in (1, 2) or self.kh_f not in (1, 2):
            raise NotImplementedError('%s: max-pool is lowered for window == stride in {1,2}' % self.name)

    def dy_needed(self):
        return True

    def out_shape(self, s):
        N, W, H, C = s
        if W % self.kw_t or H % self.kh_f:
            raise NotImplementedError('%s: pooled axes must divide evenly (W=%d, H=%d)' % (self.name, W, H))
        return (N, W // self.kw_t, H // self.kh_f, C)

    def alloc(self, sp, s):
        o = self.out_shape(s)
        sp.shape[self.key] = (s, o)
        sp.buf[self.key + '/y'] = torch.empty(o, dtype=BF16, device=self.eng.device)
# ... 487 lines not shown
```

### lstm_ctc_ocr_amd/ops.py

```python
import ctypes

import torch

from . import _native as nat
from ._native import EPI_ACCUM, EPI_BIAS, EPI_MASK, EPI_OUT_F32, EPI_RELU, EPI_ROWSWAP, call, ptr

BF16 = torch.bfloat16
F32 = torch.float32


def _st():
    return nat.stream()


def _dev(t):
    if not t.is_cuda:
        raise nat.NativeError("hot-path operators take device tensors only (got a CPU tensor)")
    return t


def ctc_workspace_bytes(max_label_len, max_time, minibatch):
    sz = ctypes.c_size_t(0)
    call("ocr_ctc_workspace_size", max_label_len, max_time, minibatch, ctypes.byref(sz))
    return sz.value
# ... 129 lines not shown

def conv3x3(x, wpack, out=None, *, bias=None, relu=False, mask=None, accumulate=False):
    Nb, W, H, Cin = x.shape
    Cout = wpack.shape[0]
    if out is None:
        assert not accumulate
        out = torch.empty((Nb, W, H, Cout), dtype=BF16, device=x.device)
    flags = ((EPI_BIAS if bias is not None else 0) | (EPI_RELU if relu else 0) | (EPI_MASK if mask is not None else 0) |
             (EPI_ACCUM if accumulate else 0))
    call("ocr_conv3x3_bf16", ptr(_dev(x)), ptr(wpack), ptr(out), Nb, W, H, Cin, Cout, ptr(bias), ptr(mask), flags, _st())
    return out


def conv3x3_pool_supported(Nb, W, H, Cin, Cout, kw, kh):
    return bool(nat.lib().ocr_conv3x3_pool_supported(Nb, W, H, Cin, Cout, kw, kh))


def conv3x3_relu_pool(x, wpack, out, pooled, bias, kw, kh):
    Nb, W, H, Cin = x.shape
    call("ocr_conv3x3_relu_pool_bf16", ptr(_dev(x)), ptr(wpack), ptr(out), ptr(pooled), Nb, W, H, Cin, wpack.shape[0], ptr(bias),
         kw, kh, _st())
    return out, pooled


def conv3x3_pool_codes_supported(Nb, W, H, Cin, Cout, kw, kh):
    return bool(nat.lib().ocr_conv3x3_pool_codes_supported(Nb, W, H, Cin, Cout, kw, kh))


def conv3x3_relu_pool_codes(x, wpack, out, pooled, codes, bias, kw, kh):
    Nb, W, H, Cin = x.shape
    Cout = wpack.shape[0]
    assert codes.dtype == torch.int32 and codes.numel() == Nb * (W // kw) * (H // kh) * (Cout // 8), (codes.dtype, tuple(codes.shape))
    call("ocr_conv3x3_relu_pool_codes_bf16", ptr(_dev(x)), ptr(wpack), ptr(out), ptr(pooled), ptr(codes), Nb, W, H, Cin, Cout, ptr(bias),
         kw, kh, _st())
    return out, pooled, codes


def conv3x3_unpool_supported(Nb, W, H, Cin, Cout, kw, kh):
    return bool(nat.lib().ocr_conv3x3_unpool_supported(int(Nb), int(W), int(H), int(Cin), int(Cout), int(kw), int(kh)))


def conv3x3_dgrad_unpool(dy, wdgrad, codes, kw, kh, relu_mask, out=None):
    Nb, W, H, Cin = dy.shape
    Cout = wdgrad.shape[0]
    assert codes.dtype == torch.int32 and codes.numel() == Nb * W * H * (Cout // 8), (codes.dtype, tuple(codes.shape))
    if out is None:
        out = torch.empty((Nb, W * kw, H * kh, Cout), dtype=BF16, device=dy.device)
    assert out.numel() == Nb * W * kw * H * kh * Cout
    call("ocr_conv3x3_dgrad_unpool_bf16", ptr(_dev(dy)), ptr(wdgrad), ptr(out), ptr(codes), Nb, W, H, Cin, Cout, kw, kh, int(relu_mask),
         _st())
    return out


def gemm_tn(A, B, out, *, Mk=None, I=None, J=None, lda=None, ldb=None, ldo=None, row_group=0, row_skip=0,
            a_row_off=0, scale=1.0, splits=0, colsum=None):
    Mk = B.shape[0] if Mk is None else Mk
    I = A.shape[1] if I is None else I
    J = B.shape[1] if J is None else J
    lda = A.stride(0) if lda is None else lda
    ldb = B.stride(0) if ldb is None else ldb
    ldo = out.stride(0) if ldo is None else ldo
    call("ocr_gemm_tn_bf16", ptr(_dev(A)), lda, ptr(B), ldb, ptr(out), ldo, Mk, I, J, row_group, row_skip, a_row_off,
         float(scale), splits, ptr(colsum), _st())
    return out


def gemm_tn_split_workspace(Mk, I, J):
    n = nat.lib().ocr_gemm_tn_split_workspace_floats(int(Mk), int(I), int(J))
    if n < 0:
        raise nat.NativeError("ocr_gemm_tn_split_workspace_floats: invalid shape (%d, %d, %d)" % (Mk, I, J))
    return int(n)


def gemm_tn_split(A, B, out, ws, *, colsum=None, scale=1.0):
    Mk, I, J = B.shape[0], A.shape[1], B.shape[1]
    call("ocr_gemm_tn_split_bf16", ptr(_dev(A)), A.stride(0), ptr(B), B.stride(0), ptr(out), out.stride(0), Mk, I, J, float(scale),
         ptr(colsum), ptr(ws), ws.numel(), _st())
    return out


def gemm_tn_batched(A, lda, strideA, B, ldb, strideB, out, ldo, strideOut, Mk, I, J, nbatch, colsum=None, strideColsum=0,
                    scale=1.0, splits=0):
    call("ocr_gemm_tn_batched_bf16", ptr(_dev(A)), lda, strideA, ptr(B), ldb, strideB, ptr(out), ldo, strideOut, Mk, I, J, nbatch,
         float(scale), splits, ptr(colsum), strideColsum, _st())
    return out


class TnJob(ctypes.Structure):
    _fields_ = [("A", ctypes.c_void_p), ("lda", ctypes.c_long), ("strideA", ctypes.c_long),
                ("B", ctypes.c_void_p), ("ldb", ctypes.c_long), ("strideB", ctypes.c_long),
                ("out", ctypes.c_void_p), ("ldo", ctypes.c_long), ("strideOut", ctypes.c_long),
                ("colsum", ctypes.c_void_p), ("strideColsum", ctypes.c_long),
                ("Mk", ctypes.c_int), ("I", ctypes.c_int), ("J", ctypes.c_int), ("nbatch", ctypes.c_int),
                ("row_group", ctypes.c_int), ("row_skip", ctypes.c_int), ("scale", ctypes.c_float), ("reserved", ctypes.c_int)]


def tn_job(A, lda, B, ldb, out, ldo, Mk, I, J, *, nbatch=1, strideA=0, strideB=0, strideOut=0, colsum=None, strideColsum=0, row_group=0,
           row_skip=0, scale=1.0):
    return TnJob(ptr(_dev(A)), lda, strideA, ptr(_dev(B)), ldb, strideB, ptr(out), ldo, strideOut, ptr(colsum), strideColsum,
                 Mk, I, J, nbatch, row_group, row_skip, float(scale), 0)


def gemm_tn_jobs_supported(jobs):
    arr = (TnJob * len(jobs))(*jobs)
    return bool(nat.lib().ocr_gemm_tn_jobs_supported(ctypes.cast(arr, ctypes.c_void_p), len(jobs)))


def gemm_tn_jobs(jobs):
    arr = (TnJob * len(jobs))(*jobs)
    call("ocr_gemm_tn_jobs_bf16", ctypes.cast(arr, ctypes.c_void_p), len(jobs), _st())


def lstm_xh(x2d, hout, seq_len, xh, Nb, T, D, U, ndir=2):
    call("ocr_lstm_xh", ptr(_dev(x2d)), ptr(hout), ptr(seq_len), ptr(xh), Nb, T, D, U, ndir, _st())
    return xh


def conv3x3_wgrad_workspace_bytes(Nb, W, H, Cin, Cout):
    sz = ctypes.c_size_t(0)
    call("ocr_conv3x3_wgrad_workspace_size", Nb, W, H, Cin, Cout, ctypes.byref(sz))
    return sz.value


WGRAD_KERNEL_NAMES = ("wgrad9", "wgrad9p<4>", "wgrad9p<8>", "wgrad9p<4>/zero-row", "wgrad9p<8>/zero-row", "gemm_tn2/nine-tap",
                      "gemm_tn2/paired-tap", "gemm_tn<1,4,4>", "gemm_tn<1,2,2>")


def conv3x3_wgrad_kernel_choice(Nb, W, H, Cin, Cout, *, workspace=True, splits=0):
    rc = nat.lib().ocr_conv3x3_wgrad_kernel_choice(int(Nb), int(W), int(H), int(Cin), int(Cout), int(bool(workspace)), int(splits))
    if rc < 0:
        raise nat.NativeError("ocr_conv3x3_wgrad_kernel_choice failed: status %d (%s)" % (-rc, nat.status_string(-rc)))
    return WGRAD_KERNEL_NAMES[rc & 255], rc >> 8


def conv3x3_wgrad(x, dy, dw, splits=0, dbias=None, workspace=None):
    Nb, W, H, Cin = x.shape
    Cout = dy.shape[-1]
    if workspace is not None:
        call("ocr_conv3x3_wgrad_ws_bf16", ptr(_dev(x)), ptr(dy), ptr(dw), ptr(dbias), Nb, W, H, Cin, Cout, splits,
             ptr(workspace), workspace.numel(), _st())
    else:
        call("ocr_conv3x3_wgrad_bf16", ptr(_dev(x)), ptr(dy), ptr(dw), ptr(dbias), Nb, W, H, Cin, Cout, splits, _st())
    return dw


def conv3x3_wgrad_deferred(x, dy, dw, dbias, workspace):
    Nb, W, H, Cin = x.shape
    Cout = dy.shape[-1]
    job = (ctypes.c_ubyte * 64)()
    nblk, deferred = ctypes.c_int(0), ctypes.c_int(0)
    call("ocr_conv3x3_wgrad_defer_bf16", ptr(_dev(x)), ptr(dy), ptr(dw), ptr(dbias), Nb, W, H, Cin, Cout, ptr(workspace),
         workspace.numel(), ctypes.cast(job, ctypes.c_void_p), ctypes.byref(nblk), ctypes.byref(deferred), _st())
    return (bytes(job), nblk.value) if deferred.value else (None, 0)


def wgrad9_reduce_jobs(table, njobs, total_blocks):
    call("ocr_wgrad9_reduce_jobs", ptr(_dev(table)), njobs, total_blocks, _st())


def conv1_fwd(x, w, bias, relu=True, out=None):
    Nb, W, H = x.shape
    Cout = w.shape[-1]
    if out is None:
        out = torch.empty((Nb, W, H, Cout), dtype=BF16, device=x.device)
    call("ocr_conv1_fwd", ptr(_dev(x)), ptr(w), ptr(bias), ptr(out), Nb, W, H, Cout, int(relu), _st())
    return out


def conv1_wgrad(x, dz, dw, db):
    Nb, W, H = x.shape
    call("ocr_conv1_wgrad", ptr(_dev(x)), ptr(dz), ptr(dw), ptr(db), Nb, W, H, dz.shape[-1], _st())


def eltwise(op, a, b, out):
    call("ocr_eltwise_bf16", op, ptr(_dev(a)), ptr(b), ptr(out), a.numel(), _st())
    return out


def conv1_pool_fwd(x, w, bias, out=None, zero=None, codes=None, ones=None):
    Nb, W, H = x.shape
    Cout = w.shape[-1]
    if out is None:
        out = torch.empty((Nb, W // 2, H // 2, Cout), dtype=BF16, device=x.device)
    if zero is not None or codes is not None or ones is not None:
        call("ocr_conv1_pool_fwd_train", ptr(_dev(x)), ptr(w), ptr(bias), ptr(out), Nb, W, H, Cout, ptr(codes),
             ptr(_dev(zero)) if zero is not None else None, 0 if zero is None else zero.numel(),
             ptr(_dev(ones)) if ones is not None else None, 0 if ones is None else ones.numel(), _st())
    else:
        call("ocr_conv1_pool_fwd", ptr(_dev(x)), ptr(w), ptr(bias), ptr(out), Nb, W, H, Cout, _st())
    return out


def conv1_pool_bwd(x, w, bias, dp, dw, db, codes=None):
    Nb, W, H = x.shape
    if codes is not None:
        call("ocr_conv1_pool_bwd_codes", ptr(_dev(x)), ptr(w), ptr(bias), ptr(dp), ptr(dw), ptr(db), Nb, W, H, w.shape[-1], ptr(codes), _st())
    else:
        call("ocr_conv1_pool_bwd", ptr(_dev(x)), ptr(w), ptr(bias), ptr(dp), ptr(dw), ptr(db), Nb, W, H, w.shape[-1], _st())


def conv1_pool_bwd_slab_rows(Nb, W, H):
    return int(nat.lib().ocr_conv1_pool_bwd_slab_rows(int(Nb), int(W), int(H)))


def conv1_pool_bwd_slab(x, w, bias, dp, slab, codes=None):
    Nb, W, H = x.shape
    assert slab.dtype == torch.float32 and tuple(slab.shape) == (conv1_pool_bwd_slab_rows(Nb, W, H), 640)
    call("ocr_conv1_pool_bwd_slab", ptr(_dev(x)), ptr(w), ptr(bias), ptr(dp), Nb, W, H, w.shape[-1], ptr(codes), ptr(slab), _st())


def maxpool_fwd(x, kw, kh, out=None):
    Nb, W, H, C = x.shape
    if out is None:
        out = torch.empty((Nb, W // kw, H // kh, C), dtype=BF16, device=x.device)
    call("ocr_maxpool_fwd", ptr(_dev(x)), ptr(out), Nb, W, H, C, kw, kh, _st())
    return out


def maxpool_bwd(x, dy, kw, kh, relu_mask, out=None):
    Nb, W, H, C = x.shape
    if out is None:
        out = torch.empty_like(x)
    call("ocr_maxpool_bwd", ptr(_dev(x)), ptr(dy), ptr(out), Nb, W, H, C, kw, kh, int(relu_mask), _st())
    return out


def maxpool_bwd_codes(codes, dy, kw, kh, relu_mask, out=None):
    Nb, Wo, Ho, C = dy.shape
    W, H = Wo * kw, Ho * kh
    assert codes.dtype == torch.int32 and codes.numel() == Nb * Wo * Ho * (C // 8), (codes.dtype, tuple(codes.shape))
    if out is None:
        out = torch.empty((Nb, W, H, C), dtype=BF16, device=dy.device)
    call("ocr_maxpool_bwd_codes", ptr(_dev(codes)), ptr(dy), ptr(out), Nb, W, H, C, kw, kh, int(relu_mask), _st())
    return out


def bn_workspace(M, C, device):
    return torch.empty(int(nat.lib().ocr_bn_workspace_bytes(int(M), int(C))), dtype=torch.uint8, device=device)


def bn_train_fwd(x2d, gamma, beta, eps, relu, workspace, out=None, save_mean=None, save_rstd=None, residual=None, partial_rows=0,
                 pooled=None, codes=None):
    M, C = x2d.shape
    if codes is not None:
        assert pooled is not None and residual is None and out is None
        assert codes.dtype == torch.int32 and tuple(codes.shape) == (M // 2, C // 8), (codes.dtype, tuple(codes.shape))
        if save_mean is None: save_mean = torch.empty(C, dtype=F32, device=x2d.device)
        if save_rstd is None: save_rstd = torch.empty(C, dtype=F32, device=x2d.device)
        call("ocr_bn_train_fwd_codes", ptr(_dev(x2d)), ptr(gamma), ptr(beta), ptr(save_mean), ptr(save_rstd), M, C,
             float(eps), int(relu), ptr(workspace), int(partial_rows), ptr(pooled), ptr(codes), _st())
        return None, save_mean, save_rstd
    if out is None: out = torch.empty_like(x2d)
    if save_mean is None: save_mean = torch.empty(C, dtype=F32, device=x2d.device)
    if save_rstd is None: save_rstd = torch.empty(C, dtype=F32, device=x2d.device)
    if partial_rows or pooled is not None:
        call("ocr_bn_train_fwd2", ptr(_dev(x2d)), ptr(out), ptr(gamma), ptr(beta), ptr(save_mean), ptr(save_rstd), M, C,
             float(eps), int(relu), ptr(workspace), ptr(residual), int(partial_rows), ptr(pooled), _st())
    else:
        call("ocr_bn_train_fwd", ptr(_dev(x2d)), ptr(out), ptr(gamma), ptr(beta), ptr(save_mean), ptr(save_rstd), M, C,
             float(eps), int(relu), ptr(workspace), ptr(residual), _st())
    return out, save_mean, save_rstd


def bn_train_bwd(x2d, y2d, dy2d, gamma, save_mean, save_rstd, dgamma, dbeta, relu, workspace, out=None, pooled_dy=False, partial_rows=0,
                 codes=None):
    M, C = x2d.shape
    if out is None: out = torch.empty_like(x2d)
    if codes is not None:
        assert pooled_dy and not partial_rows and tuple(dy2d.shape) == (M // 2, C)
        assert codes.dtype == torch.int32 and tuple(codes.shape) == (M // 2, C // 8), (codes.dtype, tuple(codes.shape))
        call("ocr_bn_train_bwd_codes", ptr(_dev(x2d)), ptr(codes), ptr(dy2d), ptr(out), ptr(gamma), ptr(save_mean), ptr(save_rstd),
             ptr(dgamma), ptr(dbeta), M, C, int(relu), ptr(workspace), _st())
        return out
    if pooled_dy or partial_rows:
        assert tuple(dy2d.shape) == ((M // 2, C) if pooled_dy else (M, C))
        call("ocr_bn_train_bwd2", ptr(_dev(x2d)), ptr(y2d), ptr(dy2d), ptr(out), ptr(gamma), ptr(save_mean), ptr(save_rstd),
             ptr(dgamma), ptr(dbeta), M, C, int(relu), ptr(workspace), int(bool(pooled_dy)), int(partial_rows), _st())
    else:
        call("ocr_bn_train_bwd", ptr(_dev(x2d)), ptr(y2d), ptr(dy2d), ptr(out), ptr(gamma), ptr(save_mean), ptr(save_rstd),
             ptr(dgamma), ptr(dbeta), M, C, int(relu), ptr(workspace), _st())
    return out


def bn_train_bwd_codes_col(x2d, codes, col, Nb, W, HC, dy_pooled_out, gamma, save_mean, save_rstd, dgamma, dbeta, relu, workspace, out=None):
    M, C = x2d.shape
    if out is None: out = torch.empty_like(x2d)
    assert codes.dtype == torch.int32 and tuple(codes.shape) == (M // 2, C // 8), (codes.dtype, tuple(codes.shape))
    assert (M // 2) * C == Nb * W * HC and dy_pooled_out.numel() == (M // 2) * C and col.numel() == Nb * (W - 1) * 2 * HC
    call("ocr_bn_train_bwd_codes_col", ptr(_dev(x2d)), ptr(codes), ptr(col), Nb, W, HC, ptr(dy_pooled_out), ptr(out), ptr(gamma),
         ptr(save_mean), ptr(save_rstd), ptr(dgamma), ptr(dbeta), M, C, int(relu), ptr(workspace), _st())
    return out


def conv3x3_stats_rows(Nb, W, H, Cin, Cout, *, bias=True, relu=False):
    flags = (EPI_BIAS if bias else 0) | (EPI_RELU if relu else 0)
    return int(nat.lib().ocr_conv3x3_stats_rows(int(Nb), int(W), int(H), int(Cin), int(Cout), flags))


def conv3x3_bnbwd_rows(Nb, W, H, Cin, Cout):
    return int(nat.lib().ocr_conv3x3_bnbwd_rows(int(Nb), int(W), int(H), int(Cin), int(Cout)))


def conv3x3_dgrad_bnbwd(dy, wdgrad, out, mask_y, z, mean, rstd, partials):
    Nb, W, H, Cin = dy.shape
    Cout = wdgrad.shape[0]
    call("ocr_conv3x3_dgrad_bnbwd_bf16", ptr(_dev(dy)), ptr(wdgrad), ptr(out), Nb, W, H, Cin, Cout, ptr(mask_y), ptr(z), ptr(mean), ptr(rstd),
# ... 213 lines not shown
```

Measured before the change: 58850 images/sec.

## Pair two conv3x3 weight-gradient kernels into one launch

Adds a paired wgrad9 launch that runs one layer's generic wgrad9 blocks and the next layer's wgrad9p blocks in a single grid, split by block index. The engine holds the first layer's wgrad until the paired partner's backward arrives and then dispatches both together, deferring their reductions as before. The aim is to fill the GPU with two small, under-occupied grids and cut one launch. In exchange, the held layer's wgrad runs later and the pair kernel carries both code paths, which may raise register or code-size pressure. The path only runs when the OCR_W9_PAIR switch is on and the shapes qualify.

```diff
diff --git a/include/ocr_hip.h b/include/ocr_hip.h
--- a/include/ocr_hip.h
+++ b/include/ocr_hip.h
@@ -97,6 +97,11 @@
 int ocr_conv3x3_wgrad_defer_bf16(const void* x, const void* dy, float* dw, float* dbias, int Nb, int W, int H, int Cin, int Cout,
                                  void* workspace, size_t workspace_bytes, void* job, int* job_blocks, int* deferred, void* stream);
 int ocr_wgrad9_reduce_jobs(const void* jobs, int njobs, int total_blocks, void* stream);
+int ocr_conv3x3_wgrad_pair_supported(const int* shape_first, const int* shape_second);
+int ocr_conv3x3_wgrad_pair_defer_bf16(const void* x0, const void* dy0, float* dw0, float* dbias0, const int* shape0, void* workspace0,
+                                      size_t workspace_bytes0, const void* x1, const void* dy1, float* dw1, float* dbias1, const int* shape1,
+                                      void* workspace1, size_t workspace_bytes1, void* job0, void* job1, int* job_blocks0, int* job_blocks1,
+                                      void* stream);
 
 int ocr_conv1_fwd(const float* x, const float* w, const float* bias, void* y, int Nb, int W, int H, int Cout,
                   int relu, void* stream);
diff --git a/lstm_ctc_ocr_amd/_native.py b/lstm_ctc_ocr_amd/_native.py
--- a/lstm_ctc_ocr_amd/_native.py
+++ b/lstm_ctc_ocr_amd/_native.py
@@ -55,6 +55,9 @@
     "ocr_conv3x3_wgrad_ws_bf16": ([_P, _P, _P, _P, _I, _I, _I, _I, _I, _I, _P, ctypes.c_size_t, _P], _I),
     "ocr_conv3x3_wgrad_defer_bf16": ([_P, _P, _P, _P, _I, _I, _I, _I, _I, _P, ctypes.c_size_t, _P, ctypes.POINTER(_I),
                                       ctypes.POINTER(_I), _P], _I),
+    "ocr_conv3x3_wgrad_pair_supported": ([ctypes.POINTER(_I), ctypes.POINTER(_I)], _I),
+    "ocr_conv3x3_wgrad_pair_defer_bf16": ([_P, _P, _P, _P, ctypes.POINTER(_I), _P, ctypes.c_size_t, _P, _P, _P, _P, ctypes.POINTER(_I), _P,
+                                           ctypes.c_size_t, _P, _P, ctypes.POINTER(_I), ctypes.POINTER(_I), _P], _I),
     "ocr_wgrad9_reduce_jobs": ([_P, _I, _I, _P], _I),
     "ocr_conv1_fwd": ([_P, _P, _P, _P, _I, _I, _I, _I, _I, _P], _I),
     "ocr_conv1_wgrad": ([_P, _P, _P, _P, _I, _I, _I, _I, _P], _I),
diff --git a/lstm_ctc_ocr_amd/csrc/common.h b/lstm_ctc_ocr_amd/csrc/common.h
--- a/lstm_ctc_ocr_amd/csrc/common.h
+++ b/lstm_ctc_ocr_amd/csrc/common.h
@@ -145,6 +145,8 @@
     return copysignf(t, x);
 }
 
+int ocr_cu_count();
+
 static inline const char* ocr_tune_env(const char* name) {
 #ifdef OCR_EXPERIMENTS
     return getenv(name);
diff --git a/lstm_ctc_ocr_amd/csrc/gemm.hip b/lstm_ctc_ocr_amd/csrc/gemm.hip
--- a/lstm_ctc_ocr_amd/csrc/gemm.hip
+++ b/lstm_ctc_ocr_amd/csrc/gemm.hip
@@ -294,6 +294,15 @@
     return k;
 }
 
+int ocr_cu_count() {
+    static int cus = 0;
+    if (!cus) {
+        int dev = 0; hipDeviceProp_t prop;
+        if (hipGetDevice(&dev) == hipSuccess && hipGetDeviceProperties(&prop, dev) == hipSuccess && prop.multiProcessorCount > 0) cus = prop.multiProcessorCount;
+    }
+    return cus > 0 ? cus : 256;
+}
+
 static bool plan_ws(ConvPlan& p, const ConvKnobs& k) {
     if (!k.ws || (p.flags & ~(EPI_BIAS | EPI_RELU | EPI_MASK))) return false;
     if (p.epi_kind && (!(p.flags & EPI_RELU) || (p.flags & EPI_MASK))) return false;
@@ -304,12 +313,7 @@
     else if (p.H == 8 && p.Cin == 128) { nc = 16; bm = 128; }
     else return false;
     if (p.W % nc || p.M % bm || (p.epi_kind == CONV_EPI_POOL22 && (p.W & 1))) return false;
-    static int cus = 0;
-    if (!cus) {
-        int dev = 0; hipDeviceProp_t prop;
-        if (hipGetDevice(&dev) == hipSuccess && hipGetDeviceProperties(&prop, dev) == hipSuccess && prop.multiProcessorCount > 0) cus = prop.multiProcessorCount;
-    }
-    const int ncu = cus > 0 ? cus : 256;
+    const int ncu = ocr_cu_count();
     const int mtiles = p.M / bm, ntiles = p.Cout / 64;
     if (k.ws == 1 && (p.Cin != 64 || (long)mtiles * ntiles < 2L * ncu)) return false;
     int slots = ncu / ntiles;
diff --git a/lstm_ctc_ocr_amd/csrc/gemm_tn.hip b/lstm_ctc_ocr_amd/csrc/gemm_tn.hip
--- a/lstm_ctc_ocr_amd/csrc/gemm_tn.hip
+++ b/lstm_ctc_ocr_amd/csrc/gemm_tn.hip
@@ -200,6 +200,10 @@
                         void* workspace, size_t ws_bytes, hipStream_t stream, void* defer_job = nullptr, int* defer_blocks = nullptr);
 int tn2_choice(int Mk, int I, int J, int mode, int splits, int nbatch, int* S);
 int wgrad9_choice(int Nb, int W, int H, int Cin, int Cout, int* S);
+bool wgrad9_pair_ok(int Nb0, int W0, int H0, int Cin0, int Cout0, int Nb1, int W1, int H1, int Cin1, int Cout1);
+int wgrad9_try_dispatch_pair(const void* const x[2], const void* const dy[2], float* const dw[2], float* const dbias[2], const int shape0[5],
+                             const int shape1[5], void* const workspace[2], const size_t ws_bytes[2], hipStream_t stream, void* const job[2],
+                             int* const job_blocks[2]);
 static int g_use_tn2 = 1, g_use_w9 = 1;
 extern "C" int ocr_set_wgrad_engine(int engine) { g_use_tn2 = engine != 0; g_use_w9 = engine >= 2; return OCR_OK; }
 
@@ -313,6 +317,29 @@
     return ocr_conv3x3_wgrad_bf16(x, dy, dw, dbias, Nb, W, H, Cin, Cout, 0, stream);
 }
 
+static bool w9_shape_valid(const int* s) { return s && s[0] > 0 && s[1] > 0 && s[2] > 0 && s[3] > 0 && s[4] > 0 && !(s[3] & 7) && !(s[4] & 7); }
+extern "C" int ocr_conv3x3_wgrad_pair_supported(const int* shape_first, const int* shape_second) {
+    if (!w9_shape_valid(shape_first) || !w9_shape_valid(shape_second)) return -OCR_ERR_INVALID;
+    const int *a = shape_first, *b = shape_second;
+    return g_use_w9 && wgrad9_pair_ok(a[0], a[1], a[2], a[3], a[4], b[0], b[1], b[2], b[3], b[4]) ? 1 : 0;
+}
+
+extern "C" int ocr_conv3x3_wgrad_pair_defer_bf16(const void* x0, const void* dy0, float* dw0, float* dbias0, const int* shape0, void* workspace0,
+                                                 size_t workspace_bytes0, const void* x1, const void* dy1, float* dw1, float* dbias1,
+                                                 const int* shape1, void* workspace1, size_t workspace_bytes1, void* job0, void* job1,
+                                                 int* job_blocks0, int* job_blocks1, void* stream) {
+    if (!x0 || !dy0 || !dw0 || !x1 || !dy1 || !dw1 || !workspace0 || !workspace1 || !job0 || !job1 || !job_blocks0 || !job_blocks1 ||
+        !w9_shape_valid(shape0) || !w9_shape_valid(shape1))
+        return OCR_ERR_INVALID;
+    if (!g_use_w9) return OCR_ERR_INVALID;
+    const void* const x[2] = {x0, x1}; const void* const dy[2] = {dy0, dy1};
+    float* const dw[2] = {dw0, dw1}; float* const db[2] = {dbias0, dbias1};
+    void* const ws[2] = {workspace0, workspace1}; const size_t wsb[2] = {workspace_bytes0, workspace_bytes1};
+    void* const job[2] = {job0, job1}; int* const nb[2] = {job_blocks0, job_blocks1};
+    const int rc = wgrad9_try_dispatch_pair(x, dy, dw, db, shape0, shape1, ws, wsb, (hipStream_t)stream, job, nb);
+    return rc < 0 ? OCR_ERR_INVALID : rc;
+}
+
 static void tn_wgrad_plan(int Mk, int Cin, int Cout, int splits, bool* big, int* k_per_split) {
     *big = (Cin >= 128 && Cout >= 128);
     long tiles = 9L * (*big ? (long)ceil_div(Cin, 128) * ceil_div(Cout, 128) : (long)ceil_div(Cin, 64) * ceil_div(Cout, 64));
diff --git a/lstm_ctc_ocr_amd/csrc/wgrad9.hip b/lstm_ctc_ocr_amd/csrc/wgrad9.hip
--- a/lstm_ctc_ocr_amd/csrc/wgrad9.hip
+++ b/lstm_ctc_ocr_amd/csrc/wgrad9.hip
@@ -71,8 +71,8 @@
     }
 }
 
-__device__ __forceinline__ void w9_block_decode(const W9Args& g, int& split, int& tile) {
-    const int b = blockIdx.x, T = g.T_ci * g.T_co;
+__device__ __forceinline__ void w9_block_decode(const W9Args& g, int b, int& split, int& tile) {
+    const int T = g.T_ci * g.T_co;
     if (g.map == 1) { const int x = b & 7, q = b >> 3; split = (q / T) * 8 + x; tile = q % T; }
     else if (g.map == 2) { const int x = b & 7, q = b >> 3, G = 8 / g.S; split = x / G; tile = (x % G) * (T / G) + q; }
     else { split = b / T; tile = b % T; }
@@ -131,7 +131,7 @@
     }
 }
 
-__global__ __launch_bounds__(512) void wgrad9_kernel(W9Args g) {
+__device__ __forceinline__ void wgrad9_body(const W9Args g, int bid) {
     extern __shared__ __attribute__((aligned(16))) unsigned char smem[];
     const int tid = threadIdx.x, lane = tid & 63;
     const unsigned lds0 = (unsigned)(size_t)(lptr_t)smem;
@@ -139,7 +139,7 @@
     const int cb = wave & 3, kh = wave >> 2;
     const int H = g.cH, W = g.cW;
     int split, tile;
-    w9_block_decode(g, split, tile);
+    w9_block_decode(g, bid, split, tile);
     const int ti = tile / g.T_co, tj = tile % g.T_co;
     const int ci0 = ti * 64, co0 = tj * 64;
     const int kbeg = split * g.k_per_split;
@@ -281,6 +281,7 @@
     if (do_cs) w9_cs_store(g, smem, cs, split, co0, tid);
     w9_store_tile(g, smem, acc, split, ci0, co0, cb, kh, lane);
 }
+__global__ __launch_bounds__(512) void wgrad9_kernel(W9Args g) { wgrad9_body(g, blockIdx.x); }
 
 __device__ long long* w9_dbg;
 #ifdef OCR_EXPERIMENTS
@@ -293,7 +294,7 @@
     return pl >= 0 && pl < H ? pl : -1;
 }
 template <int H, bool GENW>
-__global__ __launch_bounds__(512) void wgrad9p_kernel(W9Args g) {
+__device__ __forceinline__ void wgrad9p_body(const W9Args g, int bid) {
     constexpr int NC = 128 / H;
     constexpr int PS = (NC + 2 + 7) / 8 * 8;
     constexpr int XROWS = H * PS, XPIECES = XROWS / 8;
@@ -307,7 +308,7 @@
     const int cb = wave & 3, kh = wave >> 2;
     const int W = g.cW;
     int split, tile;
-    w9_block_decode(g, split, tile);
+    w9_block_decode(g, bid, split, tile);
     const int ti = tile / g.T_co, tj = tile % g.T_co;
     const int ci0 = ti * 64, co0 = tj * 64;
     const int kbeg = split * g.k_per_split;
@@ -451,6 +452,16 @@
     W9P_PHASE(4);
 #endif
 }
+template <int H, bool GENW>
+__global__ __launch_bounds__(512) void wgrad9p_kernel(W9Args g) { wgrad9p_body<H, GENW>(g, blockIdx.x); }
+
+template <int H, bool GENW>
+__global__ __launch_bounds__(512) void wgrad9p_kernel(W9Args first, W9Args second, int nblk_first) {
+    const int b = blockIdx.x;
+    if (b < nblk_first) wgrad9_body(first, b);
+    else if constexpr (H == 16) wgrad9_body(second, b - nblk_first);
+    else wgrad9p_body<H, GENW>(second, b - nblk_first);
+}
 
 __device__ __forceinline__ void w9_reduce_body(float* __restrict__ dw, const float* __restrict__ part, long n4, long slab4, int S, int rows,
                                                float* __restrict__ dbias, const float* __restrict__ cs_part, int Cout, int blk) {
@@ -556,50 +567,105 @@
     return k;
 }
 
+typedef void (*W9Kernel)(W9Args);
+typedef void (*W9PairKernel)(W9Args, W9Args, int);
+template <int H, bool GENW> constexpr W9Kernel W9P_SINGLE = wgrad9p_kernel<H, GENW>;
+template <int H, bool GENW> constexpr W9PairKernel W9P_PAIR = wgrad9p_kernel<H, GENW>;
+
 template <auto KERNEL>
 static int w9_launch(const W9Args& g, int grid, hipStream_t stream) {
     if (ocr_allow_lds<KERNEL>(W9_LDS) != hipSuccess) return OCR_ERR_EXEC;
     KERNEL<<<grid, 512, W9_LDS, stream>>>(g);
     return OCR_OK;
 }
+template <auto KERNEL>
+static int w9_launch_pair(const W9Args& first, int grid_first, const W9Args& second, int grid_second, hipStream_t stream) {
+    if (ocr_allow_lds<KERNEL>(W9_LDS) != hipSuccess) return OCR_ERR_EXEC;
+    KERNEL<<<grid_first + grid_second, 512, W9_LDS, stream>>>(first, second, grid_first);
+    return OCR_OK;
+}
+
+static int w9_setup(const void* x, const void* dy, float* dbias, int Nb, int W, int H, int Cin, int Cout, void* workspace, size_t ws_bytes,
+                    W9Plan* p, W9Args* g) {
+    const int M = Nb * W * H;
+    if (!workspace) return -1;
+    const int kern = w9_choose(M, W, H, Cin, Cout, p);
+    if (kern < 0 || ws_bytes < p->bytes) return -1;
+    *g = W9Args{};
+    g->X = (const bf16_t*)x; g->dY = (const bf16_t*)dy; g->M = M; g->Cin = Cin; g->Cout = Cout; g->cW = W; g->cH = H;
+    g->k_per_split = p->k_per_split; g->S = p->S; g->T_ci = p->T_ci; g->T_co = p->T_co; g->map = p->map;
+    g->part = (float*)workspace;
+    g->cs_part = dbias ? g->part + (size_t)p->S * 9 * Cin * Cout : nullptr;
+    return kern;
+}
+static W9ReduceJob w9_reduce_job(const W9Args& g, float* dw, float* dbias, int* blocks) {
+    const long n4 = (long)9 * g.Cin * g.Cout / 4;
+    int rows = g.S / 8;
+    rows = rows < 1 ? 1 : (rows > 8 ? 8 : rows);
+    while (rows & (rows - 1)) rows &= rows - 1;
+    const int cols = 256 / rows;
+    *blocks = (int)((n4 + cols - 1) / cols);
+    return W9ReduceJob{dw, g.part, dbias, g.cs_part, n4, n4, g.S, rows, g.Cout, 0};
+}
 
 int wgrad9_try_dispatch(const void* x, const void* dy, float* dw, float* dbias, int Nb, int W, int H, int Cin, int Cout,
                         void* workspace, size_t ws_bytes, hipStream_t stream, void* defer_job, int* defer_blocks) {
     W9Plan p;
-    const int M = Nb * W * H;
-    if (!workspace) return -1;
-    const int kern = w9_choose(M, W, H, Cin, Cout, &p);
-    if (kern < 0 || ws_bytes < p.bytes) return -1;
-    W9Args g = {};
-    g.X = (const bf16_t*)x; g.dY = (const bf16_t*)dy; g.M = M; g.Cin = Cin; g.Cout = Cout; g.cW = W; g.cH = H;
-    g.k_per_split = p.k_per_split; g.S = p.S; g.T_ci = p.T_ci; g.T_co = p.T_co; g.map = p.map;
-    g.part = (float*)workspace;
-    g.cs_part = dbias ? g.part + (size_t)p.S * 9 * Cin * Cout : nullptr;
+    W9Args g;
+    const int kern = w9_setup(x, dy, dbias, Nb, W, H, Cin, Cout, workspace, ws_bytes, &p, &g);
+    if (kern < 0) return -1;
     const int grid = p.S * p.T_ci * p.T_co;
     int rc;
     switch (kern) {
-        case W9K_P4: rc = w9_launch<wgrad9p_kernel<4, false>>(g, grid, stream); break;
-        case W9K_P8: rc = w9_launch<wgrad9p_kernel<8, false>>(g, grid, stream); break;
-        case W9K_P4_ZERO_ROW: rc = w9_launch<wgrad9p_kernel<4, true>>(g, grid, stream); break;
-        case W9K_P8_ZERO_ROW: rc = w9_launch<wgrad9p_kernel<8, true>>(g, grid, stream); break;
+        case W9K_P4: rc = w9_launch<W9P_SINGLE<4, false>>(g, grid, stream); break;
+        case W9K_P8: rc = w9_launch<W9P_SINGLE<8, false>>(g, grid, stream); break;
+        case W9K_P4_ZERO_ROW: rc = w9_launch<W9P_SINGLE<4, true>>(g, grid, stream); break;
+        case W9K_P8_ZERO_ROW: rc = w9_launch<W9P_SINGLE<8, true>>(g, grid, stream); break;
         default: rc = w9_launch<wgrad9_kernel>(g, grid, stream); break;
     }
     if (rc != OCR_OK) return rc;
     OCR_CHECK_LAUNCH();
-    const long n4 = (long)9 * Cin * Cout / 4;
-    int rows = p.S / 8;
-    rows = rows < 1 ? 1 : (rows > 8 ? 8 : rows);
-    while (rows & (rows - 1)) rows &= rows - 1;
-    const int cols = 256 / rows;
-    const int blocks = (int)((n4 + cols - 1) / cols);
+    int blocks;
+    const W9ReduceJob jb = w9_reduce_job(g, dw, dbias, &blocks);
     if (defer_job != nullptr) {
-        W9ReduceJob jb = {dw, g.part, dbias, g.cs_part, n4, n4, p.S, rows, Cout, 0};
         *(W9ReduceJob*)defer_job = jb;
         *defer_blocks = blocks;
         return OCR_OK;
     }
-    wgrad9_reduce_kernel<<<blocks, 256, 0, stream>>>(dw, g.part, n4, n4, p.S, rows, dbias, g.cs_part, Cout);
+    wgrad9_reduce_kernel<<<blocks, 256, 0, stream>>>(dw, g.part, jb.n4, jb.slab4, jb.S, jb.rows, dbias, g.cs_part, Cout);
     OCR_CHECK_LAUNCH();
+    return OCR_OK;
+}
+
+bool wgrad9_pair_ok(int Nb0, int W0, int H0, int Cin0, int Cout0, int Nb1, int W1, int H1, int Cin1, int Cout1) {
+    W9Plan p0, p1;
+    if (w9_choose(Nb0 * W0 * H0, W0, H0, Cin0, Cout0, &p0) != W9K_WGRAD9) return false;
+    if (w9_choose(Nb1 * W1 * H1, W1, H1, Cin1, Cout1, &p1) < 0) return false;
+    return 2 * p0.S * p0.T_ci * p0.T_co <= ocr_cu_count();
+}
+
+int wgrad9_try_dispatch_pair(const void* const x[2], const void* const dy[2], float* const dw[2], float* const dbias[2], const int shape0[5],
+                             const int shape1[5], void* const workspace[2], const size_t ws_bytes[2], hipStream_t stream, void* const job[2],
+                             int* const job_blocks[2]) {
+    if (!wgrad9_pair_ok(shape0[0], shape0[1], shape0[2], shape0[3], shape0[4], shape1[0], shape1[1], shape1[2], shape1[3], shape1[4])) return -1;
+    W9Plan p0, p1;
+    W9Args g0, g1;
+    const int k0 = w9_setup(x[0], dy[0], dbias[0], shape0[0], shape0[1], shape0[2], shape0[3], shape0[4], workspace[0], ws_bytes[0], &p0, &g0);
+    const int k1 = w9_setup(x[1], dy[1], dbias[1], shape1[0], shape1[1], shape1[2], shape1[3], shape1[4], workspace[1], ws_bytes[1], &p1, &g1);
+    if (k0 != W9K_WGRAD9 || k1 < 0) return -1;
+    const int grid0 = p0.S * p0.T_ci * p0.T_co, grid1 = p1.S * p1.T_ci * p1.T_co;
+    int rc;
+    switch (k1) {
+        case W9K_P4: rc = w9_launch_pair<W9P_PAIR<4, false>>(g0, grid0, g1, grid1, stream); break;
+        case W9K_P8: rc = w9_launch_pair<W9P_PAIR<8, false>>(g0, grid0, g1, grid1, stream); break;
+        case W9K_P4_ZERO_ROW: rc = w9_launch_pair<W9P_PAIR<4, true>>(g0, grid0, g1, grid1, stream); break;
+        case W9K_P8_ZERO_ROW: rc = w9_launch_pair<W9P_PAIR<8, true>>(g0, grid0, g1, grid1, stream); break;
+        default: rc = w9_launch_pair<W9P_PAIR<16, false>>(g0, grid0, g1, grid1, stream); break;
+    }
+    if (rc != OCR_OK) return rc;
+    OCR_CHECK_LAUNCH();
+    *(W9ReduceJob*)job[0] = w9_reduce_job(g0, dw[0], dbias[0], job_blocks[0]);
+    *(W9ReduceJob*)job[1] = w9_reduce_job(g1, dw[1], dbias[1], job_blocks[1]);
     return OCR_OK;
 }
 
diff --git a/lstm_ctc_ocr_amd/engine.py b/lstm_ctc_ocr_amd/engine.py
--- a/lstm_ctc_ocr_amd/engine.py
+++ b/lstm_ctc_ocr_amd/engine.py
@@ -26,10 +26,12 @@
         self.w9_pending, self.w9_tables = [], {}
         self.w9_pending_bytes = 0
         self.tn_pending = []
+        self.w9_held = None
         self.tn_side_open = False
         self.fused_pools = set()
         self.bn_stat_rows = {}
         self.bn_bwd_rows = {}
+        self.w9_hold_for = {}
         self.unpool_pools = set()
         self.col_bn = {}
         self.lstm_sync_keys = ()
@@ -65,6 +67,7 @@
             need = max(self.buf[k].numel() for k in own)
             for k in own:
                 del self.buf[k]
+            self.w9_hold_for.clear()
             self.buf['wgrad_ws'] = torch.empty(need, dtype=torch.uint8, device=dev)
         self.T, _, self.C = self.oshape[eng.ops[-1].key]
         self.costs = torch.zeros(N, dtype=F32, device=dev)
@@ -113,6 +116,7 @@
         self.overlap_allreduce = _switch('OCR_OVERLAP_ALLREDUCE')
         self.dp_graph = _env('OCR_DP_GRAPH', '0') == '1'
         self.defer_w9 = _switch('OCR_W9_DEFER')
+        self.w9_pair = _switch('OCR_W9_PAIR')
         self.w9_defer_max_bytes = _number('OCR_W9_DEFER_MAX_MB', self.W9_DEFER_MAX_BYTES >> 20) << 20
         self.w9_ws_pool = {}
         self.comm_stream = torch.cuda.Stream(device=self.device)
@@ -412,6 +416,7 @@
         sp.dy_done = set()
         sp.w9_pending = []
         sp.tn_pending = []
+        sp.w9_held = None
         logits = self.ops[-1].y(sp)
         scale = ocr_dist.loss_scale(sp.N, self.world)
         path = self.ctc_path_of(sp.C, sp.T)
@@ -429,6 +434,7 @@
             op.bwd(sp)
         self._flush_tn(sp)
         self._join_tn(sp)
+        self._release_w9(sp)
         if flush:
             self._flush_w9(sp)
 
@@ -450,6 +456,7 @@
             op.bwd(sp)
         self._flush_tn(sp)
         self._join_tn(sp)
+        self._release_w9(sp)
         self._flush_w9(sp)
 
     def tn_push(self, sp, job, keep, fallback):
@@ -484,7 +491,26 @@
     W9_JOB_DTYPE = np.dtype([('dw', '<u8'), ('part', '<u8'), ('dbias', '<u8'), ('cs_part', '<u8'), ('n4', '<i8'), ('slab4', '<i8'),
                              ('S', '<i4'), ('rows', '<i4'), ('Cout', '<i4'), ('block_start', '<i4')])
 
+    def w9_append(self, sp, job, ws):
+        sp.w9_pending.append(job)
+        sp.w9_pending_bytes += ws.numel()
+        if self.w9_flush_bytes and sp.w9_pending_bytes >= self.w9_flush_bytes:
+            self._flush_w9(sp)
+
+    def w9_hold(self, sp, key, x, dz, dw, db, ws):
+        self._release_w9(sp)
+        sp.w9_held = (key, x, dz, dw, db, ws)
+
+    def _release_w9(self, sp):
+        held, sp.w9_held = sp.w9_held, None
+        if held is not None:
+            _, x, dz, dw, db, ws = held
+            job, nblk = ops.conv3x3_wgrad_deferred(x, dz, dw, db, ws)
+            if job is not None:
+                self.w9_append(sp, (job, nblk), ws)
+
     def _flush_w9(self, sp):
+        self._release_w9(sp)
         pend, sp.w9_pending = sp.w9_pending, []
         sp.w9_pending_bytes = 0
         if not pend:
diff --git a/lstm_ctc_ocr_amd/engine_ops.py b/lstm_ctc_ocr_amd/engine_ops.py
--- a/lstm_ctc_ocr_amd/engine_ops.py
+++ b/lstm_ctc_ocr_amd/engine_ops.py
@@ -317,8 +317,24 @@
                     big = max(need, ops.conv3x3_wgrad_workspace_bytes(s[0], s[1] * scale, s[2], self.ci, self.co))
                 have_ws = pool[self.key] = torch.empty(big, dtype=torch.uint8, device=dev)
             sp.buf[self.key + '/w9ws'] = have_ws[:need]
+            if e.w9_pair:
+                self._plan_w9_pair(sp, s)
         elif need and (have is None or have.numel() < need):
             sp.buf['wgrad_ws'] = torch.empty(need, dtype=torch.uint8, device=dev)
+
+    def _plan_w9_pair(self, sp, s):
+        e = self.eng
+        i = e.ops.index(self)
+        for j in range(i - 1, -1, -1):
+            b = e.ops[j]
+            if isinstance(b, _Conv1Op) and b.key + '/slab' in sp.buf:
+                return
+            if isinstance(b, _Conv3x3Op) and b.key + '/w9ws' in sp.buf:
+                bs = sp.shape[b.key][0]
+                if ((i >= e.split_op) == (j >= e.split_op) and b.key not in sp.w9_hold_for
+                        and ops.conv3x3_wgrad_pair_supported((bs[0], bs[1], bs[2], b.ci, b.co), (s[0], s[1], s[2], self.ci, self.co))):
+                    sp.w9_hold_for[self.key] = b.key
+                return
 
     def _conv_fwd(self, sp, x, out, bias, codes):
         w, p = self.wpack.view(self.co, 3, 3, self.ci), self.pool_after
@@ -335,13 +351,19 @@
     def _conv_bwd(self, sp, x, dz, dw, db):
         e, o, p = self.eng, sp.shape[self.key][1], self.prev
         own_ws = sp.buf.get(self.key + '/w9ws')
-        if own_ws is not None:
+        held = sp.w9_held
+        if own_ws is not None and self.key in sp.w9_hold_for:
+            e.w9_hold(sp, self.key, x, dz, dw, db, own_ws)
+        elif own_ws is not None and held is not None and sp.w9_hold_for.get(held[0]) == self.key:
+            sp.w9_held = None
+            mine, theirs = ops.conv3x3_wgrad_pair_deferred((x, dz, dw, db, own_ws), held[1:])
+            e.w9_append(sp, theirs, held[5])
+            e.w9_append(sp, mine, own_ws)
+        elif own_ws is not None:
+            e._release_w9(sp)
             job, nblk = ops.conv3x3_wgrad_deferred(x, dz, dw, db, own_ws)
             if job is not None:
-                sp.w9_pending.append((job, nblk))
-                sp.w9_pending_bytes += own_ws.numel()
-                if e.w9_flush_bytes and sp.w9_pending_bytes >= e.w9_flush_bytes:
-                    e._flush_w9(sp)
+                e.w9_append(sp, (job, nblk), own_ws)
         else:
             ops.conv3x3_wgrad(x, dz, dw, dbias=db, workspace=sp.buf.get('wgrad_ws'))
         if p.key in sp.unpool_pools:
diff --git a/lstm_ctc_ocr_amd/ops.py b/lstm_ctc_ocr_amd/ops.py
--- a/lstm_ctc_ocr_amd/ops.py
+++ b/lstm_ctc_ocr_amd/ops.py
@@ -305,6 +305,26 @@
     call("ocr_conv3x3_wgrad_defer_bf16", ptr(_dev(x)), ptr(dy), ptr(dw), ptr(dbias), Nb, W, H, Cin, Cout, ptr(workspace),
          workspace.numel(), ctypes.cast(job, ctypes.c_void_p), ctypes.byref(nblk), ctypes.byref(deferred), _st())
     return (bytes(job), nblk.value) if deferred.value else (None, 0)
+
+
+def conv3x3_wgrad_pair_supported(shape_first, shape_second):
+    a, b = (ctypes.c_int * 5)(*[int(v) for v in shape_first]), (ctypes.c_int * 5)(*[int(v) for v in shape_second])
+    rc = nat.lib().ocr_conv3x3_wgrad_pair_supported(a, b)
+    if rc < 0:
+        raise nat.NativeError("ocr_conv3x3_wgrad_pair_supported failed: status %d (%s)" % (-rc, nat.status_string(-rc)))
+    return bool(rc)
+
+
+def conv3x3_wgrad_pair_deferred(first, second):
+    args, outs = [], []
+    for x, dy, dw, dbias, workspace in (first, second):
+        Nb, W, H, Cin = x.shape
+        shape = (ctypes.c_int * 5)(Nb, W, H, Cin, dy.shape[-1])
+        args += [ptr(_dev(x)), ptr(dy), ptr(dw), ptr(dbias), shape, ptr(workspace), workspace.numel()]
+        outs.append(((ctypes.c_ubyte * 64)(), ctypes.c_int(0)))
+    call("ocr_conv3x3_wgrad_pair_defer_bf16", *args, ctypes.cast(outs[0][0], ctypes.c_void_p), ctypes.cast(outs[1][0], ctypes.c_void_p),
+         ctypes.byref(outs[0][1]), ctypes.byref(outs[1][1]), _st())
+    return tuple((bytes(job), nblk.value) for job, nblk in outs)
 
 
 def wgrad9_reduce_jobs(table, njobs, total_blocks):
```

Measured after the change: 59740 images/sec, median of 6. 1.5% higher.
